# zaiisao/ConTEXTure-NeRF

Measured on AMD Instinct MI355X. Metric: UNet denoise steps/sec (CFG-batched SD2-depth UNet eval + PLMS update), higher is better.
Workload: dtype f16; 1 GPU; BASELINE configs[1]: 1 view @768^2 (latent 96^2), 50 PLMS steps (51 UNet evals), SD2-depth UNet fp16, CFG batch 2, guidance 10, random-init weights; mesh substitution napoleon.obj -> n/a for this stage (denoise loop only); latent=96, cfg_batch=2, ctx_len=77, views_per_rank=1, parallelism=view-shard x1

## Files before the change

contexture-nerf_amd/_lib.py:

```python
import ctypes as C
import os
import torch

_HERE = os.path.dirname(os.path.abspath(__file__))
LIB_PATH = os.path.join(_HERE, "libctxnerf.so")

_vp, _i32, _i64, _f32 = C.c_void_p, C.c_int32, C.c_int64, C.c_float

SIGNATURES = {
    "ctx_version": (_i32, []),
    "ctx_last_error": (C.c_char_p, []),
    "ctx_device_check": (_i32, []),
    "ctx_prepare_vertices": (_i32, [_vp, _vp, _vp, _vp, _i32, _i32, _i32, _vp, _vp, _vp, _vp, _vp]),
    "ctx_rasterize_ws_bytes": (_i64, [_i32, _i32, _i32, _i32]),
    "ctx_rasterize_fwd": (_i32, [_i32, _i32, _vp, _vp, _vp, _i32, _i32, _i32, _f32, _f32, _vp, _vp, _vp, _i64, _vp]),
    "ctx_rasterize_fused": (_i32, [_i32, _i32, _vp, _vp, _vp, _i32, _vp, _i32, _i32, _f32, _f32, _vp, _vp, _vp, _vp, _vp, _i64, _vp]),
    "ctx_normalize_depth_ws_bytes": (_i64, [_i32]),
    "ctx_normalize_depth": (_i32, [_vp, _i32, _i32, _vp, _vp, _vp, _vp]),
    "ctx_texture_mapping_fwd": (_i32, [_vp, _vp, _i32, _i32, _i32, _i32, _i32, _i32, _vp, _vp, _vp]),
    "ctx_texture_mapping_bwd": (_i32, [_vp, _vp, _i32, _i32, _i32, _i32, _vp, _vp, _vp]),
    "ctx_texmap_bwd_plan_bytes": (_i64, [_i32, _i32, _i32]),
    "ctx_texmap_bwd_plan": (_i32, [_vp, _vp, _i32, _i32, _i32, _vp, _vp]),
    "ctx_texture_mapping_bwd_binned_ws_bytes": (_i64, [_i32, _i32]),
    "ctx_texture_mapping_bwd_binned": (_i32, [_vp, _vp, _vp, _i32, _i32, _i32, _i32, _vp, _vp, _vp, _vp]),
    "ctx_texmap_plan_max_res": (_i32, []),
    "ctx_texmap_plan_stale": (_i32, [_vp, _vp]),
    "ctx_uv_scatter_fixed": (_i32, [_vp, _vp, _vp, _i32, _i32, _i32, _i32, _vp, _i32, _vp, _vp]),
    "ctx_fixed_to_float": (_i32, [_vp, _i64, _i32, _i32, _vp, _vp]),
    "ctx_uv_gather_ws_bytes": (_i64, [_i32, _i32]),
    "ctx_uv_gather_fixed": (_i32, [_vp, _vp, _vp, _vp, _vp, _vp, _vp, _i32, _i32, _i32, _i32, _i32, _i32, _i32, _vp, _vp, _i64, _vp]),
    "ctx_atlas_fill_ws_bytes": (_i64, [_i32]),
    "ctx_nearest_seed": (_i32, [_vp, _i32, _vp, _vp, _vp, _i64, _vp]),
    "ctx_atlas_fill": (_i32, [_vp, _vp, _vp, _i32, _i32, _i32, _vp, _vp, _vp, _i64, _vp]),
    "ctx_view_consistency_ws_bytes": (_i64, [_i32, _i32]),
    "ctx_view_consistency_fwd": (_i32, [_vp, _vp, _vp, _vp, _i32, _i32, _i32, _i32, _i32, _i32, _i32, _i32, _vp, _i64, _vp, _vp, _vp, _vp, _vp]),
    "ctx_view_consistency_bwd": (_i32, [_vp, _vp, _vp, _vp, _vp, _i32, _i32, _i32, _i32, _i32, _i32, _i32, _vp, _vp, _vp, _vp, _vp]),
    "ctx_texture_pack4": (_i32, [_vp, _i32, _i32, _vp, _vp]),
    "ctx_texture_mapping_packed_fwd": (_i32, [_vp, _vp, _i32, _i32, _i32, _i32, _i32, _vp, _vp, _vp]),
    "ctx_view_weights_max": (_i32, [_vp, _vp, _i32, _i32, _i32, _vp, _vp, _vp]),
    "ctx_view_weights_mask": (_i32, [_vp, _vp, _vp, _i32, _i32, _i32, _vp, _vp]),
    "ctx_face_view_map_ws_bytes": (_i64, [_i32, _i32, _i32]),
    "ctx_face_view_map": (_i32, [_vp, _i32, _i32, _i32, _vp, _vp, _vp, _vp]),
    "ctx_embed_fwd": (_i32, [_vp, _i64, _i32, _i32, _vp, _vp]),
    "ctx_uvmlp_packed_bytes": (_i64, [_i32, _i32, _i32, _i32, _i32]),
    "ctx_uvmlp_pack": (_i32, [_vp, _vp, _i32, _i32, _i32, _i32, _i32, _vp, _vp]),
    "ctx_uvmlp_fwd": (_i32, [_vp, _vp, _i64, _i32, _vp, _i32, _i32, _i32, _i32, _i32, _vp, _vp, _vp]),
    "ctx_uvmlp_saved_bytes": (_i64, [_i64, _i32, _i32, _i32]),
    "ctx_uvmlp_fwd_save": (_i32, [_vp, _vp, _i64, _i32, _vp, _i32, _i32, _i32, _i32, _i32, _i32, _vp, _vp, _vp, _vp]),
    "ctx_uvmlp_bwd_ws_bytes": (_i64, [_i64, _i32, _i32]),
    "ctx_uvmlp_bwd": (_i32, [_vp, _vp, _vp, _i64, _vp, _i32, _i32, _i32, _i32, _i32, _i32, _vp, _vp, _vp, _vp, _vp]),
    "ctx_texel_active_mark": (_i32, [_vp, _vp, _i32, _i32, _i32, _i32, _vp, _vp]),
    "ctx_texel_compact_ws_bytes": (_i64, [_i64]),
    "ctx_texel_compact": (_i32, [_vp, _i64, _vp, _vp, _vp, _vp]),
    "ctx_uvmlp_fwd_save_idx": (_i32, [_vp, _i64, _i32, _vp, _i32, _i32, _i32, _i32, _i32, _vp, _vp, _vp, _vp]),
    "ctx_uvmlp_bwd_idx": (_i32, [_vp, _vp, _vp, _i32, _vp, _i64, _vp, _i32, _i32, _i32, _i32, _i32, _vp, _vp, _vp, _vp, _vp]),
    "ctx_get_rays": (_i32, [_i32, _i32, _f32, _f32, _f32, _f32, _vp, _vp, _vp, _vp]),
    "ctx_raymarch_composite_fwd": (_i32, [_vp, _vp, _vp, _i64, _i32, _i32, _vp, _vp, _vp, _vp, _vp, _vp]),
    "ctx_raymarch_composite_fwd_noise": (_i32, [_vp, _vp, _vp, _vp, _i64, _i32, _i32, _vp, _vp, _vp, _vp, _vp, _vp]),
    "ctx_raymarch_composite_bwd": (_i32, [_vp, _vp, _vp, _vp, _i64, _i32, _i32, _vp, _vp, _vp, _vp, _vp, _vp, _vp]),
    "ctx_unet_create": (_vp, [_vp]),
    "ctx_unet_destroy": (None, [_vp]),
    "ctx_unet_param_count": (_i32, [_vp]),
    "ctx_unet_param_name": (C.c_char_p, [_vp, _i32]),
    "ctx_unet_param_shape": (_i32, [_vp, _i32, _vp]),
    "ctx_unet_weight_bytes": (_i64, [_vp]),
    "ctx_unet_workspace_bytes": (_i64, [_vp, _i32, _i32, _i32, _i32]),
    "ctx_unet_bind": (_i32, [_vp, _vp, _vp, _i64]),
    "ctx_unet_set_param": (_i32, [_vp, _i32, _vp, _vp]),
    "ctx_unet_forward": (_i32, [_vp, _vp, _vp, _vp, _i32, _i32, _i32, _i32, _vp, _vp]),
    "ctx_controlnet_create": (_vp, [_vp, _i32]),
    "ctx_controlnet_residual_bytes": (_i64, [_vp, _i32, _i32, _i32]),
    "ctx_controlnet_cond_cache_bytes": (_i64, [_vp, _i32, _i32, _i32]),
    "ctx_controlnet_forward": (_i32, [_vp, _vp, _vp, _vp, _vp, _vp, _i32, _i32, _i32, _i32, _i32, _vp, _vp]),
    "ctx_unet_set_residuals": (_i32, [_vp, _vp, C.c_float]),
    "ctx_unet_ref_bank_bytes": (_i64, [_vp, _i32, _i32, _i32]),
    "ctx_unet_workspace_bytes_ref": (_i64, [_vp, _i32, _i32, _i32, _i32, _i32, _i32]),
    "ctx_unet_forward_ref": (_i32, [_vp, _vp, _vp, _vp, _i32, _i32, _i32, _i32, _i32, _vp, _i32, _vp, _vp]),
    "ctx_unet_set_residual_fp32": (_i32, [_vp, _i32]),
    "ctx_unet_stats": (_i32, [_vp, _i32, _vp, _vp]),
    "ctx_unet_set_taps": (_i32, [_vp, _vp, _i64]),
    "ctx_unet_tap_count": (_i32, [_vp]),
    "ctx_unet_tap_info": (_i32, [_vp, _i32, _vp, _vp, _vp]),
    "ctx_vae_create": (_vp, [_vp]),
    "ctx_vae_destroy": (None, [_vp]),
    "ctx_vae_param_count": (_i32, [_vp]),
    "ctx_vae_param_name": (C.c_char_p, [_vp, _i32]),
    "ctx_vae_param_shape": (_i32, [_vp, _i32, _vp]),
    "ctx_vae_weight_bytes": (_i64, [_vp]),
    "ctx_vae_workspace_bytes": (_i64, [_vp, _i32, _i32, _i32]),
    "ctx_vae_bind": (_i32, [_vp, _vp, _vp, _i64]),
    "ctx_vae_set_param": (_i32, [_vp, _i32, _vp, _vp]),
    "ctx_vae_decode": (_i32, [_vp, _vp, _i32, _i32, _i32, _vp, _vp]),
    "ctx_vae_decoder_param_count": (_i32, [_vp]),
    "ctx_vae_encode_workspace_bytes": (_i64, [_vp, _i32, _i32, _i32]),
    "ctx_vae_encode": (_i32, [_vp, _vp, _i32, _i32, _i32, _vp, _vp]),
    "ctx_vae_flops": (C.c_double, [_vp]),
    "ctx_vae_encode_train_workspace_bytes": (_i64, [_vp, _i32, _i32, _i32]),
    "ctx_vae_encode_train": (_i32, [_vp, _vp, _i32, _i32, _i32, _vp, _vp]),
    "ctx_vae_encode_bwd": (_i32, [_vp, _vp, _f32, _vp, _vp]),
    "ctx_gemm_f16": (_i32, [_vp, _vp, _vp, _vp, _i32, _i32, _i32, _vp, _vp]),
    "ctx_conv3x3_f16": (_i32, [_vp, _vp, _vp, _vp, _vp, _i32, _i32, _i32, _i32, _i32, _i32, _i32, _vp, _vp]),
    "ctx_groupnorm_f16": (_i32, [_vp, _vp, _vp, _i32, _i32, _i32, _i32, _f32, _i32, _vp, _vp, _vp]),
    "ctx_layernorm_f16": (_i32, [_vp, _vp, _vp, _i64, _i32, _f32, _vp, _vp]),
    "ctx_attention_ws_bytes": (_i64, [_i32, _i32, _i32]),
    "ctx_attention_f16": (_i32, [_vp, _vp, _vp, _i32, _i32, _i32, _i32, _i32, _i32, _f32, _vp, _i32, _vp, _vp]),
    "ctx_groupnorm_ws_bytes": (_i64, [_i32, _i32]),
    "ctx_geglu_f16": (_i32, [_vp, _i64, _i32, _vp, _vp]),
    "ctx_profile_begin": (_i32, []),
    "ctx_profile_end": (_i32, [_i32, _vp, _vp]),
    "ctx_bench_gemm": (C.c_float, [_vp, _vp, _vp, _vp, _i32, _i32, _i32, _vp, _i32, _i32, _i32, _i32, _i32, _i32, _vp, _i32, _i32, _vp]),
    "ctx_gemm_tune": (None, [_i32, _i32]),
    "ctx_attention_tune": (None, [_i32, _i32, _i32, _f32]),
    "ctx_probe_mfma": (_i32, [_i32, _vp, _vp, _vp, _vp]),
    "ctx_probe_stage": (C.c_float, [_i32, _i32, _i32, _i32, _i32, _vp, _vp, _vp]),
    "ctx_cfg_plms_step": (_i32, [_vp, _i64, _f32, _vp, _i32, _vp, _f32, _f32, _i32, _vp, _vp, _vp]),
}


class CtxError(RuntimeError):
    pass


_lib = None


def load():
    global _lib
    if _lib is None:
        if not os.path.exists(LIB_PATH):
            raise CtxError(f"{LIB_PATH} is missing: run `python -c 'import __graft_entry__ as g; g.build()'` "
                           "(hipcc --offload-arch=gfx950). There is no CPU fallback for this path.")
        lib = C.CDLL(LIB_PATH)
        for name, (res, args) in SIGNATURES.items():
            if not hasattr(lib, name) and os.environ.get("CTX_ALLOW_PARTIAL") == "1":
                continue
            fn = getattr(lib, name)
            fn.restype = res
            fn.argtypes = args
        _lib = lib
    return _lib


def check(rc):
    if rc != 0:
        raise CtxError(f"libctxnerf error {rc}: {load().ctx_last_error().decode()}")


def stream():
    return C.c_void_p(torch.cuda.current_stream().cuda_stream)


def ptr(t, dtype=None, name="tensor"):
    if t is None:
        return C.c_void_p(0)
    if not isinstance(t, torch.Tensor) or not t.is_cuda:
        raise CtxError(f"{name}: expected a device tensor (the HIP path has no CPU fallback), got "
                       f"{type(t).__name__} on {getattr(t, 'device', '?')}")
    if not t.is_contiguous():
        raise CtxError(f"{name}: tensor must be contiguous")
    if dtype is not None and t.dtype != dtype:
        raise CtxError(f"{name}: expected dtype {dtype}, got {t.dtype}")
    return C.c_void_p(t.data_ptr())


def f32c(t, device=None):
    t = t.to(dtype=torch.float32)
    if device is not None:
        t = t.to(device)
    return t.contiguous()
```

contexture-nerf_amd/csrc/conv_halo.hip:

```cpp
#include "gemm_common.h"

#define CH_HP 328
#define CH_XPIECES 41

template <int NI>
__global__ __launch_bounds__(512) void k_conv_halo(GemmArgs a)
{
    constexpr int BN = 64 * NI;
    constexpr int WP = NI;
    constexpr int G = 1 + WP;
    constexpr int HALO = CH_HP * 64;
    constexpr int WST = BN * 64;
    extern __shared__ __attribute__((aligned(16))) f16 smem[];
    f16 *halo = smem;
    f16 *wring = smem + 2 * HALO;
    f16 *scratch = wring + 4 * WST;

    const int tid = threadIdx.x, lane = tid & 63, wave = __builtin_amdgcn_readfirstlane(tid >> 6);
    const int r = lane & 31, h = lane >> 5;
    const int wm = wave >> 1, wn = wave & 1;

    const int pw = a.W >> 4, ph = a.H >> 4;
    const int ntiles = a.ntm * a.ntn;
    const int lin = xcd_remap(blockIdx.x, ntiles * a.splitk);
// ... 53 lines not shown
    for (int mi = 0; mi < 2; ++mi) rc[mi] = (2 * wm + mi + 8 * (r >> 4) + 1) * 18 + (r & 15) + 1;
    const int wswz = (r >> 1) & 7;
    const int wrow = (wn * 32 * NI + r) * 64;

#pragma unroll
    for (int i = 0; i < 6; ++i) issue_x(wave + 8 * i, cbeg, 0);
    issue_w(0);
    issue_w(1);
    issue_w(2);
    asm volatile("s_waitcnt vmcnt(%0)" ::"n"(2 * WP) : "memory");
    ctx_barrier();
    const int grp = wave >> 2;
    if (grp == 1) ctx_barrier();

    for (int g = 0; g < nst; ++g) {
        const int ci = g / 9, t = g - ci * 9;
        const f16 *hb = halo + (ci & 1) * HALO;
        const f16 *wb = wring + (g & 3) * WST + wrow;
        const int dy = t / 3 - 1, dx = t - (t / 3) * 3 - 1;
        const int toff = dy * 18 + dx;
        int xr[2], xs[2];
#pragma unroll
        for (int mi = 0; mi < 2; ++mi) { const int R = rc[mi] + toff; xr[mi] = R * 64; xs[mi] = (R >> 1) & 7; }
        f16x8 xf[4][2], wf[4][NI];
#pragma unroll
        for (int ks = 0; ks < 4; ++ks) {
#pragma unroll
            for (int mi = 0; mi < 2; ++mi) xf[ks][mi] = *(const f16x8 *)(hb + xr[mi] + (((2 * ks + h) ^ xs[mi]) * 8));
#pragma unroll
            for (int j = 0; j < NI; ++j) wf[ks][j] = *(const f16x8 *)(wb + j * 32 * 64 + (((2 * ks + h) ^ wswz) * 8));
        }
        if (g == 0) asm volatile("s_waitcnt vmcnt(%0)" ::"n"(WP) : "memory");
        else asm volatile("s_waitcnt vmcnt(%0)" ::"n"(G) : "memory");
        __builtin_amdgcn_sched_barrier(0);
        ctx_barrier();
        __builtin_amdgcn_sched_barrier(0);
        __builtin_amdgcn_s_setprio(1);
#pragma unroll
        for (int ks = 0; ks < 4; ++ks) {
#pragma unroll
            for (int mi = 0; mi < 2; ++mi)
#pragma unroll
                for (int j = 0; j < NI; ++j) acc[mi][j] = __builtin_amdgcn_mfma_f32_32x32x16_f16(wf[ks][j], xf[ks][mi], acc[mi][j], 0, 0, 0);
            if (ks == 0) issue_x(t * 8 + wave, cbeg + ci + 1, (ci + 1) & 1);
            if (ks == 1) issue_w(g + 3);
        }
        __builtin_amdgcn_s_setprio(0);
        __builtin_amdgcn_sched_barrier(0);
        ctx_barrier();
        __builtin_amdgcn_sched_barrier(0);
    }
    if (grp == 0) ctx_barrier();
    asm volatile("s_waitcnt vmcnt(0)" ::: "memory");

    const int nw = n0 + wn * 32 * NI;
#pragma unroll
    for (int mi = 0; mi < 2; ++mi) {
        const int y = py0 + 2 * wm + mi + 8 * (r >> 4), x = px0 + (r & 15);
        const size_t m = ((size_t)b * a.H + y) * a.W + x;
        if (a.splitk > 1) {
            float *pb = a.part + ((size_t)slice * a.M + m) * a.N;
#pragma unroll
            for (int j = 0; j < NI; ++j)
#pragma unroll
                for (int g4 = 0; g4 < 4; ++g4) store_part4(a, pb, nw + j * 32 + 8 * g4 + 4 * h, acc4(acc[mi][j], g4));
            continue;
        }
        const int bidx = a.rowbias ? (int)(m / a.rows_per_batch) : 0;
#pragma unroll
        for (int j = 0; j < NI; ++j)
#pragma unroll
            for (int g4 = 0; g4 < 4; ++g4) {
                const int nn = nw + j * 32 + 8 * g4 + 4 * h;
                if (nn >= a.N) continue;
                f32x4 v = acc4(acc[mi][j], g4);
                if (a.bias) v = add4(v, *(const f16x4 *)(a.bias + nn));
                store4(a, v, m, bidx, nn);
            }
    }
}

int ctx_conv_halo_try(GemmArgs &a, int ni, hipStream_t s)
{
    if (a.stride != 1 || a.ups != 0 || (a.H & 15) || (a.W & 15) || a.Cin % 64 != 0 || a.epi != 0 || a.N % 8 != 0) return 0;
    const int B = a.M / (a.H * a.W);
    const int BN = 64 * ni;
    a.ntm = B * (a.H >> 4) * (a.W >> 4);
    a.ntn = cdiv(a.N, BN);
    const int S = (a.splitk > 1 && a.part) ? a.splitk : 1;
    if (S > a.Cin / 64) return 0;
    a.splitk = S;
    const size_t lds = (size_t)(2 * CH_HP * 64 + 4 * BN * 64 + 8 * 512) * sizeof(f16);
    const dim3 grid(a.ntm * a.ntn * S);
    if (ni == 2) ctx_launch<k_conv_halo<2>>(0, grid, dim3(512), lds, s, a); else ctx_launch<k_conv_halo<1>>(0, grid, dim3(512), lds, s, a);
    return 1;
}
```

contexture-nerf_amd/csrc/engine.h:

```cpp
#pragma once
#include "common.h"
#include "kernels.h"
#include <string>
#include <vector>

enum PackKind { PK_COPY = 0, PK_CONV3 = 1, PK_CONVIN = 2, PK_GEGLU_W = 3, PK_GEGLU_B = 4 };

struct Param {
    std::string name;
    int ndim;
    int64_t shape[4];
    int kind;
    size_t dst;
    int a, b;
    int kind2 = 0; size_t dst2 = 0; int pad2 = 0, ld2 = 0, col2 = 0;
};

struct Engine {
    const char *tag = "";
    std::vector<Param> params;
    size_t wtop = 0;
    f16 *W = nullptr;
    char *ws = nullptr;
    size_t ws_cap = 0;
    size_t top = 0, peak = 0;
    bool dry = false;
    hipStream_t s = nullptr;
    int rc = 0;
    int64_t launches[3] = {0, 0, 0};
    double flops[3] = {0, 0, 0};

    size_t walloc(size_t n) { size_t o = wtop; wtop += (n + 127) / 128 * 128; return o; }
    size_t add(const std::string &name, std::vector<int64_t> shp, int kind, size_t dst, int a = 0, int b = 0)
    {
        Param p; p.name = name; p.ndim = (int)shp.size(); p.kind = kind; p.dst = dst; p.a = a; p.b = b;
        for (int i = 0; i < 4; ++i) p.shape[i] = i < p.ndim ? shp[i] : 1;
        params.push_back(p);
        return dst;
    }
    size_t vec(const std::string &name, int n) { return add(name, {n}, PK_COPY, walloc(n)); }
    size_t lin(const std::string &name, int out, int in) { return add(name, {out, in}, PK_COPY, walloc((size_t)out * in)); }

    void *alloc(size_t bytes)
    {
        size_t o = (top + 255) / 256 * 256;
        top = o + bytes;
        if (top > peak) peak = top;
        if (!dry && top > ws_cap) { rc = CTX_E_STATE; ctx_set_error("%s: workspace too small (%zu > %zu)", tag, top, ws_cap); return ws; }
        return dry ? nullptr : (void *)(ws + o);
    }
    f16 *allocH(size_t n) { return (f16 *)alloc(n * 2); }

    void begin() { top = 0; peak = 0; rc = 0; for (int k = 0; k < 3; ++k) { launches[k] = 0; flops[k] = 0; } }
    void note(int klass, double fl, int n = 1) { launches[klass] += n; flops[klass] += fl; }
    bool live() const { return !dry && rc == 0; }
    void copy(void *dst, const void *src, size_t bytes) { if (live()) (void)hipMemcpyAsync(dst, src, bytes, hipMemcpyDeviceToDevice, s); }
    void copy2d(void *dst, size_t dpitch, const void *src, size_t spitch, size_t width, size_t rows)
    { if (live()) (void)hipMemcpy2DAsync(dst, dpitch, src, spitch, width, rows, hipMemcpyDeviceToDevice, s); }
};

#define ENGINE_RUN(e, expr) do { if ((e)->live()) { int r__ = (expr); if (r__ != 0) (e)->rc = r__; } } while (0)
#define ENGINE_LAUNCH(e, kernel, grid, block, lds, ...) do { if ((e)->live()) hipLaunchKernelGGL(kernel, grid, block, lds, (e)->s, __VA_ARGS__); } while (0)

void engine_linear(Engine &e, const f16 *X, const f16 *Wt, const f16 *bias, const void *res, int M, int N, int K, void *out, int ldc = 0,
                   int epi = 0, bool res32 = false, bool out32 = false);
struct ConvGeom { int stride = 1, ups = 0, poff = 0, zins = 0; };
void engine_conv3(Engine &e, const f16 *x, const f16 *Wt, const f16 *bias, const void *res, int B, int H, int W, int Cin, int Cout, void *out,
                  ConvGeom g = ConvGeom(), const f16 *rowbias = nullptr, int ldrb = 0, bool res32 = false, bool out32 = false);

template <class F> int engine_dry_run(Engine *e, F run)
{
    const bool was = e->dry;
    e->dry = true; const int rc = run(); e->dry = was;
    return rc;
}
inline int64_t engine_workspace_need(const Engine *e) { return (int64_t)e->peak + 4096; }
int engine_finish(Engine *e, const char *who);

int32_t engine_param_count(const Engine *e);
const char *engine_param_name(const Engine *e, int32_t i);
int32_t engine_param_shape(const Engine *e, int32_t i, int64_t shape4[4]);
int64_t engine_weight_bytes(const Engine *e);
int32_t engine_bind(Engine *e, void *weights, void *workspace, int64_t workspace_bytes, const char *who);
int32_t engine_set_param(Engine *e, int32_t i, const float *src, ctx_stream_t stream, const char *who);
```

contexture-nerf_amd/csrc/engine.hip:

```cpp
#include "engine.h"

int32_t engine_param_count(const Engine *e) { return e ? (int32_t)e->params.size() : 0; }
const char *engine_param_name(const Engine *e, int32_t i)
{
    return (e && i >= 0 && i < (int)e->params.size()) ? e->params[i].name.c_str() : "";
}
int32_t engine_param_shape(const Engine *e, int32_t i, int64_t shape4[4])
{
    if (!e || i < 0 || i >= (int)e->params.size()) return 0;
    for (int k = 0; k < 4; ++k) shape4[k] = e->params[i].shape[k];
    return e->params[i].ndim;
}
int64_t engine_weight_bytes(const Engine *e) { return e ? (int64_t)e->wtop * 2 + 256 : 0; }

int32_t engine_bind(Engine *e, void *weights, void *workspace, int64_t workspace_bytes, const char *who)
{
    CTX_REQUIRE(e && weights && workspace && workspace_bytes > 0, "%s: bad args", who);
    CTX_REQUIRE(((uintptr_t)weights & 255) == 0 && ((uintptr_t)workspace & 255) == 0, "%s: blobs must be 256-byte aligned", who);
    e->W = (f16 *)weights; e->ws = (char *)workspace; e->ws_cap = (size_t)workspace_bytes;
    return CTX_OK;
}

static void engine_gemm(Engine &e, GemmArgs &a, bool conv)
{
    e.note(0, 2.0 * a.M * a.N * a.K);
    size_t mark = e.top;
    ctx_gemm_plan(a, conv);
    if (a.zins) a.use8 = 0;
    if (a.splitk > 1) a.part = (float *)e.alloc((size_t)a.splitk * a.M * a.N * 4);
    ENGINE_RUN(&e, ctx_gemm_dispatch(a, conv, e.s));
    e.top = mark;
}

void engine_linear(Engine &e, const f16 *X, const f16 *Wt, const f16 *bias, const void *res, int M, int N, int K, void *out, int ldc, int epi,
                   bool res32, bool out32)
{
    GemmArgs a = {};
    a.X = X; a.Wt = Wt; a.bias = bias; a.residual = (const f16 *)res; a.out = (f16 *)out;
    a.M = M; a.N = N; a.K = K; a.ldc = ldc ? ldc : epi == 1 ? N / 2 : N; a.ldr = N; a.rows_per_batch = 1; a.ldrb = N; a.epi = epi;
    a.res32 = res32; a.out32 = out32;
    engine_gemm(e, a, false);
}

void engine_conv3(Engine &e, const f16 *x, const f16 *Wt, const f16 *bias, const void *res, int B, int H, int W, int Cin, int Cout, void *out,
                  ConvGeom g, const f16 *rowbias, int ldrb, bool res32, bool out32)
{
    GemmArgs a = {};
    a.Ho = ((H << g.ups) - 1) / g.stride + 1; a.Wo = ((W << g.ups) - 1) / g.stride + 1;
    a.X = x; a.Wt = Wt; a.bias = bias; a.rowbias = rowbias; a.residual = (const f16 *)res; a.out = (f16 *)out;
    a.M = B * a.Ho * a.Wo; a.N = Cout; a.K = 9 * Cin; a.ldc = Cout; a.ldr = Cout; a.rows_per_batch = a.Ho * a.Wo; a.ldrb = ldrb;
    a.H = H; a.W = W; a.Cin = Cin; a.stride = g.stride; a.ups = g.ups; a.poff = g.poff; a.zins = g.zins;
    a.res32 = res32; a.out32 = out32;
    engine_gemm(e, a, true);
}

int engine_finish(Engine *e, const char *who)
{
    if (e->live()) CTX_CHECK_LAUNCH(who);
    return e->rc;
}

__global__ void k_pack_copy(const float *__restrict__ s, int64_t n, f16 *__restrict__ d)
{
    for (int64_t i = (int64_t)blockIdx.x * 256 + threadIdx.x; i < n; i += (int64_t)gridDim.x * 256) d[i] = (f16)s[i];
}
__global__ void k_pack_conv3(const float *__restrict__ s, int Cout, int Cin, int Cinp, f16 *__restrict__ d)
{
    int64_t n = (int64_t)Cout * 9 * Cinp;
    for (int64_t i = (int64_t)blockIdx.x * 256 + threadIdx.x; i < n; i += (int64_t)gridDim.x * 256) {
        int c = (int)(i % Cinp);
        int tap = (int)((i / Cinp) % 9);
        int o = (int)(i / ((int64_t)Cinp * 9));
        d[i] = c < Cin ? (f16)s[((int64_t)o * Cin + c) * 9 + tap] : (f16)0.f;
    }
}
__global__ void k_pack_geglu(const float *__restrict__ s, int C4, int K, f16 *__restrict__ d)
{
    int64_t n = (int64_t)2 * C4 * (K > 0 ? K : 1);
    int kk = K > 0 ? K : 1;
    for (int64_t i = (int64_t)blockIdx.x * 256 + threadIdx.x; i < n; i += (int64_t)gridDim.x * 256) {
        int k = (int)(i % kk);
        int p = (int)(i / kk);
        int blk = p / 64, w = p % 64;
        int src = w < 32 ? blk * 32 + w : C4 + blk * 32 + (w - 32);
        d[i] = (f16)s[(int64_t)src * kk + k];
    }
}
__global__ void k_pack_conv3_T(const float *__restrict__ s, int Cout, int Cin, int pad, f16 *__restrict__ d)
{
    int64_t n = (int64_t)Cin * 9 * pad;
    for (int64_t i = (int64_t)blockIdx.x * 256 + threadIdx.x; i < n; i += (int64_t)gridDim.x * 256) {
        int o = (int)(i % pad), tp = (int)((i / pad) % 9), c = (int)(i / ((int64_t)pad * 9));
        int ky = 2 - tp / 3, kx = 2 - tp % 3;
        d[i] = o < Cout ? (f16)s[(((int64_t)o * Cin + c) * 3 + ky) * 3 + kx] : (f16)0.f;
    }
}
__global__ void k_pack_mat_T(const float *__restrict__ s, int out, int in, int ld, int col, f16 *__restrict__ d)
{
    int64_t n = (int64_t)out * in;
    for (int64_t i = (int64_t)blockIdx.x * 256 + threadIdx.x; i < n; i += (int64_t)gridDim.x * 256) {
        int c = (int)(i % in), o = (int)(i / in);
        d[(int64_t)c * ld + col + o] = (f16)s[i];
    }
}

int32_t engine_set_param(Engine *e, int32_t i, const float *src, ctx_stream_t stream, const char *who)
{
    CTX_REQUIRE(e && e->W && src && i >= 0 && i < (int)e->params.size(), "%s: bad args / not bound", who);
    const Param &p = e->params[i];
    hipStream_t s = (hipStream_t)stream;
    int64_t n = 1;
    for (int k = 0; k < p.ndim; ++k) n *= p.shape[k];
    f16 *d = e->W + p.dst;
    int64_t nbk = cdiv64(n, 256);
    unsigned nb = (unsigned)(nbk > 4096 ? 4096 : nbk);
    switch (p.kind) {
    case PK_COPY: hipLaunchKernelGGL(k_pack_copy, dim3(nb), dim3(256), 0, s, src, n, d); break;
    case PK_CONV3: hipLaunchKernelGGL(k_pack_conv3, dim3(nb), dim3(256), 0, s, src, p.a, p.b, p.b, d); break;
    case PK_CONVIN: hipLaunchKernelGGL(k_pack_conv3, dim3(nb), dim3(256), 0, s, src, p.a, p.b, p.b > 8 ? 16 : 8, d); break;
    case PK_GEGLU_W: hipLaunchKernelGGL(k_pack_geglu, dim3(nb), dim3(256), 0, s, src, p.a, p.b, d); break;
    case PK_GEGLU_B: hipLaunchKernelGGL(k_pack_geglu, dim3(nb), dim3(256), 0, s, src, p.a, 0, d); break;
    }
    if (p.kind2 == 1) hipLaunchKernelGGL(k_pack_conv3_T, dim3(nb), dim3(256), 0, s, src, p.a, p.b, p.pad2, e->W + p.dst2);
    else if (p.kind2 == 2) hipLaunchKernelGGL(k_pack_mat_T, dim3(nb), dim3(256), 0, s, src, (int)p.shape[0], (int)p.shape[1], p.ld2, p.col2, e->W + p.dst2);
    CTX_CHECK_LAUNCH(who);
    return CTX_OK;
}
```

contexture-nerf_amd/csrc/gemm.hip:

```cpp
#include "gemm_common.h"

template <int MI, int NI>
__device__ __forceinline__ void gemm_epilogue(const GemmArgs &a, f32x16 (&acc)[MI][NI], int mw, int nw, int r, int h)
{
#pragma unroll
    for (int mi = 0; mi < MI; ++mi) {
        int m = mw + mi * 32 + r;
        if (m >= a.M) continue;
        int bidx = a.rowbias ? m / a.rows_per_batch : 0;
        if (a.epi == 1) {
            if constexpr (NI == 2) {
                int fbase = nw / 2;
#pragma unroll
                for (int g = 0; g < 4; ++g) {
                    int nn = nw + 8 * g + 4 * h;
                    if (nn >= a.N) continue;
                    f16x4 o;
#pragma unroll
                    for (int j = 0; j < 4; ++j) {
                        float xv = acc[mi][0][4 * g + j], gv = acc[mi][1][4 * g + j];
                        if (a.bias) { xv += (float)a.bias[nn + j]; gv += (float)a.bias[nn + 32 + j]; }
                        o[j] = geglu(xv, gv);
                    }
                    *(f16x4 *)(a.out + (size_t)m * a.ldc + fbase + 8 * g + 4 * h) = o;
                }
            }
        } else {
#pragma unroll
            for (int ni = 0; ni < NI; ++ni)
#pragma unroll
                for (int g = 0; g < 4; ++g) {
                    int nn = nw + ni * 32 + 8 * g + 4 * h;
                    if (nn >= a.N) continue;
                    f32x4 v = acc4(acc[mi][ni], g);
                    if (a.bias) v = add4(v, *(const f16x4 *)(a.bias + nn));
                    store4<true>(a, v, m, bidx, nn);
                }
        }
    }
}

template <int MI, int NI>
__device__ __forceinline__ void gemm_epilogue_staged(const GemmArgs &a, f32x16 (&acc)[MI][NI], int mw, int nw, int r, int h,
                                                     float *stage, int lane)
{
    constexpr int RS = 32 * NI + 4;
    constexpr int LPR = 4 * NI;
    constexpr int RPP = 64 / LPR;
    const int prow = lane / LPR, c8 = (lane % LPR) * 8;
    const int n = nw + c8;
    f16x8 bs = {0, 0, 0, 0, 0, 0, 0, 0};
    if (a.bias && n < a.N) bs = *(const f16x8 *)(a.bias + n);
#pragma unroll
    for (int mi = 0; mi < MI; ++mi) {
#pragma unroll
        for (int ni = 0; ni < NI; ++ni)
#pragma unroll
            for (int g = 0; g < 4; ++g)
                *(f32x4 *)(stage + r * RS + ni * 32 + 8 * g + 4 * h) = acc4(acc[mi][ni], g);
#pragma unroll
        for (int p = 0; p < 32 / RPP; ++p) {
            const int row = RPP * p + prow;
            const int m = mw + mi * 32 + row;
            f32x4 v0 = *(const f32x4 *)(stage + row * RS + c8), v1 = *(const f32x4 *)(stage + row * RS + c8 + 4);
            if (m < a.M && n < a.N) {
                float v[8] = {v0[0], v0[1], v0[2], v0[3], v1[0], v1[1], v1[2], v1[3]};
                add8(v, bs);
                store8<true>(a, v, m, n);
            }
        }
    }
}

template <int WM, int WN, int MI, int NI, bool CONV, int NS, int PKT>
__global__ __launch_bounds__(64 * WM * WN) void k_gemm_pipe(GemmArgs a)
{
    constexpr int BM = 32 * MI * WM, BN = 32 * NI * WN, NW = WM * WN;
    constexpr int RP = 512 / PKT;
    constexpr int LPR = PKT / 8;
    constexpr int XI = BM / (RP * NW), WI = BN / (RP * NW);
    static_assert(XI >= 1 && WI >= 1, "tile too small for the wave count");
    constexpr int G = XI + WI;
    constexpr int STAGE = (BM + BN) * PKT;
    extern __shared__ __attribute__((aligned(16))) f16 smem[];

    const int tid = threadIdx.x, lane = tid & 63, wave = __builtin_amdgcn_readfirstlane(tid >> 6);
    const int r = lane & 31, h = lane >> 5;
    const int wm = wave / WN, wn = wave % WN;
    const GemmTile t = gemm_tile(a, blockIdx.x, PKT, BM, BN);
    const int slice = t.slice, tile_m = t.tile_m, tile_n = t.tile_n, m0 = t.m0, n0 = t.n0, kbeg = t.kbeg, nk = t.nk;
    const int lr = lane / LPR, pc = lane % LPR;

    const f16 *xp[XI], *wp[WI];
    int xst[XI], wst[WI];
    int xoff[XI], xoy[XI], xox[XI];
    bool xok[XI];
#pragma unroll
    for (int i = 0; i < XI; ++i) {
        int row = RP * (wave + NW * i) + lr;
        int m = m0 + row;
        const int lc = (pc ^ (PKT == 32 ? ((row >> 2) & 3) : ((row >> 1) & 7))) * 8;
        xok[i] = m < a.M;
        if (CONV) {
            conv_pixel(a, m, lc, xoy[i], xox[i], xoff[i]);
            xp[i] = ctx_zero_page; xst[i] = 0;
        } else {
            xoff[i] = 0; xoy[i] = 0; xox[i] = 0;
            xp[i] = xok[i] ? a.X + (size_t)m * a.K + kbeg * PKT + lc : ctx_zero_page;
            xst[i] = xok[i] ? PKT : 0;
        }
    }
#pragma unroll
    for (int i = 0; i < WI; ++i) {
        int row = RP * (wave + NW * i) + lr;
        bool ok = (n0 + row) < a.N;
        wp[i] = ok ? a.Wt + (size_t)(n0 + row) * a.K + kbeg * PKT + ((pc ^ (PKT == 32 ? ((row >> 2) & 3) : ((row >> 1) & 7))) * 8) : ctx_zero_page;
        wst[i] = ok ? PKT : 0;
    }
    const int k_lo = kbeg * PKT, k_hi = (kbeg + nk) * PKT;
    const int rot = a.krot == 1 ? (int)(((unsigned)tile_m * 13u + (unsigned)tile_n * 5u) % (unsigned)nk) : 0;
    int k_issue = k_lo + rot * PKT, issued = 0, tap_left = 0;
    if (!CONV) {
#pragma unroll
        for (int i = 0; i < XI; ++i) xp[i] += (xst[i] ? rot * PKT : 0);
    }
#pragma unroll
    for (int i = 0; i < WI; ++i) wp[i] += (wst[i] ? rot * PKT : 0);

    auto retap = [&]() {
        const ConvTap tap = conv_tap(a, k_issue);
#pragma unroll
        for (int i = 0; i < XI; ++i) {
            bool ok = xok[i];
            xp[i] = conv_tap_src<true>(a, tap, xoy[i], xox[i], xoff[i], ok);
            xst[i] = ok ? PKT : 0;
        }
        tap_left = (a.Cin - tap.c0) / PKT;
    };
    auto issue = [&](int buf) {
        if (k_issue == k_hi) {
            k_issue = k_lo;
            const int span = k_hi - k_lo;
            if (!CONV) {
#pragma unroll
                for (int i = 0; i < XI; ++i) xp[i] -= (xst[i] ? span : 0);
            }
#pragma unroll
            for (int i = 0; i < WI; ++i) wp[i] -= (wst[i] ? span : 0);
            tap_left = 0;
        }
        if (CONV) {
            if (tap_left == 0) retap();
            --tap_left;
        }
        f16 *Xs = smem + buf * STAGE;
        f16 *Ws = Xs + BM * PKT;
#pragma unroll
        for (int i = 0; i < XI; ++i) {
            __builtin_amdgcn_global_load_lds((gptr_t)xp[i], (lptr_t)(Xs + (wave + NW * i) * 512), 16, 0, 0);
            xp[i] += xst[i];
        }
#pragma unroll
        for (int i = 0; i < WI; ++i) {
            __builtin_amdgcn_global_load_lds((gptr_t)wp[i], (lptr_t)(Ws + (wave + NW * i) * 512), 16, 0, 0);
            wp[i] += wst[i];
        }
        k_issue += PKT;
        ++issued;
    };

    f32x16 acc[MI][NI];
#pragma unroll
    for (int i = 0; i < MI; ++i)
#pragma unroll
        for (int j = 0; j < NI; ++j)
#pragma unroll
            for (int q = 0; q < 16; ++q) acc[i][j][q] = 0.f;

#pragma unroll
    for (int p = 0; p < NS - 1; ++p)
        if (p < nk) issue(p);
    const int swz = PKT == 32 ? ((r >> 2) & 3) : ((r >> 1) & 7);
    const int xrow = (wm * 32 * MI + r) * PKT, wrow = BM * PKT + (wn * 32 * NI + r) * PKT;
    int kt = 0;
    for (; a.krot == 0 && kt + 2 * NS - 2 < nk; kt += NS) {
#pragma unroll
        for (int u = 0; u < NS; ++u) {
            asm volatile("s_waitcnt vmcnt(%0) lgkmcnt(0)" ::"n"((NS - 2) * G) : "memory");
            ctx_barrier();
            issue((u + NS - 1) % NS);
            const f16 *sb = smem + u * STAGE;
#pragma unroll
            for (int ks = 0; ks < PKT / 16; ++ks) {
                const int pch = ((2 * ks + h) ^ swz) * 8;
                f16x8 xf[MI], wf[NI];
#pragma unroll
                for (int i = 0; i < MI; ++i) xf[i] = *(const f16x8 *)(sb + xrow + i * 32 * PKT + pch);
#pragma unroll
                for (int j = 0; j < NI; ++j) wf[j] = *(const f16x8 *)(sb + wrow + j * 32 * PKT + pch);
#pragma unroll
                for (int i = 0; i < MI; ++i)
#pragma unroll
                    for (int j = 0; j < NI; ++j) acc[i][j] = __builtin_amdgcn_mfma_f32_32x32x16_f16(wf[j], xf[i], acc[i][j], 0, 0, 0);
            }
        }
    }
    for (; kt < nk; kt += NS) {
#pragma unroll
        for (int u = 0; u < NS; ++u) {
            if (kt + u < nk) {
                int newer = issued - 1 - (kt + u);
                if (NS >= 8 && newer >= 6) asm volatile("s_waitcnt vmcnt(%0)" ::"n"(6 * G) : "memory");
                else if (NS >= 7 && newer >= 5) asm volatile("s_waitcnt vmcnt(%0)" ::"n"(5 * G) : "memory");
                else if (NS >= 6 && newer >= 4) asm volatile("s_waitcnt vmcnt(%0)" ::"n"(4 * G) : "memory");
                else if (NS >= 5 && newer >= 3) asm volatile("s_waitcnt vmcnt(%0)" ::"n"(3 * G) : "memory");
                else if (NS >= 4 && newer >= 2) asm volatile("s_waitcnt vmcnt(%0)" ::"n"(2 * G) : "memory");
                else if (newer >= 1) asm volatile("s_waitcnt vmcnt(%0)" ::"n"(G) : "memory");
                else asm volatile("s_waitcnt vmcnt(0)" ::: "memory");
                asm volatile("s_waitcnt lgkmcnt(0)" ::: "memory");
                ctx_barrier();
                if (issued < nk) issue((u + NS - 1) % NS);
                const f16 *sb = smem + u * STAGE;
#pragma unroll
                for (int ks = 0; ks < PKT / 16; ++ks) {
                    const int pch = ((2 * ks + h) ^ swz) * 8;
                    f16x8 xf[MI], wf[NI];
#pragma unroll
                    for (int i = 0; i < MI; ++i) xf[i] = *(const f16x8 *)(sb + xrow + i * 32 * PKT + pch);
#pragma unroll
                    for (int j = 0; j < NI; ++j) wf[j] = *(const f16x8 *)(sb + wrow + j * 32 * PKT + pch);
#pragma unroll
                    for (int i = 0; i < MI; ++i)
#pragma unroll
                        for (int j = 0; j < NI; ++j) acc[i][j] = __builtin_amdgcn_mfma_f32_32x32x16_f16(wf[j], xf[i], acc[i][j], 0, 0, 0);
                }
            }
        }
    }
    if (a.splitk > 1) {
        float *pb = a.part + (size_t)slice * a.M * a.N;
#pragma unroll
        for (int mi = 0; mi < MI; ++mi) {
            int m = m0 + wm * 32 * MI + mi * 32 + r;
            if (m >= a.M) continue;
#pragma unroll
            for (int ni = 0; ni < NI; ++ni)
#pragma unroll
                for (int g = 0; g < 4; ++g)
                    store_part4(a, pb + (size_t)m * a.N, n0 + wn * 32 * NI + ni * 32 + 8 * g + 4 * h, acc4(acc[mi][ni], g));
        }
        return;
    }
    if (a.epi == 0 && a.stage_epi) {
        asm volatile("s_waitcnt vmcnt(0) lgkmcnt(0)" ::: "memory");
        ctx_barrier();
        gemm_epilogue_staged<MI, NI>(a, acc, m0 + wm * 32 * MI, n0 + wn * 32 * NI, r, h, (float *)smem + wave * (32 * (32 * NI + 4)), lane);
        return;
    }
    gemm_epilogue<MI, NI>(a, acc, m0 + wm * 32 * MI, n0 + wn * 32 * NI, r, h);
}

__global__ __launch_bounds__(256) void k_splitk_reduce(GemmArgs a)
{
    const int n4 = a.N / 4;
    const size_t total = (size_t)a.M * n4, MN = (size_t)a.M * a.N;
    for (size_t i = (size_t)blockIdx.x * 256 + threadIdx.x; i < total; i += (size_t)gridDim.x * 256) {
        int m = (int)(i / n4), nn = (int)(i % n4) * 4;
        f32x4 v = *(const f32x4 *)(a.part + (size_t)m * a.N + nn);
        for (int sidx = 1; sidx < a.splitk; ++sidx) {
            f32x4 p = *(const f32x4 *)(a.part + sidx * MN + (size_t)m * a.N + nn);
            v += p;
        }
        if (a.bias) v = add4(v, *(const f16x4 *)(a.bias + nn));
        store4<true>(a, v, m, a.rowbias ? m / a.rows_per_batch : 0, nn);
    }
}

static int g_force_tile = -1, g_force_gemm8 = -1;
extern "C" void ctx_gemm_tune(int32_t tile, int32_t gemm8)
{
    g_force_tile = tile;
    g_force_gemm8 = gemm8;
}

template <int WM, int WN, int MI, int NI, bool CONV, int NS = 4, int PKT = 32>
static void launch_gemm(GemmArgs &a, hipStream_t s)
{
    constexpr int BM = 32 * MI * WM, BN = 32 * NI * WN;
    a.ntm = cdiv(a.M, BM);
    a.ntn = cdiv(a.N, BN);
    if (a.splitk < 1 || !a.part) a.splitk = 1;
    static const int mfast = ctx_env_int("CTX_GEMM_MFAST", -1);
    a.mfast = mfast >= 0 ? mfast : ctx_gemm_mfast(a, CONV);
    static const int stg = ctx_env_int("CTX_GEMM_STAGE_EPI", 1);
    a.stage_epi = stg && (a.ldc % 8 == 0) && (!a.residual || a.ldr % 8 == 0) && (!a.rowbias || a.ldrb % 8 == 0) &&
                  (size_t)WM * WN * 32 * (32 * NI + 4) * sizeof(float) <= 160 * 1024;
    static const int steady = ctx_env_int("CTX_GEMM_STEADY", 1);
    a.pk = PKT; a.krot = steady ? 0 : 2;
    constexpr int NT = 64 * WM * WN;
    constexpr size_t ring = (size_t)NS * (BM + BN) * PKT * sizeof(f16);
    constexpr size_t patch = (size_t)WM * WN * 32 * (32 * NI + 4) * sizeof(float);
    constexpr size_t lds = (ring > patch || patch > 160 * 1024) ? ring : patch;
    ctx_launch<k_gemm_pipe<WM, WN, MI, NI, CONV, NS, PKT>>(0, dim3(a.ntm * a.ntn * a.splitk), dim3(NT), lds, s, a);
}

static void launch_reduce(GemmArgs &a, hipStream_t s)
{
    size_t total = (size_t)a.M * (a.N / 4);
    unsigned nb = (unsigned)((total + 255) / 256 < 2048 ? (total + 255) / 256 : 2048);
    ctx_launch<k_splitk_reduce>(0, dim3(nb), dim3(256), 0, s, a);
}

int ctx_gemm_pick_split(int M, int N, int K, int epi)
{
    static const int en = ctx_env_int("CTX_SPLITK", 1);
    if (!en || epi != 0 || N % 4) return 1;
    bool wide = (N % 128 == 0);
    int tiles = wide ? cdiv(M, 128) * cdiv(N, 128) : cdiv(M, 256) * cdiv(N, 64);
    if (tiles >= 200) return 1;
    if (K < 2048 && tiles > 48) return 1;
    int S = 640 / tiles;
    int maxS = (K / 32) / 8;
    if (S > maxS) S = maxS;
    if (S > 32) S = 32;
    return S < 2 ? 1 : S;
}

#include "gemm_tuned.h"
void ctx_gemm_plan(GemmArgs &a, bool conv)
{
    a.tile = -1; a.use8 = -1;
    static const int use_table = ctx_env_int("CTX_GEMM_TUNED", 1);
    if (use_table) {
        const int flags = conv ? ((a.stride == 2 ? 1 : 0) | (a.ups ? 2 : 0)) : 0;
        for (const TunedGemm &t : g_tuned)
            if (t.conv == (conv ? 1 : 0) && t.M == a.M && t.N == a.N && t.K == a.K && t.flags == flags && t.epi == a.epi) {
                a.tile = t.tile; a.use8 = t.use8; a.splitk = t.splitk;
                return;
            }
    }
    if (a.K % 64 == 0 && (!conv || a.Cin % 64 == 0)) {
        const double MN = (double)a.M * a.N;
        static const int heur144 = ctx_env_int("CTX_GEMM_HEUR144", 1);
        if (heur144 && a.epi == 0 && a.N % 8 == 0 && !a.zins && !a.res32 && !a.out32) {
            const int nt = cdiv(a.N, 160);
            const double fill = (double)a.N / (160.0 * nt);
            if (fill >= 0.9) {
                if (cdiv(a.M, 288) * nt >= 512) { a.tile = -1; a.use8 = 8; a.splitk = 1; return; }
                if (cdiv(a.M, 144) * nt >= 220) { a.tile = -1; a.use8 = 6; a.splitk = 1; return; }
            }
        }
        int tile, bm, bn;
        if (MN >= 5.0e6) { tile = a.epi == 1 ? 10 : (conv ? 12 : 11); bm = 256; bn = 128; }
        else if ((MN >= 2.5e6 && a.K >= 960) || (conv && MN >= 1.2e6 && a.K >= 5760)) { tile = 14; bm = 128; bn = 128; }
        else if (a.epi == 1) { tile = 16; bm = 64; bn = 128; }
        else { tile = 15; bm = 64; bn = 64; }
        const int tiles = cdiv(a.M, bm) * cdiv(a.N, bn);
        int S = 1;
        if (a.epi == 0 && a.N % 4 == 0) {
            S = 320 / tiles;
            const int maxS = a.K / 64 / 4;
            if (S > maxS) S = maxS;
            if (S > 12) S = 12;
            if (S < 1) S = 1;
        }
        a.tile = tile; a.splitk = S;
        a.use8 = (a.epi == 1 && MN >= 1.0e7) ? -1 : 0;
        return;
    }
    a.splitk = ctx_gemm_pick_split(a.M, a.N, a.K, a.epi);
}

int ctx_gemm_dispatch(GemmArgs &a, bool conv, hipStream_t s)
{
    const bool only_pipe = a.zins || a.res32 || a.out32;
    if (only_pipe) a.use8 = 0;
    const int want8 = only_pipe ? 0 : (g_force_gemm8 >= 0 ? g_force_gemm8 : a.use8);
    const int want_tile = g_force_tile >= 0 ? g_force_tile : (g_force_gemm8 >= 0 ? -1 : a.tile);
    const bool launched = want_tile < 0 && ((want8 >= 4 && want8 <= 8 && ctx_gemm144_try(a, conv, want8 - 4, s)) ||
                                            (conv && (want8 == 2 || want8 == 3) && ctx_conv_halo_try(a, want8 == 2 ? 2 : 1, s)) ||
                                            (want8 != 0 && want8 < 2 && ctx_gemm8_try(a, conv, want8 == 1, s)));
    if (!launched) {
        static const int big = ctx_env_int("CTX_GEMM_BIG", 1);
        const int S = a.splitk > 1 && a.part ? a.splitk : 1;
        auto wgs = [&](int bm, int bn) { return cdiv(a.M, bm) * cdiv(a.N, bn) * S; };
        const bool n128 = (a.N % 128 == 0);
        int pick;
        static const int bigk = ctx_env_int("CTX_GEMM_BIGK", 1024);
        if (big && a.M >= 8192 && a.N >= 256 && a.K >= bigk) pick = 0;
        else if (n128 && wgs(128, 128) >= 384) pick = 1;
        else if (!n128 && wgs(256, 64) >= 384) pick = 2;
        else if (wgs(128, 64) >= 320) pick = 3;
        else if (S > 1) pick = n128 ? 1 : 2;
        else pick = 4;
        static const int force = ctx_env_int("CTX_GEMM_TILE", -1);
        if (force >= 0) pick = force;
        if (want_tile >= 0) pick = want_tile;
        if (a.epi == 1 && (pick == 5 || pick == 6 || pick == 9 || pick == 11 || pick == 13 || pick == 15 || pick == 17 || pick == 19 || pick == 21 || pick == 23 || pick == 26 || pick == 27)) pick = 1;
        if (pick >= 10 && (a.K % 64 != 0 || (conv && a.Cin % 64 != 0))) pick = 1;
#define CTX_LAUNCH(WM_, WN_, MI_, NI_) do { if (conv) launch_gemm<WM_, WN_, MI_, NI_, true>(a, s); else launch_gemm<WM_, WN_, MI_, NI_, false>(a, s); } while (0)
        switch (pick) {
        case 0: CTX_LAUNCH(4, 2, 2, 2); break;
        case 1: CTX_LAUNCH(2, 2, 2, 2); break;
        case 2: CTX_LAUNCH(4, 1, 2, 2); break;
        case 3: CTX_LAUNCH(2, 1, 2, 2); break;
        case 4: CTX_LAUNCH(1, 1, 2, 2); break;
        case 5: CTX_LAUNCH(2, 2, 1, 1); break;
        case 6: CTX_LAUNCH(1, 2, 2, 1); break;
        case 7: CTX_LAUNCH(4, 2, 1, 2); break;
        case 8: CTX_LAUNCH(2, 2, 1, 2); break;
        case 9: CTX_LAUNCH(2, 2, 2, 1); break;
#define CTX_LAUNCH64(WM_, WN_, MI_, NI_) do { if (conv) launch_gemm<WM_, WN_, MI_, NI_, true, 3, 64>(a, s); else launch_gemm<WM_, WN_, MI_, NI_, false, 3, 64>(a, s); } while (0)
        case 10: CTX_LAUNCH64(8, 2, 1, 2); break;
        case 11: CTX_LAUNCH64(4, 4, 2, 1); break;
        case 12: CTX_LAUNCH64(4, 2, 2, 2); break;
        case 13: CTX_LAUNCH64(4, 4, 1, 1); break;
        case 14: CTX_LAUNCH64(4, 2, 1, 2); break;
        case 15: CTX_LAUNCH64(2, 2, 1, 1); break;
        case 16: CTX_LAUNCH64(2, 2, 1, 2); break;
        case 17: CTX_LAUNCH64(2, 2, 2, 1); break;
        case 18: CTX_LAUNCH64(2, 2, 2, 2); break;
#define CTX_LAUNCH64N2(WM_, WN_, MI_, NI_) do { if (conv) launch_gemm<WM_, WN_, MI_, NI_, true, 2, 64>(a, s); else launch_gemm<WM_, WN_, MI_, NI_, false, 2, 64>(a, s); } while (0)
        case 19: CTX_LAUNCH64N2(2, 2, 1, 1); break;
        case 20: CTX_LAUNCH64N2(4, 2, 1, 2); break;
        case 21: CTX_LAUNCH64N2(4, 4, 1, 1); break;
        case 22: CTX_LAUNCH64N2(2, 2, 2, 2); break;
#define CTX_LAUNCH64NS(NS_, WM_, WN_, MI_, NI_) do { if (conv) launch_gemm<WM_, WN_, MI_, NI_, true, NS_, 64>(a, s); else launch_gemm<WM_, WN_, MI_, NI_, false, NS_, 64>(a, s); } while (0)
        case 23: CTX_LAUNCH64NS(6, 2, 2, 1, 1); break;
        case 24: CTX_LAUNCH64NS(5, 2, 2, 1, 2); break;
        case 25: CTX_LAUNCH64NS(4, 4, 2, 1, 2); break;
        case 26: CTX_LAUNCH64NS(5, 2, 2, 2, 1); break;
        default: CTX_LAUNCH64N2(4, 2, 2, 5); break;
#undef CTX_LAUNCH64NS
#undef CTX_LAUNCH64N2
#undef CTX_LAUNCH64
        }
#undef CTX_LAUNCH
    }
    if (a.splitk > 1) launch_reduce(a, s);
    hipError_t e = hipGetLastError();
    if (e != hipSuccess) {
        ctx_set_error("gemm launch failed: %s", hipGetErrorString(e));
        return CTX_E_LAUNCH;
    }
    return CTX_OK;
}

extern "C" int32_t ctx_gemm_f16(const void *A, const void *Wt, const void *bias, const void *residual, int32_t M,
                                int32_t N, int32_t K, void *C, ctx_stream_t stream)
{
    CTX_REQUIRE(A && Wt && C, "gemm: null pointer");
    CTX_REQUIRE(M > 0 && N > 0 && K > 0 && K % 64 == 0 && N % 8 == 0, "gemm: need K%%64==0, N%%8==0 (M=%d N=%d K=%d)", M, N, K);
    CTX_REQUIRE((int64_t)M * K < (1ll << 31) && (int64_t)N * K < (1ll << 31), "gemm: operand too large for 32-bit offsets");
    GemmArgs a = {};
    a.X = (const f16 *)A; a.Wt = (const f16 *)Wt; a.bias = (const f16 *)bias; a.residual = (const f16 *)residual;
    a.out = (f16 *)C; a.M = M; a.N = N; a.K = K; a.ldc = N; a.ldr = N; a.rows_per_batch = 1; a.ldrb = N; a.epi = 0;
    a.tile = -1; a.use8 = -1;
    return ctx_gemm_dispatch(a, false, (hipStream_t)stream);
}

extern "C" int32_t ctx_conv3x3_f16(const void *x, const void *w, const void *bias, const void *rowbias,
                                   const void *residual, int32_t B, int32_t H, int32_t W, int32_t Cin, int32_t Cout,
                                   int32_t stride, int32_t upsample, void *y, ctx_stream_t stream)
{
    CTX_REQUIRE(x && w && y, "conv3x3: null pointer");
    CTX_REQUIRE(B > 0 && H > 0 && W > 0 && Cin % 64 == 0 && Cout % 8 == 0 && (stride == 1 || stride == 2) &&
                    (upsample == 0 || upsample == 1) && !(upsample && stride == 2),
                "conv3x3: need Cin%%64==0, Cout%%8==0, stride 1|2 (B=%d H=%d W=%d Cin=%d Cout=%d s=%d up=%d)", B, H, W, Cin, Cout, stride, upsample);
    GemmArgs a = {};
    int Hv = H << upsample, Wv = W << upsample;
    a.Ho = (Hv + 2 - 3) / stride + 1; a.Wo = (Wv + 2 - 3) / stride + 1;
    a.X = (const f16 *)x; a.Wt = (const f16 *)w; a.bias = (const f16 *)bias; a.rowbias = (const f16 *)rowbias;
    a.residual = (const f16 *)residual; a.out = (f16 *)y;
    a.M = B * a.Ho * a.Wo; a.N = Cout; a.K = 9 * Cin; a.ldc = Cout; a.ldr = Cout; a.rows_per_batch = a.Ho * a.Wo; a.ldrb = Cout; a.epi = 0;
    a.H = H; a.W = W; a.Cin = Cin; a.stride = stride; a.ups = upsample;
    a.tile = -1; a.use8 = -1;
    CTX_REQUIRE((int64_t)B * H * W * Cin < (1ll << 31) && (int64_t)Cout * a.K < (1ll << 31), "conv3x3: tensor too large for 32-bit offsets");
    return ctx_gemm_dispatch(a, true, (hipStream_t)stream);
}

#define GV_U 4
__global__ __launch_bounds__(256) void k_gemv_f16(const f16 *__restrict__ x, const f16 *__restrict__ w,
                                                  const f16 *__restrict__ bias, int Bm, int N, int K, int silu_in,
                                                  int silu_out, f16 *__restrict__ out)
{
    const int lane = threadIdx.x & 63;
    const int n0 = ((blockIdx.x * 256 + threadIdx.x) >> 6) * 2;
    if (n0 >= N) return;
    const int n1 = n0 + 1 < N ? n0 + 1 : n0;
    float acc[2][4] = {{0.f, 0.f, 0.f, 0.f}, {0.f, 0.f, 0.f, 0.f}};
    const f16x8 zero8 = {0, 0, 0, 0, 0, 0, 0, 0};
    for (int k0 = 0; k0 < K; k0 += 512 * GV_U) {
        f16x8 wv[2][GV_U];
#pragma unroll
        for (int u = 0; u < GV_U; ++u) {
            const int k = k0 + u * 512 + lane * 8;
            const int kc = k < K ? k : K - 8;
            wv[0][u] = *(const f16x8 *)(w + (size_t)n0 * K + kc);
            wv[1][u] = *(const f16x8 *)(w + (size_t)n1 * K + kc);
        }
#pragma unroll
        for (int u = 0; u < GV_U; ++u) {
            const int k = k0 + u * 512 + lane * 8;
            if (k >= K) { wv[0][u] = zero8; wv[1][u] = zero8; }
            const int kc = k < K ? k : K - 8;
            for (int b = 0; b < Bm; ++b) {
                f16x8 xv = *(const f16x8 *)(x + (size_t)b * K + kc);
#pragma unroll
                for (int j = 0; j < 8; ++j) {
                    float xf = (float)xv[j];
                    if (silu_in) xf = xf / (1.0f + __expf(-xf));
                    acc[0][b] += xf * (float)wv[0][u][j];
                    acc[1][b] += xf * (float)wv[1][u][j];
                }
            }
        }
    }
    for (int r = 0; r < 2; ++r) {
        const int n = n0 + r;
        for (int b = 0; b < Bm; ++b) {
            float v = wave_sum(acc[r][b]);
            if (lane == 0 && n < N) {
                if (bias) v += (float)bias[n];
                if (silu_out) v = v / (1.0f + __expf(-v));
                out[(size_t)b * N + n] = (f16)v;
            }
        }
    }
}

int ctx_gemv_f16(const f16 *x, const f16 *w, const f16 *bias, int Bm, int N, int K, int silu_in, int silu_out, f16 *out,
                 hipStream_t s)
{
    if (Bm < 1 || K % 8 != 0 || K < 8) {
        ctx_set_error("gemv: Bm=%d (>=1) K=%d (%%8)", Bm, K);
        return CTX_E_ARG;
    }
    for (int b0 = 0; b0 < Bm; b0 += 4) {
        const int nb = Bm - b0 < 4 ? Bm - b0 : 4;
        hipLaunchKernelGGL(k_gemv_f16, dim3(cdiv(N, 8)), dim3(256), 0, s, x + (size_t)b0 * K, w, bias, nb, N, K, silu_in, silu_out,
                           out + (size_t)b0 * N);
    }
    return CTX_OK;
}

extern "C" float ctx_bench_gemm(const void *A, const void *Wt, const void *bias, const void *residual, int32_t M, int32_t N,
                                int32_t K, void *C, int32_t conv_B, int32_t conv_H, int32_t conv_W, int32_t conv_Cin,
                                int32_t conv_flags, int32_t epi, void *part, int32_t splitk, int32_t iters, ctx_stream_t stream)
{
    hipStream_t s = (hipStream_t)stream;
    GemmArgs a = {};
    a.X = (const f16 *)A; a.Wt = (const f16 *)Wt; a.bias = (const f16 *)bias; a.residual = (const f16 *)residual; a.out = (f16 *)C;
    bool conv = conv_B > 0;
    if (conv) {
        a.stride = (conv_flags & 1) ? 2 : 1; a.ups = (conv_flags & 2) ? 1 : 0;
        int Hv = conv_H << a.ups, Wv = conv_W << a.ups;
        a.H = conv_H; a.W = conv_W; a.Cin = conv_Cin; a.Ho = (Hv - 1) / a.stride + 1; a.Wo = (Wv - 1) / a.stride + 1;
        a.M = conv_B * a.Ho * a.Wo; a.N = N; a.K = 9 * conv_Cin; a.rows_per_batch = a.Ho * a.Wo;
    } else {
        a.M = M; a.N = N; a.K = K; a.rows_per_batch = 1;
    }
    a.epi = epi;
    a.ldc = epi == 1 ? a.N / 2 : a.N; a.ldr = a.N; a.ldrb = a.N;
// ... 21 lines not shown
```

contexture-nerf_amd/csrc/gemm144.hip:

```cpp
#include "gemm_common.h"
#include <type_traits>

#define G144_BM 144
#define G144_BN 160
#define G144_STAGE ((G144_BM + G144_BN) * 64)

template <int WM, int WN, bool CONV, int NS, int VAR, bool UPS = false, int BMB = 9>
__global__ __launch_bounds__(64 * WM * WN) void k_gemm144(GemmArgs a)
{
    constexpr int NW = WM * WN, MI = BMB / WM, NI = 10 / WN;
    constexpr int BM = 16 * BMB, NPX = BM / 8;
    constexpr int NP = NPX + 20;
    constexpr int STAGE = (BM + G144_BN) * 64;
    static_assert(BMB % WM == 0 && (BMB == 9 || (BMB == 18 && VAR == 0)), "288-row tiles: lockstep schedule only");
    constexpr int SL = (NP + NW - 1) / NW;
    static_assert(9 % WM == 0 && 10 % WN == 0, "wave grid must divide 9 x 10 blocks");
    extern __shared__ __attribute__((aligned(16))) f16 smem[];
    const int tid = threadIdx.x, lane = tid & 63, wave = __builtin_amdgcn_readfirstlane(tid >> 6);
    const int wm = wave / WN, wn = wave % WN;
    const int r16 = lane & 15, kg = lane >> 4;

    const GemmTile tl = gemm_tile(a, blockIdx.x, 64, BM, G144_BN);
    const int slice = tl.slice, m0 = tl.m0, n0 = tl.n0, kbeg = tl.kbeg, nk = tl.nk;

    const int prow = lane >> 3, pc = lane & 7;
    constexpr bool FAST = CONV && !UPS;
    const f16 *pp[SL], *xcen[SL];
    int pst[SL], xoff[SL], xoy[SL], xox[SL], xlc[SL], xval[SL];
    bool xok[SL];
    const f16 *const zp = ctx_zero_page;
    const bool full = wave + NW * (SL - 1) < NP;
#pragma unroll
    for (int i = 0; i < SL; ++i) {
        const int p = wave + NW * i;
        const bool isx = p < NPX, live = p < NP;
        const int s = isx ? 8 * p + prow : 8 * (p - NPX) + prow;
        xlc[i] = (pc ^ ((s >> 1) & 7)) * 8;
        xoff[i] = 0; xoy[i] = 0; xox[i] = 0;
        if (isx) {
            const int m = m0 + s;
            xok[i] = m < a.M;
            if (CONV) {
                conv_pixel(a, xok[i] ? m : 0, xlc[i], xoy[i], xox[i], xoff[i]);
                pp[i] = zp; pst[i] = 0;
                if (FAST) {
                    xcen[i] = a.X + (size_t)xoff[i] + (size_t)(xoy[i] * a.W + xox[i]) * a.Cin;
                    int v = 0;
#pragma unroll
                    for (int t = 0; t < 9; ++t) {
                        const int iy = xoy[i] + t / 3 - 1 + a.poff, ix = xox[i] + t % 3 - 1 + a.poff;
                        if (xok[i] && iy >= 0 && iy < a.H && ix >= 0 && ix < a.W) v |= 1 << t;
                    }
                    xval[i] = v;
                }
            } else {
                pp[i] = xok[i] ? a.X + (size_t)m * a.K + (size_t)kbeg * 64 + xlc[i] : ctx_zero_page;
                pst[i] = xok[i] ? 64 : 0;
            }
        } else {
            const bool ok = live && (n0 + s) < a.N;
            xok[i] = ok;
            pp[i] = ok ? a.Wt + (size_t)(n0 + s) * a.K + (size_t)kbeg * 64 + xlc[i] : ctx_zero_page;
            pst[i] = ok ? 64 : 0;
        }
    }

    int k_issue = kbeg * 64, issued = 0, tap_left = 0;
    int cur_tap = CONV ? (kbeg * 64) / a.Cin : 0, cur_c0 = CONV ? kbeg * 64 - cur_tap * a.Cin : 0;
    auto retap = [&]() {
        if (FAST) {
            const int dy = cur_tap / 3 - 1 + a.poff, dx = cur_tap - (cur_tap / 3) * 3 - 1 + a.poff;
            const int soff = (dy * a.W + dx) * a.Cin + cur_c0;
#pragma unroll
            for (int i = 0; i < SL; ++i) {
                if (wave + NW * i >= NPX) continue;
                const bool v = (xval[i] >> cur_tap) & 1;
                pp[i] = v ? xcen[i] + soff : zp;
                pst[i] = v ? 64 : 0;
            }
            tap_left = (a.Cin - cur_c0) >> 6;
            return;
        }
        const ConvTap tap = conv_tap(a, k_issue);
#pragma unroll
        for (int i = 0; i < SL; ++i) {
            if (wave + NW * i >= NPX) continue;
            bool ok = xok[i];
            pp[i] = conv_tap_src(a, tap, xoy[i], xox[i], xoff[i], ok);
            pst[i] = ok ? 64 : 0;
        }
        tap_left = (a.Cin - tap.c0) / 64;
    };
    auto issue_begin = [&]() {
        if (CONV) {
            if (tap_left == 0) retap();
            --tap_left;
        }
    };
    auto issue_slot = [&](int buf, int i) {
        const int p = wave + NW * i;
        if (p < NP) {
            __builtin_amdgcn_global_load_lds((gptr_t)pp[i], (lptr_t)(smem + buf * STAGE + p * 512), 16, 0, 0);
            pp[i] += pst[i];
        }
    };
    auto issue_end = [&]() {
        k_issue += 64; ++issued;
        if (FAST) { cur_c0 += 64; if (cur_c0 == a.Cin) { cur_c0 = 0; ++cur_tap; } }
    };
    auto issue = [&](int buf) {
        issue_begin();
#pragma unroll
        for (int i = 0; i < SL; ++i) issue_slot(buf, i);
        issue_end();
    };

    f32x4 acc[MI][NI];
#pragma unroll
    for (int i = 0; i < MI; ++i)
#pragma unroll
        for (int j = 0; j < NI; ++j) acc[i][j] = (f32x4){0.f, 0.f, 0.f, 0.f};

    const int swz = (r16 >> 1) & 7;
    const int ck[2] = {(kg ^ swz) * 8, ((4 + kg) ^ swz) * 8};
    const int xrow = (wm * 16 * MI + r16) * 64, wrow = BM * 64 + (wn * 16 * NI + r16) * 64;

#pragma unroll
    for (int p = 0; p < NS - 1; ++p)
        if (p < nk) issue(p);
    auto wait_newer = [&](int newer) {
        if (newer >= 2) {
            if (full) asm volatile("s_waitcnt vmcnt(%0)" ::"n"(2 * SL) : "memory");
            else asm volatile("s_waitcnt vmcnt(%0)" ::"n"(2 * (SL - 1)) : "memory");
        } else if (newer >= 1) {
            if (full) asm volatile("s_waitcnt vmcnt(%0)" ::"n"(SL) : "memory");
            else asm volatile("s_waitcnt vmcnt(%0)" ::"n"(SL - 1) : "memory");
        } else
            asm volatile("s_waitcnt vmcnt(0)" ::: "memory");
    };
    int buf = 0;
    if constexpr (VAR == 0 && BMB == 18) {
        f16x8 xa[MI], wa[NI], wb[NI];
        auto mrow = [&](const f16x8 &xf, const f16x8 (&wf)[NI], int i) {
#pragma unroll
            for (int j = 0; j < NI; ++j) acc[i][j] = __builtin_amdgcn_mfma_f32_16x16x32_f16(wf[j], xf, acc[i][j], 0, 0, 0);
        };
        static_assert(BMB != 18 || SL <= MI, "one DMA piece per MFMA row");
        for (int kt = 0; kt < nk; ++kt) {
            wait_newer(issued - 1 - kt);
            asm volatile("s_waitcnt lgkmcnt(0)" ::: "memory");
            ctx_barrier();
            const bool go = issued < nk;
            const int pb = buf == 0 ? NS - 1 : buf - 1;
            const f16 *sb = smem + buf * STAGE;
#pragma unroll
            for (int i = 0; i < MI; ++i) xa[i] = *(const f16x8 *)(sb + xrow + i * 1024 + ck[0]);
#pragma unroll
            for (int j = 0; j < NI; ++j) wa[j] = *(const f16x8 *)(sb + wrow + j * 1024 + ck[0]);
            if (go) issue_begin();
#pragma unroll
            for (int i = 0; i < MI; ++i) {
                mrow(xa[i], wa, i);
                __builtin_amdgcn_sched_barrier(0);
                xa[i] = *(const f16x8 *)(sb + xrow + i * 1024 + ck[1]);
                if (i == 0) {
#pragma unroll
                    for (int j = 0; j < NI; ++j) wb[j] = *(const f16x8 *)(sb + wrow + j * 1024 + ck[1]);
                }
                if (go && i < SL) issue_slot(pb, i);
                __builtin_amdgcn_sched_barrier(0);
            }
            if (go) issue_end();
#pragma unroll
            for (int i = 0; i < MI; ++i) mrow(xa[i], wb, i);
            buf = buf == NS - 1 ? 0 : buf + 1;
        }
    } else if constexpr (VAR == 0) {
        for (int kt = 0; kt < nk; ++kt) {
            wait_newer(issued - 1 - kt);
            asm volatile("s_waitcnt lgkmcnt(0)" ::: "memory");
            ctx_barrier();
            if (issued < nk) issue(buf == 0 ? NS - 1 : buf - 1);
            const f16 *sb = smem + buf * STAGE;
#pragma unroll
            for (int ks = 0; ks < 2; ++ks) {
                f16x8 xf[MI], wf[NI];
#pragma unroll
                for (int i = 0; i < MI; ++i) xf[i] = *(const f16x8 *)(sb + xrow + i * 1024 + ck[ks]);
#pragma unroll
                for (int j = 0; j < NI; ++j) wf[j] = *(const f16x8 *)(sb + wrow + j * 1024 + ck[ks]);
#pragma unroll
// ... 76 lines not shown
                wait_newer(issued - 1 - (kt + 1));
            asm volatile("s_waitcnt lgkmcnt(0)" ::: "memory");
            ctx_barrier();
            const bool go = ST || issued < nk;
            const int pb = buf == 0 ? NS - 1 : buf - 1;
            const int nb_ = buf == NS - 1 ? 0 : buf + 1;
            const f16 *sc = smem + buf * STAGE, *sn = smem + nb_ * STAGE;
            const bool more = ST || kt + 1 < nk;
            if (go) issue_begin();
#pragma unroll
            for (int i = 0; i < MI; ++i) {
                mrow(xc[i], wc, i);
                __builtin_amdgcn_sched_barrier(0);
                if (i == 0) rd(xb, wb, sc, 1);
                if (go && i < SL) issue_slot(pb, i);
                __builtin_amdgcn_sched_barrier(0);
            }
            if (go) {
#pragma unroll
                for (int i = MI; i < SL; ++i) issue_slot(pb, i);
                issue_end();
            }
#pragma unroll
            for (int i = 0; i < MI; ++i) {
                mrow(xb[i], wb, i);
                if (i == 0) {
                    __builtin_amdgcn_sched_barrier(0);
                    if (more) rd(xn, wn_, sn, 0);
                    __builtin_amdgcn_sched_barrier(0);
                }
            }
            buf = nb_;
        };
        using T1 = std::integral_constant<bool, true>;
        using T0 = std::integral_constant<bool, false>;
        int kt = 0;
        for (; kt + 4 < nk; kt += 2) {
            stage(xp_, wp_, xq, wq, kt, T1{});
            stage(xq, wq, xp_, wp_, kt + 1, T1{});
        }
        for (; kt + 1 < nk; kt += 2) {
            stage(xp_, wp_, xq, wq, kt, T0{});
            stage(xq, wq, xp_, wp_, kt + 1, T0{});
        }
        if (kt < nk) stage(xp_, wp_, xq, wq, kt, T0{});
    }

    const int mb = m0 + wm * 16 * MI, nb = n0 + wn * 16 * NI;
    if (a.splitk > 1) {
        float *pb = a.part + (size_t)slice * a.M * a.N;
#pragma unroll
        for (int i = 0; i < MI; ++i) {
            const int m = mb + 16 * i + r16;
            if (m >= a.M) continue;
#pragma unroll
            for (int j = 0; j < NI; ++j) store_part4(a, pb + (size_t)m * a.N, nb + 16 * j + 4 * kg, acc[i][j]);
        }
        return;
    }
    if (a.stage_epi) {
        constexpr int RS = G144_BN + 4;
        float *tile = (float *)smem;
        asm volatile("s_waitcnt vmcnt(0) lgkmcnt(0)" ::: "memory");
        ctx_barrier();
        constexpr int NT = 64 * NW, CPR = G144_BN / 8;
#pragma unroll
        for (int half = 0; half < BMB / 9; ++half) {
            if (half) __syncthreads();
#pragma unroll
            for (int i = 0; i < MI; ++i) {
                const int blk = wm * MI + i;
                if (blk / 9 != half) continue;
#pragma unroll
                for (int j = 0; j < NI; ++j)
                    *(f32x4 *)(tile + ((blk - 9 * half) * 16 + r16) * RS + wn * 16 * NI + 16 * j + 4 * kg) = acc[i][j];
            }
            __syncthreads();
            for (int ch = tid; ch < 144 * CPR; ch += NT) {
                const int row = ch / CPR, c8 = (ch - row * CPR) * 8;
                const int m = m0 + 144 * half + row, n = n0 + c8;
                if (m >= a.M || n >= a.N) continue;
                const f32x4 v0 = *(const f32x4 *)(tile + row * RS + c8), v1 = *(const f32x4 *)(tile + row * RS + c8 + 4);
                float v[8] = {v0[0], v0[1], v0[2], v0[3], v1[0], v1[1], v1[2], v1[3]};
                if (a.bias) add8(v, *(const f16x8 *)(a.bias + n));
                store8(a, v, m, n);
            }
        }
        return;
    }
    f16x4 bs[NI];
#pragma unroll
    for (int j = 0; j < NI; ++j) {
        const int nn = nb + 16 * j + 4 * kg;
        bs[j] = (a.bias && nn < a.N) ? *(const f16x4 *)(a.bias + nn) : (f16x4){0, 0, 0, 0};
    }
#pragma unroll
    for (int i = 0; i < MI; ++i) {
        const int m = mb + 16 * i + r16;
        if (m >= a.M) continue;
        const int bidx = a.rowbias ? m / a.rows_per_batch : 0;
#pragma unroll
        for (int j = 0; j < NI; ++j) {
            const int nn = nb + 16 * j + 4 * kg;
            if (nn >= a.N) continue;
            store4(a, add4(acc[i][j], bs[j]), m, bidx, nn);
        }
    }
}

int ctx_gemm144_try(GemmArgs &a, bool conv, int form, hipStream_t s)
{
    if (a.K % 64 != 0 || (conv && a.Cin % 64 != 0) || a.N % 4 != 0 || a.epi != 0 || a.res32 || a.out32 || a.zins) return 0;
    if (a.ldc % 4 != 0 || (a.residual && a.ldr % 4 != 0) || (a.rowbias && a.ldrb % 4 != 0)) return 0;
    const int bm = form == 4 ? 288 : G144_BM;
    a.ntm = cdiv(a.M, bm);
    a.ntn = cdiv(a.N, G144_BN);
    int S = (a.splitk > 1 && a.part) ? a.splitk : 1;
    if (S > a.K / 64) S = a.K / 64;
    a.splitk = S;
    a.mfast = ctx_gemm_mfast(a, conv);
    static const int stg = ctx_env_int("CTX_G144_STAGE", 1);
    a.stage_epi = stg && form != 0 && a.N % 8 == 0 && a.ldc % 8 == 0 && (!a.residual || a.ldr % 8 == 0) && (!a.rowbias || a.ldrb % 8 == 0);
    const dim3 grid(a.ntm * a.ntn * S);
#define G144_GO(NT_, NS_, ...) ctx_launch<k_gemm144<__VA_ARGS__>>(0, grid, dim3(NT_), (size_t)NS_ * (bm + G144_BN) * 64 * sizeof(f16), s, a)
    const bool ups = conv && a.ups;
    switch (form) {
    case 4:
        if (!conv) G144_GO(960, 2, 3, 5, false, 2, 0, false, 18);
        else if (ups) G144_GO(960, 2, 3, 5, true, 2, 0, true, 18); else G144_GO(960, 2, 3, 5, true, 2, 0, false, 18);
        break;
    case 1:
        if (!conv) G144_GO(960, 3, 3, 5, false, 3, 0);
        else if (ups) G144_GO(960, 3, 3, 5, true, 3, 0, true); else G144_GO(960, 3, 3, 5, true, 3, 0);
        break;
    case 2:
        if (!conv) G144_GO(960, 4, 3, 5, false, 4, 1);
        else if (ups) G144_GO(960, 4, 3, 5, true, 4, 1, true); else G144_GO(960, 4, 3, 5, true, 4, 1);
        break;
    case 3:
        if (!conv) G144_GO(960, 4, 3, 5, false, 4, 2);
        else if (ups) G144_GO(960, 4, 3, 5, true, 4, 2, true); else G144_GO(960, 4, 3, 5, true, 4, 2);
        break;
    default:
        if (!conv) G144_GO(384, 3, 3, 2, false, 3, 0);
        else if (ups) G144_GO(384, 3, 3, 2, true, 3, 0, true); else G144_GO(384, 3, 3, 2, true, 3, 0);
        break;
    }
#undef G144_GO
    return 1;
}
```

contexture-nerf_amd/csrc/gemm8.hip:

```cpp
#include "gemm_common.h"
#include <type_traits>

#define G8_WAIT(n)                                                              \
    do {                                                                        \
        if ((n) >= 4) asm volatile("s_waitcnt vmcnt(8)" ::: "memory");          \
        else if ((n) == 3) asm volatile("s_waitcnt vmcnt(6)" ::: "memory");     \
        else if ((n) == 2) asm volatile("s_waitcnt vmcnt(4)" ::: "memory");     \
        else if ((n) == 1) asm volatile("s_waitcnt vmcnt(2)" ::: "memory");     \
        else asm volatile("s_waitcnt vmcnt(0)" ::: "memory");                   \
    } while (0)

template <bool CONV>
__global__ __launch_bounds__(512, 2) void k_gemm8(GemmArgs a)
{
    extern __shared__ __attribute__((aligned(16))) f16 smem[];
    const int tid = threadIdx.x, lane = tid & 63, wave = __builtin_amdgcn_readfirstlane(tid >> 6);
    const int wr = wave >> 2, wc = wave & 3;
    const int r16 = lane & 15, kg = lane >> 4;

    const GemmTile tl = gemm_tile(a, blockIdx.x, 64, 256, 256);
    const int slice = tl.slice, m0 = tl.m0, n0 = tl.n0, kbeg = tl.kbeg, nkt = tl.nk;
    const int nht = 4 * nkt;

    const int prow = lane >> 3, pc = lane & 7;
// ... 137 lines not shown
#pragma unroll
        for (int ks = 0; ks < 2; ++ks)
#pragma unroll
            for (int i = 0; i < 4; ++i)
#pragma unroll
                for (int j = 0; j < 2; ++j) acc[4 + i][j] = __builtin_amdgcn_mfma_f32_16x16x32_f16(wf0[j][ks], xf[i][ks], acc[4 + i][j], 0, 0, 0);
        __builtin_amdgcn_s_setprio(0);
        __builtin_amdgcn_sched_barrier(0);
        ctx_barrier();
        __builtin_amdgcn_sched_barrier(0);
    };
    {
        using T1 = std::integral_constant<bool, true>;
        using T0 = std::integral_constant<bool, false>;
        int t = 0;
        for (; t + 2 < nkt; ++t) ktile(t, T1{});
        for (; t < nkt; ++t) ktile(t, T0{});
    }
    if (wr == 0) ctx_barrier();

    const int mb = m0 + wr * 128, nb = n0 + wc * 64;
    if (a.splitk > 1) {
        float *pb = a.part + (size_t)slice * a.M * a.N;
#pragma unroll
        for (int i = 0; i < 8; ++i) {
            const int m = mb + 16 * i + r16;
            if (m >= a.M) continue;
#pragma unroll
            for (int j = 0; j < 4; ++j) store_part4(a, pb + (size_t)m * a.N, nb + 16 * j + 4 * kg, acc[i][j]);
        }
        return;
    }
    if (a.epi == 1) {
        const int fbase = nb / 2;
        f16x4 bv[2], bg[2];
#pragma unroll
        for (int j = 0; j < 2; ++j) {
            const int nn = nb + 16 * j + 4 * kg;
            bv[j] = (a.bias && nn < a.N) ? *(const f16x4 *)(a.bias + nn) : (f16x4){0, 0, 0, 0};
            bg[j] = (a.bias && nn < a.N) ? *(const f16x4 *)(a.bias + nn + 32) : (f16x4){0, 0, 0, 0};
        }
#pragma unroll
        for (int i = 0; i < 8; ++i) {
            const int m = mb + 16 * i + r16;
            if (m >= a.M) continue;
#pragma unroll
            for (int j = 0; j < 2; ++j) {
                const int nn = nb + 16 * j + 4 * kg;
                if (nn >= a.N) continue;
                f16x4 o;
#pragma unroll
                for (int e = 0; e < 4; ++e) o[e] = geglu(acc[i][j][e] + (float)bv[j][e], acc[i][2 + j][e] + (float)bg[j][e]);
                *(f16x4 *)(a.out + (size_t)m * a.ldc + fbase + 16 * j + 4 * kg) = o;
            }
        }
        return;
    }
    f16x4 bs[4];
#pragma unroll
    for (int j = 0; j < 4; ++j) {
        const int nn = nb + 16 * j + 4 * kg;
        bs[j] = (a.bias && nn < a.N) ? *(const f16x4 *)(a.bias + nn) : (f16x4){0, 0, 0, 0};
    }
#pragma unroll
    for (int i = 0; i < 8; ++i) {
        const int m = mb + 16 * i + r16;
        if (m >= a.M) continue;
        const int bidx = a.rowbias ? m / a.rows_per_batch : 0;
#pragma unroll
        for (int j = 0; j < 4; ++j) {
            const int nn = nb + 16 * j + 4 * kg;
            if (nn >= a.N) continue;
            store4(a, add4(acc[i][j], bs[j]), m, bidx, nn);
        }
    }
}

int ctx_gemm8_try(GemmArgs &a, bool conv, bool force, hipStream_t s)
{
    const int en = force ? 2 : ctx_env_int("CTX_GEMM8", 1);
    const int min_tiles = ctx_env_int("CTX_GEMM8_MIN_TILES", 180);
    if (!en) return 0;
    if (a.K % 64 != 0 || (conv && a.Cin % 64 != 0) || a.N % 8 != 0) return 0;
    if (a.epi == 1 && a.N % 64 != 0) return 0;
    const int ntm = cdiv(a.M, 256), ntn = cdiv(a.N, 256);
    const int S = (a.splitk > 1 && a.part) ? a.splitk : 1;
    if (en != 2) {
        const double useful = (double)a.M * a.N / ((double)ntm * ntn * 65536.0);
        if (ntm * ntn * S < min_tiles || useful < 0.8 || a.K / 64 / S < 4) return 0;
    }
    a.ntm = ntm; a.ntn = ntn; a.splitk = S;
    a.mfast = ctx_gemm_mfast(a, conv);
    const dim3 grid(ntm * ntn * S);
    if (conv) ctx_launch<k_gemm8<true>>(0, grid, dim3(512), 131072, s, a); else ctx_launch<k_gemm8<false>>(0, grid, dim3(512), 131072, s, a);
    return 1;
}
```

contexture-nerf_amd/csrc/gemm_common.h:

```cpp
#pragma once
#include "common.h"
#include "kernels.h"
#include <hip/hip_ext.h>
#include <stdlib.h>

typedef const __attribute__((address_space(1))) void *gptr_t;
typedef __attribute__((address_space(3))) void *lptr_t;
inline __device__ __attribute__((aligned(128))) f16 ctx_zero_page[64];

__device__ __forceinline__ int xcd_remap(int bid, int nwg)
{
    int q = nwg >> 3, r = nwg & 7, x = bid & 7;
    return (x < r ? x * (q + 1) : r * (q + 1) + (x - r) * q) + (bid >> 3);
}

struct GemmTile { int slice, tile_m, tile_n, m0, n0, kbeg, nk; };
__device__ __forceinline__ GemmTile gemm_tile(const GemmArgs &a, int block, int pkt, int bm, int bn)
{
    const int ntiles = a.ntm * a.ntn;
    const int lin = xcd_remap(block, ntiles * a.splitk);
    GemmTile t;
    t.slice = lin / ntiles;
    const int bid = lin - t.slice * ntiles;
    t.tile_n = a.mfast ? bid / a.ntm : bid % a.ntn;
    t.tile_m = a.mfast ? bid % a.ntm : bid / a.ntn;
    t.m0 = t.tile_m * bm; t.n0 = t.tile_n * bn;
    const int nk_all = a.K / pkt;
    t.kbeg = (int)((long)nk_all * t.slice / a.splitk);
    t.nk = (int)((long)nk_all * (t.slice + 1) / a.splitk) - t.kbeg;
    return t;
}

__device__ __forceinline__ void conv_pixel(const GemmArgs &a, int m, int lc, int &oy, int &ox, int &off)
{
    const int hw = a.Ho * a.Wo;
    const int b = m / hw, p = m - b * hw;
    const int y = p / a.Wo, x = p - y * a.Wo;
    off = b * a.H * a.W * a.Cin + lc;
    oy = y * a.stride; ox = x * a.stride;
}
struct ConvTap { int dy, dx, c0, Hv, Wv; };
__device__ __forceinline__ ConvTap conv_tap(const GemmArgs &a, int k0)
{
    const int tap = k0 / a.Cin;
    return {tap / 3 - 1 + a.poff, tap % 3 - 1 + a.poff, k0 - tap * a.Cin, a.H << a.ups, a.W << a.ups};
}
template <bool ZINS = false>
__device__ __forceinline__ const f16 *conv_tap_src(const GemmArgs &a, const ConvTap &t, int oy, int ox, int off, bool &ok)
{
    const int iy = oy + t.dy, ix = ox + t.dx;
    ok = ok && iy >= 0 && iy < t.Hv && ix >= 0 && ix < t.Wv;
    if (ZINS) ok = ok && !(a.zins && ((iy | ix) & 1));
    return ok ? a.X + off + (((iy >> a.ups) * a.W + (ix >> a.ups)) * a.Cin) + t.c0 : ctx_zero_page;
}

__device__ __forceinline__ float fast_erf(float x)
{
    float ax = __builtin_fabsf(x);
    float t = __builtin_amdgcn_rcpf(1.0f + 0.3275911f * ax);
    float p = t * (0.254829592f + t * (-0.284496736f + t * (1.421413741f + t * (-1.453152027f + t * 1.061405429f))));
    float e = 1.0f - p * __builtin_amdgcn_exp2f(-1.4426950408889634f * ax * ax);
    return __builtin_copysignf(e, x);
}
__device__ __forceinline__ float gelu_erf(float x) { return 0.5f * x * (1.0f + fast_erf(x * 0.70710678118654752f)); }

__device__ __forceinline__ f32x4 acc4(const f32x16 &c, int g) { return (f32x4){c[4 * g], c[4 * g + 1], c[4 * g + 2], c[4 * g + 3]}; }
__device__ __forceinline__ f32x4 add4(f32x4 v, f16x4 b)
{
#pragma unroll
    for (int e = 0; e < 4; ++e) v[e] += (float)b[e];
    return v;
}
__device__ __forceinline__ void add8(float (&v)[8], f16x8 b)
{
#pragma unroll
    for (int e = 0; e < 8; ++e) v[e] += (float)b[e];
}

template <bool F32 = false>
__device__ __forceinline__ void store4(const GemmArgs &a, f32x4 v, size_t m, int bidx, int nn)
{
    if (a.rowbias) v = add4(v, *(const f16x4 *)(a.rowbias + (size_t)bidx * a.ldrb + nn));
    if (a.residual) {
        if (F32 && a.res32) v += *(const f32x4 *)((const float *)a.residual + m * a.ldr + nn);
        else v = add4(v, *(const f16x4 *)(a.residual + m * a.ldr + nn));
    }
    if (F32 && a.out32) {
        *(f32x4 *)((float *)a.out + m * a.ldc + nn) = v;
        return;
    }
    f16x4 o;
#pragma unroll
    for (int e = 0; e < 4; ++e) o[e] = (f16)v[e];
    *(f16x4 *)(a.out + m * a.ldc + nn) = o;
}
template <bool F32 = false>
__device__ __forceinline__ void store8(const GemmArgs &a, float (&v)[8], int m, int n)
{
    if (a.rowbias) add8(v, *(const f16x8 *)(a.rowbias + (size_t)(m / a.rows_per_batch) * a.ldrb + n));
    if (a.residual) {
        if (F32 && a.res32) {
            const float *rp = (const float *)a.residual + (size_t)m * a.ldr + n;
            f32x4 b0 = *(const f32x4 *)rp, b1 = *(const f32x4 *)(rp + 4);
#pragma unroll
            for (int e = 0; e < 4; ++e) { v[e] += b0[e]; v[4 + e] += b1[e]; }
        } else
            add8(v, *(const f16x8 *)(a.residual + (size_t)m * a.ldr + n));
    }
    if (F32 && a.out32) {
        float *op = (float *)a.out + (size_t)m * a.ldc + n;
        *(f32x4 *)op = (f32x4){v[0], v[1], v[2], v[3]}; *(f32x4 *)(op + 4) = (f32x4){v[4], v[5], v[6], v[7]};
        return;
    }
    f16x8 o;
#pragma unroll
    for (int e = 0; e < 8; ++e) o[e] = (f16)v[e];
    *(f16x8 *)(a.out + (size_t)m * a.ldc + n) = o;
}
__device__ __forceinline__ void store_part4(const GemmArgs &a, float *row, int nn, f32x4 v)
{
    if (nn < a.N) *(f32x4 *)(row + nn) = v;
}
__device__ __forceinline__ f16 geglu(float xv, float gv) { return (f16)(xv * gelu_erf(gv)); }

static inline int ctx_gemm_mfast(const GemmArgs &a, bool conv)
{
    const double wbytes = (double)a.N * a.K, xbytes = (double)a.M * (conv ? a.Cin : a.K);
    return wbytes > xbytes ? 1 : 0;
}
template <auto KERN, class Args>
static inline void ctx_launch(int klass, dim3 grid, dim3 block, size_t lds, hipStream_t s, const Args &a)
{
    static bool attr_done = false;
    if (lds && !attr_done) {
        (void)hipFuncSetAttribute((const void *)KERN, hipFuncAttributeMaxDynamicSharedMemorySize, (int)lds);
        attr_done = true;
    }
    if (ctx_prof_on()) {
        hipEvent_t e0, e1;
        ctx_prof_events(klass, &e0, &e1);
        hipExtLaunchKernelGGL(KERN, grid, block, lds, s, e0, e1, 0, a);
    } else
        hipLaunchKernelGGL(KERN, grid, block, lds, s, a);
}
```

contexture-nerf_amd/csrc/kernels.h:

```cpp
#pragma once
#include "common.h"

struct GemmArgs {
    const f16 *X;
    const f16 *Wt;
    const f16 *bias;
    const f16 *rowbias;
    const f16 *residual;
    f16 *out;
    int M, N, K;
    int ldc, ldr;
    int rows_per_batch;
    int ldrb;
    int epi;
    int H, W, Cin, Ho, Wo, stride, ups;
    int poff;
    int res32, out32;
    int zins;
    int ntm, ntn;
    int splitk;
    float *part;
    int pk;
    int krot;
    int tile, use8;
    int stage_epi;
    int mfast;
};

int ctx_gemm_dispatch(GemmArgs &a, bool conv, hipStream_t s);
int ctx_gemm8_try(GemmArgs &a, bool conv, bool force, hipStream_t s);
int ctx_conv_halo_try(GemmArgs &a, int ni, hipStream_t s);
int ctx_gemm144_try(GemmArgs &a, bool conv, int form, hipStream_t s);
int ctx_gemm_pick_split(int M, int N, int K, int epi);
void ctx_gemm_plan(GemmArgs &a, bool conv);
int ctx_gemv_f16(const f16 *x, const f16 *w, const f16 *bias, int Bm, int N, int K, int silu_in, int silu_out, f16 *out, hipStream_t s);
int ctx_concat_f16(const f16 *a, const f16 *b, int64_t M, int Ca, int Cb, f16 *y, hipStream_t s);
int ctx_transpose_v_f16(const f16 *v, int B, int S, int ld, int heads, int Sp, f16 *vt, hipStream_t s);
int ctx_f32_to_f16(const float *x, int64_t n, f16 *y, hipStream_t s);
int ctx_time_embed_f16(const float *t, int B, int dim, f16 *out, hipStream_t s);
int ctx_conv_in_f16(const float *x, const f16 *w, const f16 *bias, int B, int Cin, int H, int W, int Cout, f16 *y, hipStream_t s);
int ctx_conv_out_f16(const f16 *x, const f16 *w, const f16 *bias, int B, int H, int W, int C, int Cout, float *out, hipStream_t s);
int ctx_attention_core(const f16 *Q, const f16 *K, const f16 *V, int B, int Sq, int Skv, int heads, int q_stride,
                       int kv_stride, float scale, f16 *O, int o_stride, hipStream_t s);
extern "C" int64_t ctx_groupnorm_ws_bytes(int32_t B, int32_t groups);
int ctx_groupnorm_any(const void *x, int x32, const void *gamma, const void *beta, int B, int HW, int C, int groups, float eps, int silu,
                      void *y, void *stats_ws, hipStream_t stream);
int64_t ctx_groupnorm_bwd_ws_bytes(int B, int groups);
int ctx_groupnorm_bwd_f16(const f16 *x, const f16 *dy, const f16 *gamma, const f16 *beta, const f16 *add, int B, int HW, int C, int groups,
                          float eps, int silu, f16 *dx, void *ws, hipStream_t s);
int ctx_layernorm_any(const void *x, int x32, const void *gamma, const void *beta, int64_t rows, int C, float eps, void *y, hipStream_t stream);
int ctx_concat_f32(const float *a, const float *b, int64_t M, int Ca, int Cb, float *y, hipStream_t s);
int ctx_f16_to_f32(const f16 *x, int64_t n, float *y, hipStream_t s);

bool ctx_prof_on(void);
void ctx_prof_events(int klass, hipEvent_t *a, hipEvent_t *b);
```

contexture-nerf_amd/csrc/norm.hip:

```cpp
#include "common.h"
#include "kernels.h"
#include <math.h>


struct Wide8 {
    float v[8];
    __device__ __forceinline__ float get(int j) const { return v[j]; }
};
template <bool X32> struct Raw8;
template <> struct Raw8<false> {
    f16x8 a;
    __device__ __forceinline__ float get(int j) const { return (float)a[j]; }
    __device__ __forceinline__ Wide8 widen() const
    {
        Wide8 r;
#pragma unroll
        for (int j = 0; j < 8; ++j) r.v[j] = (float)a[j];
        return r;
    }
};
template <> struct Raw8<true> {
    f32x4 a, b;
    __device__ __forceinline__ float get(int j) const { return j < 4 ? a[j] : b[j - 4]; }
    __device__ __forceinline__ Wide8 widen() const
    {
        Wide8 r;
#pragma unroll
        for (int j = 0; j < 4; ++j) { r.v[j] = a[j]; r.v[4 + j] = b[j]; }
        return r;
    }
};
template <bool X32>
__device__ __forceinline__ Raw8<X32> ldraw(const void *base, size_t elem)
{
    Raw8<X32> r;
    if constexpr (X32) { r.a = *(const f32x4 *)((const float *)base + elem); r.b = *(const f32x4 *)((const float *)base + elem + 4); }
    else r.a = *(const f16x8 *)((const f16 *)base + elem);
    return r;
}

#define GN_MAX_GROUPS 64
#define GN_MAX_SPLITS 128
#define GN_MAX_C 4096
#define GN_U 4
#define GN_AU 6
#define GN_FOLD 8

template <bool X32>
__global__ __launch_bounds__(1024) void k_gn_stats(const void *__restrict__ x, int HW, int C, int G, int NS, int PL,
                                                   float *__restrict__ part)
{
    extern __shared__ float s_part[];
    const int c8n = C / 8;
    const int b = blockIdx.y, sp = blockIdx.x;
    const int c8 = threadIdx.x % c8n, pl = threadIdx.x / c8n;
    const int per = (HW + NS - 1) / NS;
    const int p0 = sp * per, p1 = min(HW, p0 + per);
    float s[8], q[8];
#pragma unroll
    for (int j = 0; j < 8; ++j) { s[j] = 0.f; q[j] = 0.f; }
    const size_t base = ((size_t)b * HW) * C + c8 * 8;
    for (int p = p0 + pl; p < p1; p += PL * GN_U) {
        Wide8 v[GN_U];
#pragma unroll
        for (int u = 0; u < GN_U; ++u) v[u] = ldraw<X32>(x, base + (size_t)min(p + u * PL, p1 - 1) * C).widen();
#pragma unroll
        for (int u = 0; u < GN_U; ++u) {
            const bool live = p + u * PL < p1;
#pragma unroll
            for (int j = 0; j < 8; ++j) { float f = live ? v[u].get(j) : 0.f; s[j] += f; q[j] += f * f; }
        }
    }
#pragma unroll
    for (int j = 0; j < 8; ++j) {
        s_part[((size_t)pl * C + c8 * 8 + j) * 2 + 0] = s[j];
        s_part[((size_t)pl * C + c8 * 8 + j) * 2 + 1] = q[j];
    }
    __syncthreads();
    float *s_ch = s_part + (size_t)PL * C * 2;
    const int na = max(1, (int)blockDim.x / C);
    for (int it = threadIdx.x; it < C * na; it += blockDim.x) {
        const int a = it / C, c = it - a * C;
        float ss = 0.f, qq = 0.f;
#pragma unroll 4
        for (int l = a; l < PL; l += na) {
            ss += s_part[((size_t)l * C + c) * 2 + 0];
            qq += s_part[((size_t)l * C + c) * 2 + 1];
        }
        s_ch[((size_t)a * C + c) * 2 + 0] = ss;
        s_ch[((size_t)a * C + c) * 2 + 1] = qq;
    }
    __syncthreads();
    const int cg = C / G, cells = na * cg;
    const int octs = (int)blockDim.x >> 3;
    for (int g0 = 0; g0 < G; g0 += octs) {
        const int oc = (int)threadIdx.x >> 3, l = threadIdx.x & 7;
        const int g = oc < octs ? g0 + oc : G;
        float ss = 0.f, qq = 0.f;
        if (g < G)
            for (int k = l; k < cells; k += 8) {
                int a = k / cg, c = g * cg + (k - a * cg);
                ss += s_ch[((size_t)a * C + c) * 2 + 0];
                qq += s_ch[((size_t)a * C + c) * 2 + 1];
            }
#pragma unroll
        for (int o = 4; o > 0; o >>= 1) { ss += __shfl_xor(ss, o, 64); qq += __shfl_xor(qq, o, 64); }
        if (g < G && l == 0) {
            part[(((size_t)b * NS + sp) * G + g) * 2 + 0] = ss;
            part[(((size_t)b * NS + sp) * G + g) * 2 + 1] = qq;
        }
    }
}

__device__ __forceinline__ float2 gn_mean_rstd(float sum, float sumsq, float n, float eps)
{
    const float mean = sum / n;
    return make_float2(mean, rsqrtf(fmaxf(sumsq / n - mean * mean, 0.f) + eps));
}
template <class MR>
__device__ __forceinline__ void gn_scale_shift(MR mr, f16x8 ga, f16x8 be, float (&sa)[8], float (&sh)[8])
{
#pragma unroll
    for (int j = 0; j < 8; ++j) {
        const float2 m = mr(j);
        sa[j] = m.y * (float)ga[j];
        sh[j] = (float)be[j] - m.x * sa[j];
    }
}
template <class V8>
__device__ __forceinline__ void gn_store(const V8 &v, const float (&sa)[8], const float (&sh)[8], int silu, f16 *dst)
{
    f16x8 o;
#pragma unroll
    for (int j = 0; j < 8; ++j) {
        float t = v.get(j) * sa[j] + sh[j];
        if (silu) t = t * __builtin_amdgcn_rcpf(1.0f + __builtin_amdgcn_exp2f(-1.4426950408889634f * t));
        o[j] = (f16)t;
    }
    *(f16x8 *)dst = o;
}

template <bool X32>
__global__ __launch_bounds__(512) void k_gn_apply(const void *__restrict__ x, const float *__restrict__ part,
                                                  const f16 *__restrict__ gamma, const f16 *__restrict__ beta, int HW, int C,
                                                  int G, int NS, int PL, float eps, int silu, f16 *__restrict__ y)
{
    constexpr int AU = GN_AU;
    __shared__ float s_mean[GN_MAX_GROUPS], s_rstd[GN_MAX_GROUPS];
    const int b = blockIdx.y;
    const int c8n = C / 8;
    const int c8 = threadIdx.x % c8n, pl = threadIdx.x / c8n;
    const int p0 = blockIdx.x * (PL * AU);
    const size_t xb = (size_t)b * HW * C + c8 * 8;
    f16 *yb = y + (size_t)b * HW * C + c8 * 8;
    Raw8<X32> v[AU];
#pragma unroll
    for (int u = 0; u < AU; ++u) v[u] = ldraw<X32>(x, xb + (size_t)min(p0 + u * PL + pl, HW - 1) * C);
    const f16x8 ga = *(const f16x8 *)(gamma + c8 * 8), be = *(const f16x8 *)(beta + c8 * 8);
    if (threadIdx.x < 256) {
        const int lpg = min(256 / G, 64);
        const int gi = threadIdx.x / lpg, l = threadIdx.x % lpg;
        const int g = min(gi, G - 1);
        float s = 0.f, q = 0.f;
        for (int k0 = 0; k0 < NS; k0 += GN_FOLD * lpg) {
            float2 pv[GN_FOLD];
#pragma unroll
            for (int k = 0; k < GN_FOLD; ++k)
                pv[k] = *(const float2 *)(part + (((size_t)b * NS + min(k0 + k * lpg + l, NS - 1)) * G + g) * 2);
#pragma unroll
            for (int k = 0; k < GN_FOLD; ++k)
                if (k0 + k * lpg + l < NS) { s += pv[k].x; q += pv[k].y; }
        }
        for (int o = lpg >> 1; o > 0; o >>= 1) { s += __shfl_xor(s, o, 64); q += __shfl_xor(q, o, 64); }
        if (l == 0 && gi < G) {
            const float2 m = gn_mean_rstd(s, q, (float)HW * (float)(C / G), eps);
            s_mean[g] = m.x;
            s_rstd[g] = m.y;
        }
    }
    __syncthreads();
    const int cg = C / G;
    float sa[8], sh[8];
    gn_scale_shift([&](int j) { const int gg = (c8 * 8 + j) / cg; return make_float2(s_mean[gg], s_rstd[gg]); }, ga, be, sa, sh);
#pragma unroll
    for (int u = 0; u < AU; ++u) {
        const int p = p0 + u * PL + pl;
        if (p < HW) gn_store(v[u], sa, sh, silu, yb + (size_t)p * C);
    }
}

#define GN_FT 512
#define GN_FU 12
template <bool X32>
__global__ __launch_bounds__(GN_FT) void k_gn_fused(const void *__restrict__ x, const f16 *__restrict__ gamma,
                                                    const f16 *__restrict__ beta, int HW, int C, int G, int PLF, float eps, int silu,
                                                    f16 *__restrict__ y)
{
    __shared__ float s_red[2][GN_FT / 64];
    const int g = blockIdx.x, b = blockIdx.y;
    const int cg = C / G, cpg = cg / 8;
    const int c = threadIdx.x % cpg, pl = threadIdx.x / cpg;
    const bool act = pl < PLF;
    const size_t xb = (size_t)b * HW * C + g * cg + c * 8;
    f16 *yb = y + (size_t)b * HW * C + g * cg + c * 8;
    const f16x8 ga = *(const f16x8 *)(gamma + g * cg + c * 8), be = *(const f16x8 *)(beta + g * cg + c * 8);
    Wide8 v[GN_FU];
#pragma unroll
    for (int u = 0; u < GN_FU; ++u) v[u] = ldraw<X32>(x, xb + (size_t)min(pl + PLF * u, HW - 1) * C).widen();
    float s = 0.f, q = 0.f;
#pragma unroll
    for (int u = 0; u < GN_FU; ++u)
        if (act && pl + PLF * u < HW) {
#pragma unroll
            for (int j = 0; j < 8; ++j) { float f = v[u].get(j); s += f; q += f * f; }
        }
    s = wave_sum_dpp(s); q = wave_sum_dpp(q);
    const int wave = threadIdx.x >> 6;
    if ((threadIdx.x & 63) == 0) { s_red[0][wave] = s; s_red[1][wave] = q; }
    __syncthreads();
    float ss = 0.f, qq = 0.f;
    const int nw = ((int)blockDim.x + 63) >> 6;
    for (int w = 0; w < nw; ++w) { ss += s_red[0][w]; qq += s_red[1][w]; }
    const float2 m = gn_mean_rstd(ss, qq, (float)HW * (float)cg, eps);
    float sa[8], sh[8];
    gn_scale_shift([&](int) { return m; }, ga, be, sa, sh);
#pragma unroll
    for (int u = 0; u < GN_FU; ++u) {
        const int p = pl + PLF * u;
        if (act && p < HW) gn_store(v[u], sa, sh, silu, yb + (size_t)p * C);
    }
}

extern "C" int64_t ctx_groupnorm_ws_bytes(int32_t B, int32_t groups)
{
    return ((int64_t)B * GN_MAX_SPLITS * groups * 2 + (int64_t)B * 2 * GN_MAX_C) * 4;
}

extern "C" int32_t ctx_groupnorm_f16(const void *x, const void *gamma, const void *beta, int32_t B, int32_t HW, int32_t C,
                                     int32_t groups, float eps, int32_t silu, void *y, void *stats_ws, ctx_stream_t stream)
{
    return ctx_groupnorm_any(x, 0, gamma, beta, B, HW, C, groups, eps, silu, y, stats_ws, (hipStream_t)stream);
}

int ctx_groupnorm_any(const void *x, int x32, const void *gamma, const void *beta, int B, int HW, int C, int groups, float eps, int silu,
                      void *y, void *stats_ws, hipStream_t stream)
{
    CTX_REQUIRE(x && gamma && beta && y && stats_ws, "groupnorm: null pointer");
    CTX_REQUIRE(B > 0 && HW > 0 && C % 8 == 0 && C % groups == 0 && groups <= GN_MAX_GROUPS && C <= GN_MAX_C &&
                    256 % groups == 0 && (256 / groups & (256 / groups - 1)) == 0,
                "groupnorm: unsupported B=%d HW=%d C=%d groups=%d", B, HW, C, groups);
    {
        static const int fuse = ctx_env_int("CTX_GN_FUSED", 1);
        const int cg = C / groups;
        const int cpg = cg / 8;
        const int plf = cg % 8 == 0 ? GN_FT / cpg : 0;
        if (fuse && cg % 8 == 0 && cpg <= GN_FT && (HW + plf - 1) / plf <= GN_FU) {
            const int thr = (cpg * plf + 63) / 64 * 64;
            CTX_BOOL_GO(x32, X, hipLaunchKernelGGL(k_gn_fused<X>, dim3(groups, B), dim3(thr), 0, stream, x, (const f16 *)gamma, (const f16 *)beta, HW, C,
                                                   groups, plf, eps, silu, (f16 *)y));
            CTX_CHECK_LAUNCH("groupnorm");
            return CTX_OK;
        }
    }
    int c8n = C / 8;
    int PL = 1024 / c8n;
    if (PL < 1) PL = 1;
    if (PL > HW) PL = HW;
    int threads = c8n * PL;
    int NS = min(GN_MAX_SPLITS, max(1, HW / PL));
    {
        static const int ns_env = ctx_env_int("CTX_GN_NS", 0);
        const int64_t sample_bytes = (int64_t)HW * C * (x32 ? 4 : 2);
        const int by_size = (int)min((int64_t)GN_MAX_SPLITS, sample_bytes / (384 * 1024));
        const int want = ns_env > 0 ? ns_env : max(16, max(by_size, (64 + B - 1) / B));
        NS = min(NS, want);
    }
    float *part = (float *)stats_ws;
    const int na = threads / C > 1 ? threads / C : 1;
    size_t lds = (size_t)(PL + na) * C * 2 * sizeof(float);
    static bool attr = false;
    if (!attr) {
        (void)hipFuncSetAttribute((const void *)k_gn_stats<false>, hipFuncAttributeMaxDynamicSharedMemorySize, 80 * 1024);
        (void)hipFuncSetAttribute((const void *)k_gn_stats<true>, hipFuncAttributeMaxDynamicSharedMemorySize, 80 * 1024);
        attr = true;
    }
    CTX_BOOL_GO(x32, X, hipLaunchKernelGGL(k_gn_stats<X>, dim3(NS, B), dim3(threads), lds, stream, x, HW, C, groups, NS, PL, part));
    {
        const int apl = (256 + c8n - 1) / c8n;
        const int athreads = c8n * apl;
        const int nb = (HW + apl * GN_AU - 1) / (apl * GN_AU);
        CTX_BOOL_GO(x32, X, hipLaunchKernelGGL(k_gn_apply<X>, dim3(nb, B), dim3(athreads), 0, stream, x, part, (const f16 *)gamma, (const f16 *)beta, HW, C,
                                               groups, NS, apl, eps, silu, (f16 *)y));
    }
    CTX_CHECK_LAUNCH("groupnorm");
    return CTX_OK;
}

#define GNB_MAX_SPLITS 128

__device__ __forceinline__ float gnb_du(float dy, float u, float gamma, int silu)
{
    if (silu) { const float sg = 1.0f / (1.0f + __expf(-u)); dy *= sg * (1.0f + u * (1.0f - sg)); }
    return dy * gamma;
}
template <int MODE>
__global__ __launch_bounds__(256) void k_gnb_reduce(const f16 *__restrict__ x, const f16 *__restrict__ dy, const f16 *__restrict__ gamma,
                                                    const f16 *__restrict__ beta, const float *__restrict__ mr, int HW, int C, int G, int NS,
                                                    int silu, float *__restrict__ part)
{
    extern __shared__ float sm[];
    const int c8n = C / 8, PL = 256 / c8n;
    const int b = blockIdx.y, sp = blockIdx.x;
    const int c8 = threadIdx.x % c8n, pl = threadIdx.x / c8n;
    const int per = (HW + NS - 1) / NS, p0 = sp * per, p1 = min(HW, p0 + per), cg = C / G;
    float s[8], q[8], a[8], b0[8], ga[8], mu[8], rs[8];
#pragma unroll
    for (int j = 0; j < 8; ++j) {
        s[j] = 0.f; q[j] = 0.f;
        if (MODE == 1) {
            const int c = c8 * 8 + j, g = c / cg;
            mu[j] = mr[((size_t)b * G + g) * 2]; rs[j] = mr[((size_t)b * G + g) * 2 + 1];
            ga[j] = (float)gamma[c]; a[j] = rs[j] * ga[j]; b0[j] = (float)beta[c] - mu[j] * a[j];
        }
    }
    if (pl < PL)
        for (int p = p0 + pl; p < p1; p += PL) {
            const size_t off = ((size_t)b * HW + p) * C + c8 * 8;
            const f16x8 xv = *(const f16x8 *)(x + off);
            if (MODE == 0) {
#pragma unroll
                for (int j = 0; j < 8; ++j) { float f = (float)xv[j]; s[j] += f; q[j] += f * f; }
            } else {
                const f16x8 dv = *(const f16x8 *)(dy + off);
#pragma unroll
                for (int j = 0; j < 8; ++j) {
                    const float xf = (float)xv[j], du = gnb_du((float)dv[j], xf * a[j] + b0[j], ga[j], silu);
                    s[j] += du; q[j] += du * ((xf - mu[j]) * rs[j]);
                }
            }
        }
    if (pl < PL) {
#pragma unroll
        for (int j = 0; j < 8; ++j) { sm[((size_t)pl * C + c8 * 8 + j) * 2] = s[j]; sm[((size_t)pl * C + c8 * 8 + j) * 2 + 1] = q[j]; }
    }
    __syncthreads();
    float *ch = sm + (size_t)PL * C * 2;
    for (int c = threadIdx.x; c < C; c += 256) {
        float ss = 0.f, qq = 0.f;
        for (int l = 0; l < PL; ++l) { ss += sm[((size_t)l * C + c) * 2]; qq += sm[((size_t)l * C + c) * 2 + 1]; }
        ch[c * 2] = ss; ch[c * 2 + 1] = qq;
    }
    __syncthreads();
    for (int g = threadIdx.x; g < G; g += 256) {
        float ss = 0.f, qq = 0.f;
        for (int c = g * cg; c < (g + 1) * cg; ++c) { ss += ch[c * 2]; qq += ch[c * 2 + 1]; }
        part[(((size_t)b * NS + sp) * G + g) * 2] = ss; part[(((size_t)b * NS + sp) * G + g) * 2 + 1] = qq;
    }
}
template <int MODE>
__global__ void k_gnb_finalize(const float *__restrict__ part, int G, int NS, float n, float eps, float *__restrict__ out)
{
    const int b = blockIdx.x;
    for (int g = threadIdx.x; g < G; g += blockDim.x) {
        float ss = 0.f, qq = 0.f;
        for (int k = 0; k < NS; ++k) { ss += part[(((size_t)b * NS + k) * G + g) * 2]; qq += part[(((size_t)b * NS + k) * G + g) * 2 + 1]; }
        if (MODE == 0) {
            const float2 m = gn_mean_rstd(ss, qq, n, eps);
            out[((size_t)b * G + g) * 2] = m.x; out[((size_t)b * G + g) * 2 + 1] = m.y;
        } else { out[((size_t)b * G + g) * 2] = ss / n; out[((size_t)b * G + g) * 2 + 1] = qq / n; }
    }
}
__global__ __launch_bounds__(256) void k_gnb_apply(const f16 *__restrict__ x, const f16 *__restrict__ dy, const f16 *__restrict__ gamma,
                                                   const f16 *__restrict__ beta, const float *__restrict__ mr, const float *__restrict__ cc,
                                                   const f16 *__restrict__ add, int HW, int C, int G, int silu, f16 *__restrict__ dx)
// ... 183 lines not shown
```

contexture-nerf_amd/csrc/unet.hip:

```cpp
#include "engine.h"
#include <string.h>

struct ResP {
    int cin, cout;
    size_t n1g, n1b, c1w, c1b, n2g, n2b, c2w, c2b, scw, scb;
    int temb_row;
};
struct TrP {
    int C, heads;
    size_t ng, nb, piw, pib, l1g, l1b, qkv, o1w, o1b, l2g, l2b, q2, kv2, o2w, o2b, l3g, l3b, f1w, f1b, f2w, f2b, pow_, pob;
    int kv_row;
};
struct LevelP {
    std::vector<ResP> res;
    std::vector<TrP> tr;
    bool has_attn = false, has_sampler = false;
    size_t sw = 0, sb = 0;
    int sc = 0;
};

struct ctx_unet : Engine {
    ctx_unet_config_t cfg;
    size_t ciw, cib, t1w, t1b, t2w, t2b, tpw, tpb, cng, cnb, cow, cob;
    int temb_dim = 0, temb_rows = 0;
// ... 232 lines not shown
extern "C" int32_t ctx_unet_param_count(const ctx_unet_t *u) { return engine_param_count(u); }
extern "C" const char *ctx_unet_param_name(const ctx_unet_t *u, int32_t i) { return engine_param_name(u, i); }
extern "C" int32_t ctx_unet_param_shape(const ctx_unet_t *u, int32_t i, int64_t shape4[4]) { return engine_param_shape(u, i, shape4); }
extern "C" int64_t ctx_unet_weight_bytes(const ctx_unet_t *u) { return engine_weight_bytes(u); }
extern "C" int32_t ctx_unet_bind(ctx_unet_t *u, void *weights, void *workspace, int64_t workspace_bytes)
{
    return engine_bind(u, weights, workspace, workspace_bytes, "unet_bind");
}
extern "C" int32_t ctx_unet_set_param(ctx_unet_t *u, int32_t i, const float *src, ctx_stream_t stream)
{
    return engine_set_param(u, i, src, stream, "unet_set_param");
}

__global__ __launch_bounds__(256) void k_conv_small(const float *__restrict__ x32, const f16 *__restrict__ x16, const f16 *__restrict__ w,
                                                    const f16 *__restrict__ bias, int B, int H, int W, int Cin, int Cout, int stride,
                                                    int silu, f16 *__restrict__ y)
{
    const int Ho = (H - 1) / stride + 1, Wo = (W - 1) / stride + 1, o8n = Cout / 8;
    const int64_t total = (int64_t)B * Ho * Wo * o8n;
    for (int64_t i = (int64_t)blockIdx.x * 256 + threadIdx.x; i < total; i += (int64_t)gridDim.x * 256) {
        const int o8 = (int)(i % o8n);
        const int64_t pix = i / o8n;
        const int b = (int)(pix / ((int64_t)Ho * Wo)), p = (int)(pix % ((int64_t)Ho * Wo));
        const int oy = p / Wo, ox = p % Wo;
        float acc[8];
#pragma unroll
        for (int j = 0; j < 8; ++j) acc[j] = (float)bias[o8 * 8 + j];
        for (int t = 0; t < 9; ++t) {
            const int iy = oy * stride + t / 3 - 1, ix = ox * stride + t % 3 - 1;
            if (iy < 0 || iy >= H || ix < 0 || ix >= W) continue;
            if (x16 && (Cin & 7) == 0) {
                const f16 *xp = x16 + (((int64_t)b * H + iy) * W + ix) * Cin;
                const f16 *wp = w + ((int64_t)(o8 * 8) * 9 + t) * Cin;
                for (int c = 0; c < Cin; c += 8) {
                    const f16x8 xv = *(const f16x8 *)(xp + c);
                    float xf[8];
#pragma unroll
                    for (int q = 0; q < 8; ++q) xf[q] = (float)xv[q];
#pragma unroll
                    for (int j = 0; j < 8; ++j) {
                        const f16x8 wv = *(const f16x8 *)(wp + (int64_t)j * 9 * Cin + c);
#pragma unroll
                        for (int q = 0; q < 8; ++q) acc[j] += xf[q] * (float)wv[q];
                    }
                }
                continue;
            }
            for (int c = 0; c < Cin; ++c) {
                const float v = x32 ? (float)(f16)x32[(((int64_t)b * Cin + c) * H + iy) * W + ix]
                                    : (float)x16[(((int64_t)b * H + iy) * W + ix) * Cin + c];
#pragma unroll
                for (int j = 0; j < 8; ++j) acc[j] += v * (float)w[(((int64_t)(o8 * 8 + j)) * 9 + t) * Cin + c];
            }
        }
        f16x8 o;
#pragma unroll
        for (int j = 0; j < 8; ++j) {
            float v = acc[j];
            if (silu) v = v / (1.0f + __expf(-v));
            o[j] = (f16)v;
        }
        *(f16x8 *)(y + pix * Cout + o8 * 8) = o;
    }
}

__global__ __launch_bounds__(256) void k_add_scaled_f16(f16 *__restrict__ dst, const f16 *__restrict__ src, float scale, int64_t n8)
{
    for (int64_t i = (int64_t)blockIdx.x * 256 + threadIdx.x; i < n8; i += (int64_t)gridDim.x * 256) {
        f16x8 a = *(const f16x8 *)(dst + i * 8), b = *(const f16x8 *)(src + i * 8);
#pragma unroll
        for (int j = 0; j < 8; ++j) a[j] = (f16)((float)a[j] + scale * (float)b[j]);
        *(f16x8 *)(dst + i * 8) = a;
    }
}

#define RUN(expr) ENGINE_RUN(u, expr)

static void op_gemm(ctx_unet *u, const f16 *X, size_t w, size_t bias, bool has_bias, const void *res, int M, int N, int K, void *out,
                    int epi = 0, bool res_s = false, bool out_s = false)
{
    engine_linear(*u, X, u->W + w, has_bias ? u->W + bias : nullptr, res, M, N, K, out, 0, epi, u->res32 && res_s && res, u->res32 && out_s);
}
static void op_conv(ctx_unet *u, const f16 *x, size_t w, size_t bias, const f16 *rowbias, int ldrb, const void *res, int B, int H,
                    int W, int Cin, int Cout, int stride, int ups, void *out, bool res_s = false, bool out_s = false)
{
    engine_conv3(*u, x, u->W + w, u->W + bias, res, B, H, W, Cin, Cout, out, ConvGeom{stride, ups}, rowbias, ldrb, u->res32 && res_s && res,
                 u->res32 && out_s);
}
static void op_gn(ctx_unet *u, const void *x, size_t g, size_t b, int B, int HW, int C, float eps, int silu, f16 *y, void *stats, bool x_s = true)
{
    u->note(2, 0, 2);
    RUN(ctx_groupnorm_any(x, (u->res32 && x_s) ? 1 : 0, u->W + g, u->W + b, B, HW, C, u->cfg.groups, eps, silu, y, stats, u->s));
}
static void op_ln(ctx_unet *u, const void *x, size_t g, size_t b, int64_t rows, int C, f16 *y)
{
    u->note(2, 0);
    RUN(ctx_layernorm_any(x, u->res32 ? 1 : 0, u->W + g, u->W + b, rows, C, 1e-5f, y, u->s));
}
static const f16 *op_as16(ctx_unet *u, const void *x, size_t n)
{
    if (!u->res32) return (const f16 *)x;
    f16 *c = u->allocH(n);
    u->note(2, 0);
    RUN(ctx_f32_to_f16((const float *)x, (int64_t)n, c, u->s));
    return c;
}
static void op_attn(ctx_unet *u, const f16 *Q, const f16 *K, const f16 *V, int B, int Sq, int Skv, int heads, int qs, int kvs, f16 *O)
{
    u->note(1, 4.0 * B * heads * (double)Sq * Skv * 64);
    RUN(ctx_attention_core(Q, K, V, B, Sq, Skv, heads, qs, kvs, 0.125f, O, heads * 64, u->s));
}

struct FwdCtx {
    int B, L;
    const f16 *tproj;
    const f16 *ctx16;
    const f16 *kv_all;
    void *gn_stats;
};

static void *run_resnet(ctx_unet *u, const FwdCtx &f, const ResP &r, const void *x, int H, int W, void *out)
{
    const int B = f.B, HW = H * W, M = B * HW;
    size_t mark = u->top;
    f16 *t1 = u->allocH((size_t)M * r.cin);
    op_gn(u, x, r.n1g, r.n1b, B, HW, r.cin, u->cfg.norm_eps, 1, t1, f.gn_stats);
    f16 *h = u->allocH((size_t)M * r.cout);
    op_conv(u, t1, r.c1w, r.c1b, f.tproj ? f.tproj + r.temb_row : nullptr, u->temb_rows, nullptr, B, H, W, r.cin, r.cout, 1, 0, h);
    f16 *t2 = u->allocH((size_t)M * r.cout);
    op_gn(u, h, r.n2g, r.n2b, B, HW, r.cout, u->cfg.norm_eps, 1, t2, f.gn_stats, false);
    const void *sc = x;
    if (r.cin != r.cout) {
        void *s2 = u->allocS((size_t)M * r.cout);
        op_gemm(u, op_as16(u, x, (size_t)M * r.cin), r.scw, r.scb, true, nullptr, M, r.cout, r.cin, s2, 0, false, true);
        sc = s2;
    }
    op_conv(u, t2, r.c2w, r.c2b, nullptr, 0, sc, B, H, W, r.cout, r.cout, 1, 0, out, true, true);
    u->top = mark;
    return out;
}

static void *run_transformer(ctx_unet *u, const FwdCtx &f, const TrP &t, const void *x, int H, int W, void *out)
{
    const int B = f.B, S = H * W, M = B * S, C = t.C, cd = u->cfg.cross_attention_dim;
    size_t mark = u->top;
    f16 *g = u->allocH((size_t)M * C);
    op_gn(u, x, t.ng, t.nb, B, S, C, 1e-6f, 0, g, f.gn_stats);
    void *h0 = u->allocS((size_t)M * C);
    op_gemm(u, g, t.piw, t.pib, true, nullptr, M, C, C, h0, 0, false, true);
    f16 *l = g;
    op_ln(u, h0, t.l1g, t.l1b, M, C, l);
    f16 *a = nullptr;
    if (u->ref_mode == 2) {
        if (u->ref_k >= (int)u->ref_slots.size() || u->ref_slots[u->ref_k].C != C ||
            u->ref_slots[u->ref_k].rows != B - u->ref_row0) {
            u->rc = CTX_E_STATE;
            ctx_set_error("unet: the reference bank does not match this pass (run the 'w' pass on the condition latent first; layer %d)", u->ref_k);
            u->top = mark;
            return out;
        }
        const ctx_unet::RefSlot sl = u->ref_slots[u->ref_k++];
        f16 *q = u->allocH((size_t)M * C);
        op_gemm(u, l, t.qkv, 0, false, nullptr, M, C, C, q);
        a = u->allocH((size_t)M * C);
        f16 *kv = u->allocH((size_t)(S + sl.tokens) * 2 * C);
        for (int b = 0; b < B; ++b) {
            const int Sr = b >= u->ref_row0 ? sl.tokens : 0;
            op_gemm(u, l ? l + (size_t)b * S * C : nullptr, t.qkv + (size_t)C * C, 0, false, nullptr, S, 2 * C, C, kv);
            if (Sr)
                op_gemm(u, u->ref_bank ? u->ref_bank + sl.off + (size_t)(b - u->ref_row0) * sl.tokens * C : nullptr,
                        t.qkv + (size_t)C * C, 0, false, nullptr, Sr, 2 * C, C, kv ? kv + (size_t)S * 2 * C : nullptr);
            op_attn(u, q ? q + (size_t)b * S * C : nullptr, kv, kv ? kv + C : nullptr, 1, S, S + Sr, t.heads, C, 2 * C,
                    a ? a + (size_t)b * S * C : nullptr);
        }
    } else {
        if (u->ref_mode == 1) {
            ctx_unet::RefSlot sl; sl.off = u->ref_cursor; sl.tokens = S; sl.C = C; sl.rows = B;
            u->ref_slots.push_back(sl);
            u->ref_cursor += (size_t)M * C;
            if (u->ref_bank) u->copy(u->ref_bank + sl.off, l, (size_t)M * C * 2);
        }
        f16 *qkv = u->allocH((size_t)M * 3 * C);
        op_gemm(u, l, t.qkv, 0, false, nullptr, M, 3 * C, C, qkv);
        a = u->allocH((size_t)M * C);
        op_attn(u, qkv, qkv + C, qkv + 2 * C, B, S, S, t.heads, 3 * C, 3 * C, a);
    }
    void *h1 = u->allocS((size_t)M * C);
    op_gemm(u, a, t.o1w, t.o1b, true, h0, M, C, C, h1, 0, true, true);
    op_ln(u, h1, t.l2g, t.l2b, M, C, l);
    f16 *q = a;
    op_gemm(u, l, t.q2, 0, false, nullptr, M, C, C, q);
    const f16 *kv = f.kv_all + t.kv_row;
    f16 *a2 = u->allocH((size_t)M * C);
    op_attn(u, q, kv, kv + C, B, S, f.L, t.heads, C, u->kv_rows_total, a2);
    void *h2 = h0;
    op_gemm(u, a2, t.o2w, t.o2b, true, h1, M, C, C, h2, 0, true, true);
    op_ln(u, h2, t.l3g, t.l3b, M, C, l);
    f16 *ff = u->allocH((size_t)M * 4 * C);
    op_gemm(u, l, t.f1w, t.f1b, true, nullptr, M, 8 * C, C, ff, 1);
    void *h3 = h1;
    op_gemm(u, ff, t.f2w, t.f2b, true, h2, M, C, 4 * C, h3, 0, true, true);
    op_gemm(u, op_as16(u, h3, (size_t)M * C), t.pow_, t.pob, true, x, M, C, C, out, 0, true, true);
    u->top = mark;
    return out;
}

static int unet_run(ctx_unet *u, const float *sample, const float *timestep, const float *ctx, int B, int H, int W, int L, float *out)
{
    const ctx_unet_config_t &c = u->cfg;
    const int n = c.n_levels, lpb = c.layers_per_block;
    const int *ch = c.block_out_channels;
    u->begin();
    u->ref_k = 0; u->ref_cursor = 0;
    u->taps.clear(); u->tap_cursor = 0;
    if (u->ref_mode == 1) u->ref_slots.clear();
    FwdCtx f; f.B = B; f.L = L;
    f.gn_stats = u->alloc((size_t)ctx_groupnorm_ws_bytes(B, c.groups));
// ... 58 lines not shown
    }
    struct Skip { void *p; int C, h, w; };
    std::vector<Skip> skips;
    skips.push_back({x, ch[0], h, w});
    u->tap(x, B * h * w, ch[0]);
    int cur = ch[0];
    for (int i = 0; i < n; ++i) {
        LevelP &Lv = u->down[i];
        for (int j = 0; j < lpb; ++j) {
            int cout = Lv.res[j].cout;
            void *o = u->allocS((size_t)B * h * w * cout);
            if (Lv.has_attn) {
                size_t mark = u->top;
                void *t = u->allocS((size_t)B * h * w * cout);
                run_resnet(u, f, Lv.res[j], x, h, w, t);
                u->tap(t, B * h * w, cout);
                run_transformer(u, f, Lv.tr[j], t, h, w, o);
                u->top = mark;
            } else run_resnet(u, f, Lv.res[j], x, h, w, o);
            u->tap(o, B * h * w, cout);
            x = o; cur = cout;
            skips.push_back({x, cur, h, w});
        }
        if (Lv.has_sampler) {
            int ho = (h - 1) / 2 + 1, wo = (w - 1) / 2 + 1;
            void *o = u->allocS((size_t)B * ho * wo * cur);
            size_t m0 = u->top;
            op_conv(u, op_as16(u, x, (size_t)B * h * w * cur), Lv.sw, Lv.sb, nullptr, 0, nullptr, B, h, w, cur, cur, 2, 0, o, false, true);
            u->top = m0;
            x = o; h = ho; w = wo;
            u->tap(x, B * h * w, cur);
            skips.push_back({x, cur, h, w});
        }
    }
    size_t res_off = 0;
    if (u->is_controlnet) {
        if (skips.size() != u->zc_w.size()) { ctx_set_error("controlnet: %zu skip tensors but %zu zero convolutions", skips.size(), u->zc_w.size()); return CTX_E_STATE; }
        for (size_t k = 0; k < skips.size(); ++k) {
            const Skip &sk = skips[k];
            const size_t nel = (size_t)B * sk.h * sk.w * sk.C;
            op_gemm(u, (const f16 *)sk.p, u->zc_w[k], u->zc_b[k], true, nullptr, B * sk.h * sk.w, sk.C, sk.C, u->cn_out ? u->cn_out + res_off : nullptr);
            res_off += nel;
        }
    } else if (u->add_res) {
        for (size_t k = 0; k < skips.size(); ++k) {
            Skip &sk = skips[k];
            const size_t nel = (size_t)B * sk.h * sk.w * sk.C;
            if (sk.p == x) {
                f16 *cp = u->allocH(nel);
                u->copy(cp, sk.p, nel * 2);
                sk.p = cp;
            }
            add_scaled((f16 *)sk.p, u->add_res + res_off, u->add_scale, nel);
            res_off += nel;
        }
    }
    {
        void *o1 = u->allocS((size_t)B * h * w * cur);
        run_resnet(u, f, u->mid.res[0], x, h, w, o1);
        u->tap(o1, B * h * w, cur);
        void *o2 = u->allocS((size_t)B * h * w * cur);
        run_transformer(u, f, u->mid.tr[0], o1, h, w, o2);
        u->tap(o2, B * h * w, cur);
        void *o3 = u->allocS((size_t)B * h * w * cur);
        run_resnet(u, f, u->mid.res[1], o2, h, w, o3);
        u->tap(o3, B * h * w, cur);
        x = o3;
    }
    if (u->is_controlnet) {
        op_gemm(u, (const f16 *)x, u->zm_w, u->zm_b, true, nullptr, B * h * w, cur, cur, u->cn_out ? u->cn_out + res_off : nullptr);
        res_off += (size_t)B * h * w * cur;
        u->ref_cursor = res_off;
        return engine_finish(u, "controlnet_forward");
    }
    if (u->add_res) add_scaled((f16 *)x, u->add_res + res_off, u->add_scale, (size_t)B * h * w * cur);
    for (int i = 0; i < n; ++i) {
        LevelP &Lv = u->up[i];
        for (int j = 0; j <= lpb; ++j) {
            Skip sk = skips.back(); skips.pop_back();
            if (sk.h != h || sk.w != w) { ctx_set_error("unet: skip size mismatch (H, W must be multiples of %d)", 1 << (n - 1)); return CTX_E_ARG; }
            int cin = cur + sk.C, cout = Lv.res[j].cout;
            void *o = u->allocS((size_t)B * h * w * cout);
            size_t mark = u->top;
            void *cat = u->allocS((size_t)B * h * w * cin);
            u->note(2, 0);
            if (u->res32) RUN(ctx_concat_f32((const float *)x, (const float *)sk.p, (int64_t)B * h * w, cur, sk.C, (float *)cat, u->s));
            else RUN(ctx_concat_f16((const f16 *)x, (const f16 *)sk.p, (int64_t)B * h * w, cur, sk.C, (f16 *)cat, u->s));
            if (Lv.has_attn) {
                void *t = u->allocS((size_t)B * h * w * cout);
                run_resnet(u, f, Lv.res[j], cat, h, w, t);
                u->tap(t, B * h * w, cout);
                run_transformer(u, f, Lv.tr[j], t, h, w, o);
            } else run_resnet(u, f, Lv.res[j], cat, h, w, o);
            u->tap(o, B * h * w, cout);
            u->top = mark;
            x = o; cur = cout;
        }
        if (Lv.has_sampler) {
            void *o = u->allocS((size_t)B * (2 * h) * (2 * w) * cur);
            size_t m0 = u->top;
            op_conv(u, op_as16(u, x, (size_t)B * h * w * cur), Lv.sw, Lv.sb, nullptr, 0, nullptr, B, h, w, cur, cur, 1, 1, o, false, true);
            u->top = m0;
            x = o; h *= 2; w *= 2;
            u->tap(x, B * h * w, cur);
        }
    }
    f16 *y = u->allocH((size_t)B * h * w * cur);
    op_gn(u, x, u->cng, u->cnb, B, h * w, cur, c.norm_eps, 1, y, f.gn_stats);
    u->note(2, 2.0 * B * h * w * cur * c.out_channels * 9);
    RUN(ctx_conv_out_f16(y, u->W + u->cow, u->W + u->cob, B, h, w, cur, c.out_channels, out, u->s));
    return engine_finish(u, "unet_forward");
}

static int unet_dry(ctx_unet *u, int B, int H, int W, int L)
{
    return engine_dry_run(u, [&] { return unet_run(u, nullptr, nullptr, nullptr, B, H, W, L, nullptr); });
}

static int check_dims(const ctx_unet *u, int B, int H, int W, int L)
{
    int div = 1 << (u->cfg.n_levels - 1);
    if (B < 1 || B > 16 || H < div || W < div || H % div || W % div || L < 1) {
        ctx_set_error("unet: need 1<=B<=16, H,W multiples of %d, ctx_len>=1 (B=%d H=%d W=%d L=%d)", div, B, H, W, L);
        return CTX_E_ARG;
    }
    return 0;
}

extern "C" int64_t ctx_unet_workspace_bytes(const ctx_unet_t *cu, int32_t B, int32_t H, int32_t W, int32_t ctx_len)
{
    ctx_unet *u = const_cast<ctx_unet *>(cu);
    if (!u || check_dims(u, B, H, W, ctx_len)) return -1;
    unet_dry(u, B, H, W, ctx_len);
    return engine_workspace_need(u);
}

extern "C" int32_t ctx_unet_forward(ctx_unet_t *u, const float *sample, const float *timestep, const float *ctx, int32_t B,
                                    int32_t H, int32_t W, int32_t ctx_len, float *out, ctx_stream_t stream)
{
    CTX_REQUIRE(u && sample && timestep && ctx && out, "unet_forward: null pointer");
    CTX_REQUIRE(u->W && u->ws, "unet_forward: ctx_unet_bind() first");
    if (check_dims(u, B, H, W, ctx_len)) return CTX_E_ARG;
    u->s = (hipStream_t)stream;
    u->dry = false;
    return unet_run(u, sample, timestep, ctx, B, H, W, ctx_len, out);
}

extern "C" int64_t ctx_controlnet_residual_bytes(const ctx_unet_t *cu, int32_t B, int32_t H, int32_t W)
{
    ctx_unet *u = const_cast<ctx_unet *>(cu);
    if (!u || !u->is_controlnet || check_dims(u, B, H, W, 1)) return -1;
    return unet_dry(u, B, H, W, 1) ? -1 : (int64_t)u->ref_cursor * 2 + 256;
}

extern "C" int64_t ctx_controlnet_cond_cache_bytes(const ctx_unet_t *u, int32_t B, int32_t H, int32_t W)
{
    if (!u || !u->is_controlnet || B < 1 || H < 1 || W < 1 || u->cond_convs.size() < 2) return -1;
    return (int64_t)B * H * W * u->cond_convs[u->cond_convs.size() - 2].cout * 2 + 256;
}

extern "C" int32_t ctx_controlnet_forward(ctx_unet_t *u, const float *sample, const float *timestep, const float *ctx, const float *cond,
                                          void *cond_cache, int32_t cache_valid, int32_t B, int32_t H, int32_t W, int32_t ctx_len,
                                          void *residuals, ctx_stream_t stream)
{
    CTX_REQUIRE(u && sample && timestep && ctx && cond && residuals, "controlnet_forward: null pointer");
    CTX_REQUIRE(!cache_valid || cond_cache, "controlnet_forward: cache_valid without a cond_cache buffer");
    CTX_REQUIRE(u->is_controlnet, "controlnet_forward: the handle is a UNet (create it with ctx_controlnet_create)");
    CTX_REQUIRE(u->W && u->ws, "controlnet_forward: ctx_unet_bind() first");
    if (check_dims(u, B, H, W, ctx_len)) return CTX_E_ARG;
    u->s = (hipStream_t)stream; u->dry = false;
    u->cn_cond = cond; u->cn_out = (f16 *)residuals; u->cn_cache = (f16 *)cond_cache; u->cn_cache_valid = cache_valid != 0;
    int rc = unet_run(u, sample, timestep, ctx, B, H, W, ctx_len, nullptr);
    u->cn_cond = nullptr; u->cn_out = nullptr; u->cn_cache = nullptr; u->cn_cache_valid = false;
    return rc;
}

// ... 79 lines not shown
```

include/ctx_nerf.h:

```cpp
#ifndef CTX_NERF_H
#define CTX_NERF_H
#include <stdint.h>
#ifdef __cplusplus
extern "C" {
#endif

#define CTX_OK 0
#define CTX_E_ARG (-1)
#define CTX_E_LAUNCH (-2)
#define CTX_E_STATE (-3)

typedef void *ctx_stream_t;

int32_t ctx_version(void);
const char *ctx_last_error(void);
int32_t ctx_device_check(void);

int32_t ctx_prepare_vertices(const float *verts, const int64_t *faces, const float *cam,
                             const float *proj3, int32_t B, int32_t V, int32_t F,
                             float *fv_cam, float *fv_img, float *fnorm,
                             void *ws , ctx_stream_t stream);

int64_t ctx_rasterize_ws_bytes(int32_t H, int32_t W, int32_t B, int32_t F);
int32_t ctx_rasterize_fwd(int32_t H, int32_t W, const float *face_z, const float *face_xy,
// ... 99 lines not shown
int32_t ctx_raymarch_composite_fwd_noise(const float *raw, const float *z_vals, const float *rays_d,
                                         const float *noise , int64_t R, int32_t S, int32_t white_bkgd,
                                         float *rgb, float *disp, float *acc, float *weights , float *depth,
                                         ctx_stream_t stream);
int32_t ctx_raymarch_composite_bwd(const float *raw, const float *z_vals, const float *rays_d,
                                   const float *noise , int64_t R, int32_t S, int32_t white_bkgd,
                                   const float *g_rgb, const float *g_disp, const float *g_acc, const float *g_weights,
                                   const float *g_depth, float *grad_raw, ctx_stream_t stream);

typedef struct ctx_unet ctx_unet_t;
typedef struct {
    int32_t in_channels, out_channels;
    int32_t n_levels;
    int32_t block_out_channels[4];
    int32_t heads[4];
    int32_t down_attn[4], up_attn[4];
    int32_t layers_per_block;
    int32_t cross_attention_dim;
    int32_t groups;
    float norm_eps;
} ctx_unet_config_t;

ctx_unet_t *ctx_unet_create(const ctx_unet_config_t *cfg);
void ctx_unet_destroy(ctx_unet_t *u);
int32_t ctx_unet_param_count(const ctx_unet_t *u);
const char *ctx_unet_param_name(const ctx_unet_t *u, int32_t i);
int32_t ctx_unet_param_shape(const ctx_unet_t *u, int32_t i, int64_t shape4[4]);
int64_t ctx_unet_weight_bytes(const ctx_unet_t *u);
int64_t ctx_unet_workspace_bytes(const ctx_unet_t *u, int32_t B, int32_t H, int32_t W, int32_t ctx_len);
int32_t ctx_unet_bind(ctx_unet_t *u, void *weights, void *workspace, int64_t workspace_bytes);
int32_t ctx_unet_set_param(ctx_unet_t *u, int32_t i, const float *src, ctx_stream_t stream);
int32_t ctx_unet_forward(ctx_unet_t *u, const float *sample, const float *timestep, const float *ctx,
                         int32_t B, int32_t H, int32_t W, int32_t ctx_len, float *out, ctx_stream_t stream);
int64_t ctx_unet_ref_bank_bytes(const ctx_unet_t *u, int32_t B, int32_t H, int32_t W);
int64_t ctx_unet_workspace_bytes_ref(const ctx_unet_t *u, int32_t B, int32_t H, int32_t W, int32_t ctx_len, int32_t mode,
                                     int32_t ref_row0);
int32_t ctx_unet_forward_ref(ctx_unet_t *u, const float *sample, const float *timestep, const float *ctx,
                             int32_t B, int32_t H, int32_t W, int32_t ctx_len, int32_t mode, void *bank, int32_t ref_row0,
                             float *out, ctx_stream_t stream);
ctx_unet_t *ctx_controlnet_create(const ctx_unet_config_t *cfg, int32_t cond_channels);
int64_t ctx_controlnet_residual_bytes(const ctx_unet_t *cn, int32_t B, int32_t H, int32_t W);
int64_t ctx_controlnet_cond_cache_bytes(const ctx_unet_t *cn, int32_t B, int32_t H, int32_t W);
int32_t ctx_controlnet_forward(ctx_unet_t *cn, const float *sample, const float *timestep, const float *ctx,
                               const float *cond , void *cond_cache, int32_t cache_valid,
                               int32_t B, int32_t H, int32_t W, int32_t ctx_len, void *residuals, ctx_stream_t stream);
int32_t ctx_unet_set_residuals(ctx_unet_t *u, const void *residuals , float scale);
int32_t ctx_unet_set_residual_fp32(ctx_unet_t *u, int32_t on);
int32_t ctx_unet_stats(const ctx_unet_t *u, int32_t klass, int64_t *launches, double *flops);
int32_t ctx_unet_set_taps(ctx_unet_t *u, void *buf, int64_t capacity);
int32_t ctx_unet_tap_count(const ctx_unet_t *u);
int32_t ctx_unet_tap_info(const ctx_unet_t *u, int32_t i, int64_t *offset, int32_t *rows, int32_t *channels);

typedef struct ctx_vae ctx_vae_t;
typedef struct {
    int32_t latent_channels, out_channels;
    int32_t n_levels;
    int32_t block_out_channels[4];
    int32_t layers_per_block;
    int32_t groups;
} ctx_vae_config_t;
ctx_vae_t *ctx_vae_create(const ctx_vae_config_t *cfg);
void ctx_vae_destroy(ctx_vae_t *v);
int32_t ctx_vae_param_count(const ctx_vae_t *v);
const char *ctx_vae_param_name(const ctx_vae_t *v, int32_t i);
int32_t ctx_vae_param_shape(const ctx_vae_t *v, int32_t i, int64_t shape4[4]);
int64_t ctx_vae_weight_bytes(const ctx_vae_t *v);
int64_t ctx_vae_workspace_bytes(const ctx_vae_t *v, int32_t B, int32_t H, int32_t W);
int32_t ctx_vae_bind(ctx_vae_t *v, void *weights, void *workspace, int64_t workspace_bytes);
int32_t ctx_vae_set_param(ctx_vae_t *v, int32_t i, const float *src, ctx_stream_t stream);
int32_t ctx_vae_decode(ctx_vae_t *v, const float *latents, int32_t B, int32_t H, int32_t W, float *image, ctx_stream_t stream);
int32_t ctx_vae_decoder_param_count(const ctx_vae_t *v);
int64_t ctx_vae_encode_workspace_bytes(const ctx_vae_t *v, int32_t B, int32_t H, int32_t W);
int32_t ctx_vae_encode(ctx_vae_t *v, const float *image, int32_t B, int32_t H, int32_t W, float *moments, ctx_stream_t stream);
double ctx_vae_flops(const ctx_vae_t *v);
int64_t ctx_vae_encode_train_workspace_bytes(const ctx_vae_t *v, int32_t B, int32_t H, int32_t W);
int32_t ctx_vae_encode_train(ctx_vae_t *v, const float *image, int32_t B, int32_t H, int32_t W, float *moments, ctx_stream_t stream);
int32_t ctx_vae_encode_bwd(ctx_vae_t *v, const float *grad_moments, float gscale, float *grad_image, ctx_stream_t stream);

int32_t ctx_gemm_f16(const void *A, const void *Wt, const void *bias, const void *residual,
                     int32_t M, int32_t N, int32_t K, void *C, ctx_stream_t stream);
int32_t ctx_conv3x3_f16(const void *x, const void *w, const void *bias, const void *rowbias,
                        const void *residual, int32_t B, int32_t H, int32_t W, int32_t Cin,
                        int32_t Cout, int32_t stride, int32_t upsample, void *y, ctx_stream_t stream);
int64_t ctx_groupnorm_ws_bytes(int32_t B, int32_t groups);
int32_t ctx_groupnorm_f16(const void *x, const void *gamma, const void *beta, int32_t B, int32_t HW,
                          int32_t C, int32_t groups, float eps, int32_t silu, void *y, void *stats_ws,
                          ctx_stream_t stream);
int32_t ctx_layernorm_f16(const void *x, const void *gamma, const void *beta, int64_t rows, int32_t C,
                          float eps, void *y, ctx_stream_t stream);
int64_t ctx_attention_ws_bytes(int32_t B, int32_t Skv, int32_t heads);
int32_t ctx_attention_f16(const void *Q, const void *K, const void *V, int32_t B, int32_t Sq, int32_t Skv,
                          int32_t heads, int32_t q_stride, int32_t kv_stride, float scale, void *O,
                          int32_t o_stride, void *vt_ws, ctx_stream_t stream);
int32_t ctx_geglu_f16(const void *h, int64_t M, int32_t C4, void *y, ctx_stream_t stream);

int32_t ctx_cfg_plms_step(const float *eps_pair, int64_t n, float guidance, float *ets, int32_t head,
                          const float *coef4, float sample_coeff, float eps_coeff, int32_t mode,
                          float *cur_sample_ws, float *x, ctx_stream_t stream);

int32_t ctx_profile_begin(void);
int32_t ctx_profile_end(int32_t klass, double *total_ms , int64_t *count );

float ctx_bench_gemm(const void *A, const void *Wt, const void *bias, const void *residual, int32_t M, int32_t N, int32_t K,
                     void *C, int32_t conv_B, int32_t conv_H, int32_t conv_W, int32_t conv_Cin, int32_t conv_flags, int32_t epi,
                     void *part, int32_t splitk, int32_t iters, ctx_stream_t stream);

void ctx_gemm_tune(int32_t tile, int32_t gemm8);

void ctx_attention_tune(int32_t ns, int32_t nw8, int32_t spread, float lazy);

int32_t ctx_probe_mfma(int32_t which, const void *A, const void *Bt, float *C, ctx_stream_t stream);

float ctx_probe_stage(int32_t mode, int32_t waves, int32_t u, int32_t iters, int32_t shared_region, const void *src, void *sink,
                      ctx_stream_t stream);

#ifdef __cplusplus
}
#endif
#endif
```

Before: 116.8 steps/s.

## Fold resnet shortcut GEMM into conv2 as K segments and drop skip concat

When a resnet block has a 1x1 shortcut projection, the shortcut is appended as extra K segments to the second 3x3 conv GEMM. The block input and shortcut weights are read directly, and a second bias is added in the epilogue, so the separate shortcut GEMM and its residual round trip go away. In up blocks the skip concatenation is also avoided: groupnorm reads the two inputs separately and the conv segments point at each source. This adds complexity to the conv address generation and tile selection, and one shape (M=4608, 320->640) is excluded by a hardcoded check.

```diff
diff --git a/contexture-nerf_amd/_lib.py b/contexture-nerf_amd/_lib.py
--- a/contexture-nerf_amd/_lib.py
+++ b/contexture-nerf_amd/_lib.py
@@ -100,7 +100,11 @@
     "ctx_vae_encode_bwd": (_i32, [_vp, _vp, _f32, _vp, _vp]),
     "ctx_gemm_f16": (_i32, [_vp, _vp, _vp, _vp, _i32, _i32, _i32, _vp, _vp]),
     "ctx_conv3x3_f16": (_i32, [_vp, _vp, _vp, _vp, _vp, _i32, _i32, _i32, _i32, _i32, _i32, _i32, _vp, _vp]),
+    "ctx_conv3x3_seg_f16": (_i32, [_vp, _vp, _vp, _vp, _vp, _vp, _i32, _i32, _i32, _i32, _i32, _vp, _vp, _i32, _i32, _vp, _vp, _i32, _i32,
+                                   _vp, _i32, _vp, _vp]),
+    "ctx_gemm_last_kernel": (None, [_vp, _vp]),
     "ctx_groupnorm_f16": (_i32, [_vp, _vp, _vp, _i32, _i32, _i32, _i32, _f32, _i32, _vp, _vp, _vp]),
+    "ctx_groupnorm2_f16": (_i32, [_vp, _vp, _i32, _vp, _vp, _i32, _i32, _i32, _i32, _f32, _i32, _vp, _vp, _vp]),
     "ctx_layernorm_f16": (_i32, [_vp, _vp, _vp, _i64, _i32, _f32, _vp, _vp]),
     "ctx_attention_ws_bytes": (_i64, [_i32, _i32, _i32]),
     "ctx_attention_f16": (_i32, [_vp, _vp, _vp, _i32, _i32, _i32, _i32, _i32, _i32, _f32, _vp, _i32, _vp, _vp]),
diff --git a/contexture-nerf_amd/csrc/conv_halo.hip b/contexture-nerf_amd/csrc/conv_halo.hip
--- a/contexture-nerf_amd/csrc/conv_halo.hip
+++ b/contexture-nerf_amd/csrc/conv_halo.hip
@@ -159,6 +159,7 @@
 
 int ctx_conv_halo_try(GemmArgs &a, int ni, hipStream_t s)
 {
+    if (a.nseg) return 0;
     if (a.stride != 1 || a.ups != 0 || (a.H & 15) || (a.W & 15) || a.Cin % 64 != 0 || a.epi != 0 || a.N % 8 != 0) return 0;
     const int B = a.M / (a.H * a.W);
     const int BN = 64 * ni;
diff --git a/contexture-nerf_amd/csrc/engine.h b/contexture-nerf_amd/csrc/engine.h
--- a/contexture-nerf_amd/csrc/engine.h
+++ b/contexture-nerf_amd/csrc/engine.h
@@ -65,8 +65,10 @@
 void engine_linear(Engine &e, const f16 *X, const f16 *Wt, const f16 *bias, const void *res, int M, int N, int K, void *out, int ldc = 0,
                    int epi = 0, bool res32 = false, bool out32 = false);
 struct ConvGeom { int stride = 1, ups = 0, poff = 0, zins = 0; };
+struct ConvSegs { int n = 0; const f16 *x[2] = {nullptr, nullptr}; const f16 *w[2] = {nullptr, nullptr}; int C[2] = {0, 0}, ldw[2] = {0, 0}; const f16 *bias2 = nullptr; };
 void engine_conv3(Engine &e, const f16 *x, const f16 *Wt, const f16 *bias, const void *res, int B, int H, int W, int Cin, int Cout, void *out,
-                  ConvGeom g = ConvGeom(), const f16 *rowbias = nullptr, int ldrb = 0, bool res32 = false, bool out32 = false);
+                  ConvGeom g = ConvGeom(), const f16 *rowbias = nullptr, int ldrb = 0, bool res32 = false, bool out32 = false,
+                  const ConvSegs *segs = nullptr);
 
 template <class F> int engine_dry_run(Engine *e, F run)
 {
diff --git a/contexture-nerf_amd/csrc/engine.hip b/contexture-nerf_amd/csrc/engine.hip
--- a/contexture-nerf_amd/csrc/engine.hip
+++ b/contexture-nerf_amd/csrc/engine.hip
@@ -21,11 +21,21 @@
     return CTX_OK;
 }
 
-static void engine_gemm(Engine &e, GemmArgs &a, bool conv)
+static void engine_gemm(Engine &e, GemmArgs &a, bool conv, const ConvSegs *segs = nullptr)
 {
     e.note(0, 2.0 * a.M * a.N * a.K);
     size_t mark = e.top;
     ctx_gemm_plan(a, conv);
+    if (segs && segs->n) {
+        int kseg = 0;
+        a.nseg = segs->n; a.bias2 = segs->bias2;
+        for (int i = 0; i < segs->n; ++i) {
+            a.segX[i] = segs->x[i]; a.segW[i] = segs->w[i]; a.segC[i] = segs->C[i]; a.segLdw[i] = segs->ldw[i];
+            kseg += segs->C[i];
+        }
+        a.K += kseg;
+        e.note(0, 2.0 * a.M * a.N * kseg);
+    }
     if (a.zins) a.use8 = 0;
     if (a.splitk > 1) a.part = (float *)e.alloc((size_t)a.splitk * a.M * a.N * 4);
     ENGINE_RUN(&e, ctx_gemm_dispatch(a, conv, e.s));
@@ -43,7 +53,7 @@
 }
 
 void engine_conv3(Engine &e, const f16 *x, const f16 *Wt, const f16 *bias, const void *res, int B, int H, int W, int Cin, int Cout, void *out,
-                  ConvGeom g, const f16 *rowbias, int ldrb, bool res32, bool out32)
+                  ConvGeom g, const f16 *rowbias, int ldrb, bool res32, bool out32, const ConvSegs *segs)
 {
     GemmArgs a = {};
     a.Ho = ((H << g.ups) - 1) / g.stride + 1; a.Wo = ((W << g.ups) - 1) / g.stride + 1;
@@ -51,7 +61,7 @@
     a.M = B * a.Ho * a.Wo; a.N = Cout; a.K = 9 * Cin; a.ldc = Cout; a.ldr = Cout; a.rows_per_batch = a.Ho * a.Wo; a.ldrb = ldrb;
     a.H = H; a.W = W; a.Cin = Cin; a.stride = g.stride; a.ups = g.ups; a.poff = g.poff; a.zins = g.zins;
     a.res32 = res32; a.out32 = out32;
-    engine_gemm(e, a, true);
+    engine_gemm(e, a, true, segs);
 }
 
 int engine_finish(Engine *e, const char *who)
diff --git a/contexture-nerf_amd/csrc/gemm.hip b/contexture-nerf_amd/csrc/gemm.hip
--- a/contexture-nerf_amd/csrc/gemm.hip
+++ b/contexture-nerf_amd/csrc/gemm.hip
@@ -33,8 +33,7 @@
                     int nn = nw + ni * 32 + 8 * g + 4 * h;
                     if (nn >= a.N) continue;
                     f32x4 v = acc4(acc[mi][ni], g);
-                    if (a.bias) v = add4(v, *(const f16x4 *)(a.bias + nn));
-                    store4<true>(a, v, m, bidx, nn);
+                    store4<true>(a, bias4(a, v, nn), m, bidx, nn);
                 }
         }
     }
@@ -66,6 +65,7 @@
             if (m < a.M && n < a.N) {
                 float v[8] = {v0[0], v0[1], v0[2], v0[3], v1[0], v1[1], v1[2], v1[3]};
                 add8(v, bs);
+                if (a.bias2) add8(v, *(const f16x8 *)(a.bias2 + n));
                 store8<true>(a, v, m, n);
             }
         }
@@ -114,11 +114,11 @@
     for (int i = 0; i < WI; ++i) {
         int row = RP * (wave + NW * i) + lr;
         bool ok = (n0 + row) < a.N;
-        wp[i] = ok ? a.Wt + (size_t)(n0 + row) * a.K + kbeg * PKT + ((pc ^ (PKT == 32 ? ((row >> 2) & 3) : ((row >> 1) & 7))) * 8) : ctx_zero_page;
+        wp[i] = ok ? a.Wt + (size_t)(n0 + row) * (CONV ? 9 * a.Cin : a.K) + kbeg * PKT + ((pc ^ (PKT == 32 ? ((row >> 2) & 3) : ((row >> 1) & 7))) * 8) : ctx_zero_page;
         wst[i] = ok ? PKT : 0;
     }
     const int k_lo = kbeg * PKT, k_hi = (kbeg + nk) * PKT;
-    const int rot = a.krot == 1 ? (int)(((unsigned)tile_m * 13u + (unsigned)tile_n * 5u) % (unsigned)nk) : 0;
+    const int rot = a.krot == 1 && !a.nseg ? (int)(((unsigned)tile_m * 13u + (unsigned)tile_n * 5u) % (unsigned)nk) : 0;
     int k_issue = k_lo + rot * PKT, issued = 0, tap_left = 0;
     if (!CONV) {
 #pragma unroll
@@ -128,14 +128,29 @@
     for (int i = 0; i < WI; ++i) wp[i] += (wst[i] ? rot * PKT : 0);
 
     auto retap = [&]() {
-        const ConvTap tap = conv_tap(a, k_issue);
+        const bool seg = a.nseg && k_issue >= 9 * a.Cin;
+        const ConvSrc cs = conv_stage_src(a, k_issue);
+        const int sg = cs.src - 9;
+        const ConvTap tap = conv_tap(a, seg ? 4 * a.Cin : k_issue);
+        unsigned lox = 0;
+        if (seg) {
+            static_assert(PKT == 32 || NW % 2 == 0, "the chunk swizzle must not depend on the piece");
+            const int ln = conv_seg_lane(lane), lr = ln / LPR, row0 = RP * wave + lr;
+            lox = (unsigned)(lr * cs.C + ((ln % LPR) ^ (PKT == 32 ? ((row0 >> 2) & 3) : ((row0 >> 1) & 7))) * 8);
+            const ConvWJump wj = conv_seg_wjump(a, sg, cs.c0, k_issue, sg == 0 || issued == 0);
+#pragma unroll
+            for (int i = 0; i < WI; ++i) {
+                const long step = wj.jump + ((long)(n0 + RP * (wave + NW * i)) * wj.dld + lr * wj.dld) * (long)sizeof(f16);
+                wp[i] = (const f16 *)((const char *)wp[i] + (wst[i] ? step : 0));
+            }
+        }
 #pragma unroll
         for (int i = 0; i < XI; ++i) {
             bool ok = xok[i];
-            xp[i] = conv_tap_src<true>(a, tap, xoy[i], xox[i], xoff[i], ok);
+            xp[i] = conv_tap_src<true>(a, tap, xoy[i], xox[i], xoff[i], ok, seg ? conv_seg_x(a, sg, m0 + RP * (wave + NW * i), cs.c0) + lox : nullptr);
             xst[i] = ok ? PKT : 0;
         }
-        tap_left = (a.Cin - tap.c0) / PKT;
+        tap_left = (cs.C - cs.c0) / PKT;
     };
     auto issue = [&](int buf) {
         if (k_issue == k_hi) {
@@ -271,12 +286,13 @@
             f32x4 p = *(const f32x4 *)(a.part + sidx * MN + (size_t)m * a.N + nn);
             v += p;
         }
-        if (a.bias) v = add4(v, *(const f16x4 *)(a.bias + nn));
+        v = bias4(a, v, nn);
         store4<true>(a, v, m, a.rowbias ? m / a.rows_per_batch : 0, nn);
     }
 }
 
 static int g_force_tile = -1, g_force_gemm8 = -1;
+static int g_last_tile = -1, g_last_use8 = -1;
 extern "C" void ctx_gemm_tune(int32_t tile, int32_t gemm8)
 {
     g_force_tile = tile;
@@ -373,6 +389,21 @@
 
 int ctx_gemm_dispatch(GemmArgs &a, bool conv, hipStream_t s)
 {
+    bool seg64 = true;
+    if (a.nseg) {
+        int kseg = 0;
+        bool ok = conv && a.nseg <= CTX_GEMM_MAX_SEG && a.stride == 1 && !a.ups && !a.poff && !a.zins && a.epi == 0;
+        for (int i = 0; ok && i < a.nseg; ++i) {
+            ok = a.segX[i] && a.segW[i] && a.segC[i] > 0 && a.segC[i] % 32 == 0 && a.segLdw[i] % 8 == 0;
+            ok = ok && (int64_t)a.M * a.segC[i] < (1ll << 31) && (int64_t)a.N * a.segLdw[i] < (1ll << 31);
+            seg64 = seg64 && a.segC[i] % 64 == 0;
+            kseg += a.segC[i];
+        }
+        if (!ok || a.K != 9 * a.Cin + kseg) {
+            ctx_set_error("gemm: K segments need a stride-1 3x3 convolution without upsample and channel counts in multiples of 32");
+            return CTX_E_ARG;
+        }
+    }
     const bool only_pipe = a.zins || a.res32 || a.out32;
     if (only_pipe) a.use8 = 0;
     const int want8 = only_pipe ? 0 : (g_force_gemm8 >= 0 ? g_force_gemm8 : a.use8);
@@ -380,6 +411,7 @@
     const bool launched = want_tile < 0 && ((want8 >= 4 && want8 <= 8 && ctx_gemm144_try(a, conv, want8 - 4, s)) ||
                                             (conv && (want8 == 2 || want8 == 3) && ctx_conv_halo_try(a, want8 == 2 ? 2 : 1, s)) ||
                                             (want8 != 0 && want8 < 2 && ctx_gemm8_try(a, conv, want8 == 1, s)));
+    g_last_use8 = launched ? (want8 < 0 ? 1 : want8) : 0; g_last_tile = -1;
     if (!launched) {
         static const int big = ctx_env_int("CTX_GEMM_BIG", 1);
         const int S = a.splitk > 1 && a.part ? a.splitk : 1;
@@ -397,8 +429,9 @@
         if (force >= 0) pick = force;
         if (want_tile >= 0) pick = want_tile;
         if (a.epi == 1 && (pick == 5 || pick == 6 || pick == 9 || pick == 11 || pick == 13 || pick == 15 || pick == 17 || pick == 19 || pick == 21 || pick == 23 || pick == 26 || pick == 27)) pick = 1;
-        if (pick >= 10 && (a.K % 64 != 0 || (conv && a.Cin % 64 != 0))) pick = 1;
+        if (pick >= 10 && (a.K % 64 != 0 || (conv && a.Cin % 64 != 0) || !seg64)) pick = 1;
 #define CTX_LAUNCH(WM_, WN_, MI_, NI_) do { if (conv) launch_gemm<WM_, WN_, MI_, NI_, true>(a, s); else launch_gemm<WM_, WN_, MI_, NI_, false>(a, s); } while (0)
+        g_last_tile = pick;
         switch (pick) {
         case 0: CTX_LAUNCH(4, 2, 2, 2); break;
         case 1: CTX_LAUNCH(2, 2, 2, 2); break;
@@ -446,6 +479,12 @@
     return CTX_OK;
 }
 
+extern "C" void ctx_gemm_last_kernel(int32_t *tile, int32_t *use8)
+{
+    if (tile) *tile = g_last_tile;
+    if (use8) *use8 = g_last_use8;
+}
+
 extern "C" int32_t ctx_gemm_f16(const void *A, const void *Wt, const void *bias, const void *residual, int32_t M,
                                 int32_t N, int32_t K, void *C, ctx_stream_t stream)
 {
@@ -479,6 +518,30 @@
     return ctx_gemm_dispatch(a, true, (hipStream_t)stream);
 }
 
+extern "C" int32_t ctx_conv3x3_seg_f16(const void *x, const void *w, const void *bias, const void *bias2, const void *rowbias,
+                                       const void *residual, int32_t B, int32_t H, int32_t W, int32_t Cin, int32_t Cout, const void *xa,
+                                       const void *wa, int32_t Ca, int32_t ldwa, const void *xb, const void *wb, int32_t Cb, int32_t ldwb,
+                                       void *part, int32_t splitk, void *y, ctx_stream_t stream)
+{
+    CTX_REQUIRE(x && w && y && xa && wa, "conv3x3_seg: null pointer");
+    CTX_REQUIRE(B > 0 && H > 0 && W > 0 && Cin % 32 == 0 && Cout % 8 == 0, "conv3x3_seg: need Cin%%32==0, Cout%%8==0 (Cin=%d Cout=%d)", Cin, Cout);
+    GemmArgs a = {};
+    a.Ho = H; a.Wo = W;
+    a.X = (const f16 *)x; a.Wt = (const f16 *)w; a.bias = (const f16 *)bias; a.bias2 = (const f16 *)bias2; a.rowbias = (const f16 *)rowbias;
+    a.residual = (const f16 *)residual; a.out = (f16 *)y;
+    a.M = B * H * W; a.N = Cout; a.K = 9 * Cin; a.ldc = Cout; a.ldr = Cout; a.rows_per_batch = H * W; a.ldrb = Cout;
+    a.H = H; a.W = W; a.Cin = Cin; a.stride = 1;
+    a.tile = -1; a.use8 = -1;
+    if (splitk < 0 && part) ctx_gemm_plan(a, true); else a.splitk = splitk;
+    a.part = (float *)part;
+    a.nseg = xb ? 2 : 1;
+    a.segX[0] = (const f16 *)xa; a.segW[0] = (const f16 *)wa; a.segC[0] = Ca; a.segLdw[0] = ldwa;
+    a.segX[1] = (const f16 *)xb; a.segW[1] = (const f16 *)wb; a.segC[1] = xb ? Cb : 0; a.segLdw[1] = ldwb;
+    a.K += a.segC[0] + a.segC[1];
+    CTX_REQUIRE((int64_t)a.M * (Cin > Ca + Cb ? Cin : Ca + Cb) < (1ll << 31) && (int64_t)Cout * a.K < (1ll << 31), "conv3x3_seg: tensor too large for 32-bit offsets");
+    return ctx_gemm_dispatch(a, true, (hipStream_t)stream);
+}
+
 #define GV_U 4
 __global__ __launch_bounds__(256) void k_gemv_f16(const f16 *__restrict__ x, const f16 *__restrict__ w,
                                                   const f16 *__restrict__ bias, int Bm, int N, int K, int silu_in,
diff --git a/contexture-nerf_amd/csrc/gemm144.hip b/contexture-nerf_amd/csrc/gemm144.hip
--- a/contexture-nerf_amd/csrc/gemm144.hip
+++ b/contexture-nerf_amd/csrc/gemm144.hip
@@ -12,6 +12,7 @@
     constexpr int BM = 16 * BMB, NPX = BM / 8;
     constexpr int NP = NPX + 20;
     constexpr int STAGE = (BM + G144_BN) * 64;
+    static_assert(NPX % 2 == 0, "the K segments' chunk swizzle takes a weight piece's parity from its slot");
     static_assert(BMB % WM == 0 && (BMB == 9 || (BMB == 18 && VAR == 0)), "288-row tiles: lockstep schedule only");
     constexpr int SL = (NP + NW - 1) / NW;
     static_assert(9 % WM == 0 && 10 % WN == 0, "wave grid must divide 9 x 10 blocks");
@@ -60,25 +61,44 @@
         } else {
             const bool ok = live && (n0 + s) < a.N;
             xok[i] = ok;
-            pp[i] = ok ? a.Wt + (size_t)(n0 + s) * a.K + (size_t)kbeg * 64 + xlc[i] : ctx_zero_page;
+            pp[i] = ok ? a.Wt + (size_t)(n0 + s) * (CONV ? 9 * a.Cin : a.K) + (size_t)kbeg * 64 + xlc[i] : ctx_zero_page;
             pst[i] = ok ? 64 : 0;
         }
     }
 
     int k_issue = kbeg * 64, issued = 0, tap_left = 0;
-    int cur_tap = CONV ? (kbeg * 64) / a.Cin : 0, cur_c0 = CONV ? kbeg * 64 - cur_tap * a.Cin : 0;
+    int cur_tap = 0, cur_c0 = 0, cur_C = a.Cin;
+    if (CONV) { const ConvSrc cs = conv_stage_src(a, kbeg * 64); cur_tap = cs.src; cur_c0 = cs.c0; cur_C = cs.C; }
     auto retap = [&]() {
         if (FAST) {
-            const int dy = cur_tap / 3 - 1 + a.poff, dx = cur_tap - (cur_tap / 3) * 3 - 1 + a.poff;
-            const int soff = (dy * a.W + dx) * a.Cin + cur_c0;
+            const bool seg = cur_tap >= 9;
+            const int sg = cur_tap - 9, tap = seg ? 4 : cur_tap;
+            if (seg) cur_C = sg ? a.segC[1] : a.segC[0];
+            const int dy = tap / 3 - 1 + a.poff, dx = tap - (tap / 3) * 3 - 1 + a.poff;
+            const int soff = seg ? cur_c0 : (dy * a.W + dx) * a.Cin + cur_c0;
+            ConvWJump wj = {0, 0};
+            if (seg) wj = conv_seg_wjump(a, sg, cur_c0, k_issue, sg == 0 || issued == 0);
 #pragma unroll
             for (int i = 0; i < SL; ++i) {
-                if (wave + NW * i >= NPX) continue;
-                const bool v = (xval[i] >> cur_tap) & 1;
-                pp[i] = v ? xcen[i] + soff : zp;
+                const int p = wave + NW * i;
+                if (p >= NPX) {
+                    if (seg) {
+                        const int prow = conv_seg_lane(lane) >> 3;
+                        const long step = wj.jump + ((long)(n0 + 8 * (p - NPX)) * wj.dld + prow * wj.dld) * (long)sizeof(f16);
+                        pp[i] = (const f16 *)((const char *)pp[i] + (pst[i] ? step : 0));
+                    }
+                    continue;
+                }
+                const f16 *cen = xcen[i];
+                if (seg) {
+                    const int ln = conv_seg_lane(lane), prow = ln >> 3;
+                    cen = conv_seg_x(a, sg, m0 + 8 * p, 0) + (unsigned)(prow * cur_C + (((ln & 7) ^ (prow >> 1) ^ ((p & 1) << 2)) << 3));
+                }
+                const bool v = (xval[i] >> tap) & 1;
+                pp[i] = v ? cen + soff : zp;
                 pst[i] = v ? 64 : 0;
             }
-            tap_left = (a.Cin - cur_c0) >> 6;
+            tap_left = (cur_C - cur_c0) >> 6;
             return;
         }
         const ConvTap tap = conv_tap(a, k_issue);
@@ -106,7 +126,7 @@
     };
     auto issue_end = [&]() {
         k_issue += 64; ++issued;
-        if (FAST) { cur_c0 += 64; if (cur_c0 == a.Cin) { cur_c0 = 0; ++cur_tap; } }
+        if (FAST) { cur_c0 += 64; if (cur_c0 == cur_C) { cur_c0 = 0; ++cur_tap; } }
     };
     auto issue = [&](int buf) {
         issue_begin();
@@ -349,7 +369,7 @@
                 if (m >= a.M || n >= a.N) continue;
                 const f32x4 v0 = *(const f32x4 *)(tile + row * RS + c8), v1 = *(const f32x4 *)(tile + row * RS + c8 + 4);
                 float v[8] = {v0[0], v0[1], v0[2], v0[3], v1[0], v1[1], v1[2], v1[3]};
-                if (a.bias) add8(v, *(const f16x8 *)(a.bias + n));
+                bias8(a, v, n);
                 store8(a, v, m, n);
             }
         }
@@ -370,7 +390,9 @@
         for (int j = 0; j < NI; ++j) {
             const int nn = nb + 16 * j + 4 * kg;
             if (nn >= a.N) continue;
-            store4(a, add4(acc[i][j], bs[j]), m, bidx, nn);
+            f32x4 v = add4(acc[i][j], bs[j]);
+            if (a.bias2) v = add4(v, *(const f16x4 *)(a.bias2 + nn));
+            store4(a, v, m, bidx, nn);
         }
     }
 }
@@ -378,6 +400,8 @@
 int ctx_gemm144_try(GemmArgs &a, bool conv, int form, hipStream_t s)
 {
     if (a.K % 64 != 0 || (conv && a.Cin % 64 != 0) || a.N % 4 != 0 || a.epi != 0 || a.res32 || a.out32 || a.zins) return 0;
+    for (int i = 0; i < a.nseg; ++i)
+        if (a.segC[i] % 64 != 0 || a.segLdw[i] % 64 != 0) return 0;
     if (a.ldc % 4 != 0 || (a.residual && a.ldr % 4 != 0) || (a.rowbias && a.ldrb % 4 != 0)) return 0;
     const int bm = form == 4 ? 288 : G144_BM;
     a.ntm = cdiv(a.M, bm);
diff --git a/contexture-nerf_amd/csrc/gemm8.hip b/contexture-nerf_amd/csrc/gemm8.hip
--- a/contexture-nerf_amd/csrc/gemm8.hip
+++ b/contexture-nerf_amd/csrc/gemm8.hip
@@ -243,6 +243,7 @@
     const int min_tiles = ctx_env_int("CTX_GEMM8_MIN_TILES", 180);
     if (!en) return 0;
     if (a.K % 64 != 0 || (conv && a.Cin % 64 != 0) || a.N % 8 != 0) return 0;
+    if (a.nseg) return 0;
     if (a.epi == 1 && a.N % 64 != 0) return 0;
     const int ntm = cdiv(a.M, 256), ntn = cdiv(a.N, 256);
     const int S = (a.splitk > 1 && a.part) ? a.splitk : 1;
diff --git a/contexture-nerf_amd/csrc/gemm_common.h b/contexture-nerf_amd/csrc/gemm_common.h
--- a/contexture-nerf_amd/csrc/gemm_common.h
+++ b/contexture-nerf_amd/csrc/gemm_common.h
@@ -46,12 +46,45 @@
     return {tap / 3 - 1 + a.poff, tap % 3 - 1 + a.poff, k0 - tap * a.Cin, a.H << a.ups, a.W << a.ups};
 }
 template <bool ZINS = false>
-__device__ __forceinline__ const f16 *conv_tap_src(const GemmArgs &a, const ConvTap &t, int oy, int ox, int off, bool &ok)
+__device__ __forceinline__ const f16 *conv_tap_src(const GemmArgs &a, const ConvTap &t, int oy, int ox, int off, bool &ok, const f16 *cen = nullptr)
 {
     const int iy = oy + t.dy, ix = ox + t.dx;
     ok = ok && iy >= 0 && iy < t.Hv && ix >= 0 && ix < t.Wv;
     if (ZINS) ok = ok && !(a.zins && ((iy | ix) & 1));
-    return ok ? a.X + off + (((iy >> a.ups) * a.W + (ix >> a.ups)) * a.Cin) + t.c0 : ctx_zero_page;
+    const f16 *src = a.X + off + (((iy >> a.ups) * a.W + (ix >> a.ups)) * a.Cin) + t.c0;
+    if (cen) src = cen;
+    return ok ? src : ctx_zero_page;
+}
+
+struct ConvSrc { int src, c0, C; };
+__device__ __forceinline__ ConvSrc conv_stage_src(const GemmArgs &a, int k0)
+{
+    const int k9 = 9 * a.Cin;
+    if (k0 < k9) { const int tap = k0 / a.Cin; return {tap, k0 - tap * a.Cin, a.Cin}; }
+    const int k1 = k0 - k9;
+    if (k1 < a.segC[0]) return {9, k1, a.segC[0]};
+    return {10, k1 - a.segC[0], a.segC[1]};
+}
+__device__ __forceinline__ const f16 *conv_seg_x(const GemmArgs &a, int s, int m, int c)
+{
+    return (s ? a.segX[1] : a.segX[0]) + (unsigned)(m * (s ? a.segC[1] : a.segC[0]) + c);
+}
+__device__ __forceinline__ const f16 *conv_seg_w(const GemmArgs &a, int s, int n, int c)
+{
+    return (s ? a.segW[1] : a.segW[0]) + (unsigned)(n * (s ? a.segLdw[1] : a.segLdw[0]) + c);
+}
+__device__ __forceinline__ int conv_seg_lane(int lane)
+{
+    asm volatile("" : "+v"(lane));
+    return lane;
+}
+
+struct ConvWJump { long jump; int dld; };
+__device__ __forceinline__ ConvWJump conv_seg_wjump(const GemmArgs &a, int sg, int c0, int k_issue, bool fresh)
+{
+    const f16 *from = fresh ? a.Wt + k_issue : a.segW[0] + a.segC[0];
+    const f16 *to = (sg ? a.segW[1] : a.segW[0]) + c0;
+    return {(long)((const char *)to - (const char *)from), (sg ? a.segLdw[1] : a.segLdw[0]) - (fresh ? 9 * a.Cin : a.segLdw[0])};
 }
 
 __device__ __forceinline__ float fast_erf(float x)
@@ -75,6 +108,18 @@
 {
 #pragma unroll
     for (int e = 0; e < 8; ++e) v[e] += (float)b[e];
+}
+
+__device__ __forceinline__ f32x4 bias4(const GemmArgs &a, f32x4 v, int n)
+{
+    if (a.bias) v = add4(v, *(const f16x4 *)(a.bias + n));
+    if (a.bias2) v = add4(v, *(const f16x4 *)(a.bias2 + n));
+    return v;
+}
+__device__ __forceinline__ void bias8(const GemmArgs &a, float (&v)[8], int n)
+{
+    if (a.bias) add8(v, *(const f16x8 *)(a.bias + n));
+    if (a.bias2) add8(v, *(const f16x8 *)(a.bias2 + n));
 }
 
 template <bool F32 = false>
diff --git a/contexture-nerf_amd/csrc/kernels.h b/contexture-nerf_amd/csrc/kernels.h
--- a/contexture-nerf_amd/csrc/kernels.h
+++ b/contexture-nerf_amd/csrc/kernels.h
@@ -25,7 +25,13 @@
     int tile, use8;
     int stage_epi;
     int mfast;
+    int nseg;
+    const f16 *segX[2];
+    const f16 *segW[2];
+    int segC[2], segLdw[2];
+    const f16 *bias2;
 };
+#define CTX_GEMM_MAX_SEG 2
 
 int ctx_gemm_dispatch(GemmArgs &a, bool conv, hipStream_t s);
 int ctx_gemm8_try(GemmArgs &a, bool conv, bool force, hipStream_t s);
@@ -44,7 +50,7 @@
                        int kv_stride, float scale, f16 *O, int o_stride, hipStream_t s);
 extern "C" int64_t ctx_groupnorm_ws_bytes(int32_t B, int32_t groups);
 int ctx_groupnorm_any(const void *x, int x32, const void *gamma, const void *beta, int B, int HW, int C, int groups, float eps, int silu,
-                      void *y, void *stats_ws, hipStream_t stream);
+                      void *y, void *stats_ws, hipStream_t stream, const void *x2 = nullptr, int Ca = 0);
 int64_t ctx_groupnorm_bwd_ws_bytes(int B, int groups);
 int ctx_groupnorm_bwd_f16(const f16 *x, const f16 *dy, const f16 *gamma, const f16 *beta, const f16 *add, int B, int HW, int C, int groups,
                           float eps, int silu, f16 *dx, void *ws, hipStream_t s);
diff --git a/contexture-nerf_amd/csrc/norm.hip b/contexture-nerf_amd/csrc/norm.hip
--- a/contexture-nerf_amd/csrc/norm.hip
+++ b/contexture-nerf_amd/csrc/norm.hip
@@ -39,6 +39,13 @@
     return r;
 }
 
+struct GnSrc { const void *p; int cs, col; };
+__device__ __forceinline__ GnSrc gn_src(const void *x, const void *x2, int Ca, int C, int ch)
+{
+    if (!x2) return {x, C, ch};
+    return ch < Ca ? GnSrc{x, Ca, ch} : GnSrc{x2, C - Ca, ch - Ca};
+}
+
 #define GN_MAX_GROUPS 64
 #define GN_MAX_SPLITS 128
 #define GN_MAX_C 4096
@@ -47,8 +54,8 @@
 #define GN_FOLD 8
 
 template <bool X32>
-__global__ __launch_bounds__(1024) void k_gn_stats(const void *__restrict__ x, int HW, int C, int G, int NS, int PL,
-                                                   float *__restrict__ part)
+__global__ __launch_bounds__(1024) void k_gn_stats(const void *__restrict__ x, const void *__restrict__ x2, int Ca, int HW, int C, int G,
+                                                   int NS, int PL, float *__restrict__ part)
 {
     extern __shared__ float s_part[];
     const int c8n = C / 8;
@@ -59,11 +66,12 @@
     float s[8], q[8];
 #pragma unroll
     for (int j = 0; j < 8; ++j) { s[j] = 0.f; q[j] = 0.f; }
-    const size_t base = ((size_t)b * HW) * C + c8 * 8;
+    const GnSrc src = gn_src(x, x2, Ca, C, c8 * 8);
+    const size_t base = ((size_t)b * HW) * src.cs + src.col;
     for (int p = p0 + pl; p < p1; p += PL * GN_U) {
         Wide8 v[GN_U];
 #pragma unroll
-        for (int u = 0; u < GN_U; ++u) v[u] = ldraw<X32>(x, base + (size_t)min(p + u * PL, p1 - 1) * C).widen();
+        for (int u = 0; u < GN_U; ++u) v[u] = ldraw<X32>(src.p, base + (size_t)min(p + u * PL, p1 - 1) * src.cs).widen();
 #pragma unroll
         for (int u = 0; u < GN_U; ++u) {
             const bool live = p + u * PL < p1;
@@ -141,7 +149,7 @@
 }
 
 template <bool X32>
-__global__ __launch_bounds__(512) void k_gn_apply(const void *__restrict__ x, const float *__restrict__ part,
+__global__ __launch_bounds__(512) void k_gn_apply(const void *__restrict__ x, const void *__restrict__ x2, int Ca, const float *__restrict__ part,
                                                   const f16 *__restrict__ gamma, const f16 *__restrict__ beta, int HW, int C,
                                                   int G, int NS, int PL, float eps, int silu, f16 *__restrict__ y)
 {
@@ -151,11 +159,12 @@
     const int c8n = C / 8;
     const int c8 = threadIdx.x % c8n, pl = threadIdx.x / c8n;
     const int p0 = blockIdx.x * (PL * AU);
-    const size_t xb = (size_t)b * HW * C + c8 * 8;
+    const GnSrc src = gn_src(x, x2, Ca, C, c8 * 8);
+    const size_t xb = (size_t)b * HW * src.cs + src.col;
     f16 *yb = y + (size_t)b * HW * C + c8 * 8;
     Raw8<X32> v[AU];
 #pragma unroll
-    for (int u = 0; u < AU; ++u) v[u] = ldraw<X32>(x, xb + (size_t)min(p0 + u * PL + pl, HW - 1) * C);
+    for (int u = 0; u < AU; ++u) v[u] = ldraw<X32>(src.p, xb + (size_t)min(p0 + u * PL + pl, HW - 1) * src.cs);
     const f16x8 ga = *(const f16x8 *)(gamma + c8 * 8), be = *(const f16x8 *)(beta + c8 * 8);
     if (threadIdx.x < 256) {
         const int lpg = min(256 / G, 64);
@@ -192,7 +201,7 @@
 #define GN_FT 512
 #define GN_FU 12
 template <bool X32>
-__global__ __launch_bounds__(GN_FT) void k_gn_fused(const void *__restrict__ x, const f16 *__restrict__ gamma,
+__global__ __launch_bounds__(GN_FT) void k_gn_fused(const void *__restrict__ x, const void *__restrict__ x2, int Ca, const f16 *__restrict__ gamma,
                                                     const f16 *__restrict__ beta, int HW, int C, int G, int PLF, float eps, int silu,
                                                     f16 *__restrict__ y)
 {
@@ -201,12 +210,13 @@
     const int cg = C / G, cpg = cg / 8;
     const int c = threadIdx.x % cpg, pl = threadIdx.x / cpg;
     const bool act = pl < PLF;
-    const size_t xb = (size_t)b * HW * C + g * cg + c * 8;
+    const GnSrc src = gn_src(x, x2, Ca, C, g * cg + c * 8);
+    const size_t xb = (size_t)b * HW * src.cs + src.col;
     f16 *yb = y + (size_t)b * HW * C + g * cg + c * 8;
     const f16x8 ga = *(const f16x8 *)(gamma + g * cg + c * 8), be = *(const f16x8 *)(beta + g * cg + c * 8);
     Wide8 v[GN_FU];
 #pragma unroll
-    for (int u = 0; u < GN_FU; ++u) v[u] = ldraw<X32>(x, xb + (size_t)min(pl + PLF * u, HW - 1) * C).widen();
+    for (int u = 0; u < GN_FU; ++u) v[u] = ldraw<X32>(src.p, xb + (size_t)min(pl + PLF * u, HW - 1) * src.cs).widen();
     float s = 0.f, q = 0.f;
 #pragma unroll
     for (int u = 0; u < GN_FU; ++u)
@@ -242,10 +252,18 @@
     return ctx_groupnorm_any(x, 0, gamma, beta, B, HW, C, groups, eps, silu, y, stats_ws, (hipStream_t)stream);
 }
 
+extern "C" int32_t ctx_groupnorm2_f16(const void *xa, const void *xb, int32_t Ca, const void *gamma, const void *beta, int32_t B, int32_t HW,
+                                      int32_t C, int32_t groups, float eps, int32_t silu, void *y, void *stats_ws, ctx_stream_t stream)
+{
+    CTX_REQUIRE(xb, "groupnorm2: null pointer");
+    return ctx_groupnorm_any(xa, 0, gamma, beta, B, HW, C, groups, eps, silu, y, stats_ws, (hipStream_t)stream, xb, Ca);
+}
+
 int ctx_groupnorm_any(const void *x, int x32, const void *gamma, const void *beta, int B, int HW, int C, int groups, float eps, int silu,
-                      void *y, void *stats_ws, hipStream_t stream)
+                      void *y, void *stats_ws, hipStream_t stream, const void *x2, int Ca)
 {
     CTX_REQUIRE(x && gamma && beta && y && stats_ws, "groupnorm: null pointer");
+    CTX_REQUIRE(!x2 || (Ca > 0 && Ca < C && Ca % 8 == 0), "groupnorm: two sources need 0 < Ca < C in whole 8-channel columns (Ca=%d C=%d)", Ca, C);
     CTX_REQUIRE(B > 0 && HW > 0 && C % 8 == 0 && C % groups == 0 && groups <= GN_MAX_GROUPS && C <= GN_MAX_C &&
                     256 % groups == 0 && (256 / groups & (256 / groups - 1)) == 0,
                 "groupnorm: unsupported B=%d HW=%d C=%d groups=%d", B, HW, C, groups);
@@ -254,9 +272,9 @@
         const int cg = C / groups;
         const int cpg = cg / 8;
         const int plf = cg % 8 == 0 ? GN_FT / cpg : 0;
-        if (fuse && cg % 8 == 0 && cpg <= GN_FT && (HW + plf - 1) / plf <= GN_FU) {
+        if (fuse && cg % 8 == 0 && cpg <= GN_FT && (HW + plf - 1) / plf <= GN_FU && (!x2 || Ca % cg == 0)) {
             const int thr = (cpg * plf + 63) / 64 * 64;
-            CTX_BOOL_GO(x32, X, hipLaunchKernelGGL(k_gn_fused<X>, dim3(groups, B), dim3(thr), 0, stream, x, (const f16 *)gamma, (const f16 *)beta, HW, C,
+            CTX_BOOL_GO(x32, X, hipLaunchKernelGGL(k_gn_fused<X>, dim3(groups, B), dim3(thr), 0, stream, x, x2, Ca, (const f16 *)gamma, (const f16 *)beta, HW, C,
                                                    groups, plf, eps, silu, (f16 *)y));
             CTX_CHECK_LAUNCH("groupnorm");
             return CTX_OK;
@@ -284,12 +302,12 @@
         (void)hipFuncSetAttribute((const void *)k_gn_stats<true>, hipFuncAttributeMaxDynamicSharedMemorySize, 80 * 1024);
         attr = true;
     }
-    CTX_BOOL_GO(x32, X, hipLaunchKernelGGL(k_gn_stats<X>, dim3(NS, B), dim3(threads), lds, stream, x, HW, C, groups, NS, PL, part));
+    CTX_BOOL_GO(x32, X, hipLaunchKernelGGL(k_gn_stats<X>, dim3(NS, B), dim3(threads), lds, stream, x, x2, Ca, HW, C, groups, NS, PL, part));
     {
         const int apl = (256 + c8n - 1) / c8n;
         const int athreads = c8n * apl;
         const int nb = (HW + apl * GN_AU - 1) / (apl * GN_AU);
-        CTX_BOOL_GO(x32, X, hipLaunchKernelGGL(k_gn_apply<X>, dim3(nb, B), dim3(athreads), 0, stream, x, part, (const f16 *)gamma, (const f16 *)beta, HW, C,
+        CTX_BOOL_GO(x32, X, hipLaunchKernelGGL(k_gn_apply<X>, dim3(nb, B), dim3(athreads), 0, stream, x, x2, Ca, part, (const f16 *)gamma, (const f16 *)beta, HW, C,
                                                groups, NS, apl, eps, silu, (f16 *)y));
     }
     CTX_CHECK_LAUNCH("groupnorm");
diff --git a/contexture-nerf_amd/csrc/unet.hip b/contexture-nerf_amd/csrc/unet.hip
--- a/contexture-nerf_amd/csrc/unet.hip
+++ b/contexture-nerf_amd/csrc/unet.hip
@@ -338,15 +338,16 @@
     engine_linear(*u, X, u->W + w, has_bias ? u->W + bias : nullptr, res, M, N, K, out, 0, epi, u->res32 && res_s && res, u->res32 && out_s);
 }
 static void op_conv(ctx_unet *u, const f16 *x, size_t w, size_t bias, const f16 *rowbias, int ldrb, const void *res, int B, int H,
-                    int W, int Cin, int Cout, int stride, int ups, void *out, bool res_s = false, bool out_s = false)
+                    int W, int Cin, int Cout, int stride, int ups, void *out, bool res_s = false, bool out_s = false, const ConvSegs *segs = nullptr)
 {
     engine_conv3(*u, x, u->W + w, u->W + bias, res, B, H, W, Cin, Cout, out, ConvGeom{stride, ups}, rowbias, ldrb, u->res32 && res_s && res,
-                 u->res32 && out_s);
-}
-static void op_gn(ctx_unet *u, const void *x, size_t g, size_t b, int B, int HW, int C, float eps, int silu, f16 *y, void *stats, bool x_s = true)
+                 u->res32 && out_s, segs);
+}
+static void op_gn(ctx_unet *u, const void *x, size_t g, size_t b, int B, int HW, int C, float eps, int silu, f16 *y, void *stats, bool x_s = true,
+                  const void *x2 = nullptr, int Ca = 0)
 {
     u->note(2, 0, 2);
-    RUN(ctx_groupnorm_any(x, (u->res32 && x_s) ? 1 : 0, u->W + g, u->W + b, B, HW, C, u->cfg.groups, eps, silu, y, stats, u->s));
+    RUN(ctx_groupnorm_any(x, (u->res32 && x_s) ? 1 : 0, u->W + g, u->W + b, B, HW, C, u->cfg.groups, eps, silu, y, stats, u->s, x2, Ca));
 }
 static void op_ln(ctx_unet *u, const void *x, size_t g, size_t b, int64_t rows, int C, f16 *y)
 {
@@ -375,20 +376,53 @@
     void *gn_stats;
 };
 
-static void *run_resnet(ctx_unet *u, const FwdCtx &f, const ResP &r, const void *x, int H, int W, void *out)
+static int resnet_fold_mode(void)
+{
+    static const int m = ctx_env_int("CTX_RESNET_FOLD", 1);
+    return m;
+}
+static bool resnet_fold_loses(int M, int cin, int cout) { return M == 4608 && cin == 320 && cout == 640; }
+
+static void *run_resnet(ctx_unet *u, const FwdCtx &f, const ResP &r, const void *x, int H, int W, void *out, const void *x2 = nullptr, int Ca = 0)
 {
     const int B = f.B, HW = H * W, M = B * HW;
     size_t mark = u->top;
+    const int mode = u->res32 ? 0 : resnet_fold_mode();
+    const bool pair = Ca > 0;
+    const int Cb = r.cin - Ca;
+    const bool segs_ok = r.cout % 32 == 0 && (pair ? (Ca % 32 == 0 && Cb % 32 == 0) : r.cin % 32 == 0);
+    const bool fold = mode == 1 && r.cin != r.cout && segs_ok && !resnet_fold_loses(M, r.cin, r.cout);
+    const bool gn_pair = pair && mode != 0 && Ca % 8 == 0;
+    const void *xin = x;
+    if (pair) {
+        u->note(2, 0);
+        if (!gn_pair || !fold) {
+            void *cat = u->allocS((size_t)M * r.cin);
+            if (u->res32) RUN(ctx_concat_f32((const float *)x, (const float *)x2, (int64_t)M, Ca, Cb, (float *)cat, u->s));
+            else RUN(ctx_concat_f16((const f16 *)x, (const f16 *)x2, (int64_t)M, Ca, Cb, (f16 *)cat, u->s));
+            xin = cat;
+        }
+    }
     f16 *t1 = u->allocH((size_t)M * r.cin);
-    op_gn(u, x, r.n1g, r.n1b, B, HW, r.cin, u->cfg.norm_eps, 1, t1, f.gn_stats);
+    if (gn_pair) op_gn(u, x, r.n1g, r.n1b, B, HW, r.cin, u->cfg.norm_eps, 1, t1, f.gn_stats, true, x2, Ca);
+    else op_gn(u, xin, r.n1g, r.n1b, B, HW, r.cin, u->cfg.norm_eps, 1, t1, f.gn_stats);
     f16 *h = u->allocH((size_t)M * r.cout);
     op_conv(u, t1, r.c1w, r.c1b, f.tproj ? f.tproj + r.temb_row : nullptr, u->temb_rows, nullptr, B, H, W, r.cin, r.cout, 1, 0, h);
     f16 *t2 = u->allocH((size_t)M * r.cout);
     op_gn(u, h, r.n2g, r.n2b, B, HW, r.cout, u->cfg.norm_eps, 1, t2, f.gn_stats, false);
-    const void *sc = x;
+    if (fold) {
+        ConvSegs sg;
+        sg.n = pair ? 2 : 1; sg.bias2 = u->W + r.scb;
+        sg.x[0] = (const f16 *)x; sg.w[0] = u->W + r.scw; sg.C[0] = pair ? Ca : r.cin; sg.ldw[0] = r.cin;
+        if (pair) { sg.x[1] = (const f16 *)x2; sg.w[1] = u->W + r.scw + Ca; sg.C[1] = Cb; sg.ldw[1] = r.cin; }
+        op_conv(u, t2, r.c2w, r.c2b, nullptr, 0, nullptr, B, H, W, r.cout, r.cout, 1, 0, out, true, true, &sg);
+        u->top = mark;
+        return out;
+    }
+    const void *sc = xin;
     if (r.cin != r.cout) {
         void *s2 = u->allocS((size_t)M * r.cout);
-        op_gemm(u, op_as16(u, x, (size_t)M * r.cin), r.scw, r.scb, true, nullptr, M, r.cout, r.cin, s2, 0, false, true);
+        op_gemm(u, op_as16(u, xin, (size_t)M * r.cin), r.scw, r.scb, true, nullptr, M, r.cout, r.cin, s2, 0, false, true);
         sc = s2;
     }
     op_conv(u, t2, r.c2w, r.c2b, nullptr, 0, sc, B, H, W, r.cout, r.cout, 1, 0, out, true, true);
@@ -613,16 +647,13 @@
             int cin = cur + sk.C, cout = Lv.res[j].cout;
             void *o = u->allocS((size_t)B * h * w * cout);
             size_t mark = u->top;
-            void *cat = u->allocS((size_t)B * h * w * cin);
-            u->note(2, 0);
-            if (u->res32) RUN(ctx_concat_f32((const float *)x, (const float *)sk.p, (int64_t)B * h * w, cur, sk.C, (float *)cat, u->s));
-            else RUN(ctx_concat_f16((const f16 *)x, (const f16 *)sk.p, (int64_t)B * h * w, cur, sk.C, (f16 *)cat, u->s));
+            if (cin != Lv.res[j].cin) { ctx_set_error("unet: up block input has %d channels, its resnet expects %d", cin, Lv.res[j].cin); return CTX_E_STATE; }
             if (Lv.has_attn) {
                 void *t = u->allocS((size_t)B * h * w * cout);
-                run_resnet(u, f, Lv.res[j], cat, h, w, t);
+                run_resnet(u, f, Lv.res[j], x, h, w, t, sk.p, cur);
                 u->tap(t, B * h * w, cout);
                 run_transformer(u, f, Lv.tr[j], t, h, w, o);
-            } else run_resnet(u, f, Lv.res[j], cat, h, w, o);
+            } else run_resnet(u, f, Lv.res[j], x, h, w, o, sk.p, cur);
             u->tap(o, B * h * w, cout);
             u->top = mark;
             x = o; cur = cout;
diff --git a/include/ctx_nerf.h b/include/ctx_nerf.h
--- a/include/ctx_nerf.h
+++ b/include/ctx_nerf.h
@@ -205,10 +205,18 @@
 int32_t ctx_conv3x3_f16(const void *x, const void *w, const void *bias, const void *rowbias,
                         const void *residual, int32_t B, int32_t H, int32_t W, int32_t Cin,
                         int32_t Cout, int32_t stride, int32_t upsample, void *y, ctx_stream_t stream);
+int32_t ctx_conv3x3_seg_f16(const void *x, const void *w, const void *bias, const void *bias2, const void *rowbias,
+                            const void *residual, int32_t B, int32_t H, int32_t W, int32_t Cin, int32_t Cout,
+                            const void *xa, const void *wa, int32_t Ca, int32_t ldwa, const void *xb, const void *wb,
+                            int32_t Cb, int32_t ldwb, void *part, int32_t splitk, void *y, ctx_stream_t stream);
+void ctx_gemm_last_kernel(int32_t *tile, int32_t *use8);
 int64_t ctx_groupnorm_ws_bytes(int32_t B, int32_t groups);
 int32_t ctx_groupnorm_f16(const void *x, const void *gamma, const void *beta, int32_t B, int32_t HW,
                           int32_t C, int32_t groups, float eps, int32_t silu, void *y, void *stats_ws,
                           ctx_stream_t stream);
+int32_t ctx_groupnorm2_f16(const void *xa, const void *xb, int32_t Ca, const void *gamma, const void *beta, int32_t B,
+                           int32_t HW, int32_t C, int32_t groups, float eps, int32_t silu, void *y, void *stats_ws,
+                           ctx_stream_t stream);
 int32_t ctx_layernorm_f16(const void *x, const void *gamma, const void *beta, int64_t rows, int32_t C,
                           float eps, void *y, ctx_stream_t stream);
 int64_t ctx_attention_ws_bytes(int32_t B, int32_t Skv, int32_t heads);
```

Measured after the change: 118.6 steps/s, median of 6. 1.02x the previous value.
